# vlongle/pixie

Hardware: AMD Instinct MI355X
Metric: voxels/s (128^3 U-Net fwd) + MPM particle-steps/s (higher is better)
Workload: dtype f32 (operands split fp16 hi+lo, 3 f16 MFMAs/product, fp32 accumulate); 1 GPU; 128^3x64 feature grid -> SegmentationUNet+RegressionUNet forward (+argmax/one-hot combine), 1 scene per GPU per step; grid=128, feature_channels=64, parallelism=scene-parallel x1, executor=c+hip_graph

## Files before the change

### include/pixie_hip.h

```cpp
#ifndef PIXIE_HIP_H
#define PIXIE_HIP_H

#include <stdint.h>

#ifdef __cplusplus
extern "C" {
#endif

const char* pixie_last_error(void);
const char* pixie_build_arch(void);

typedef struct pixie_mpm pixie_mpm;

int pixie_mpm_create(pixie_mpm** out, int n_particles, int n_grid, double grid_lim);
int pixie_mpm_destroy(pixie_mpm* h);
int pixie_mpm_regrid(pixie_mpm* h, int n_grid, double grid_lim, void* stream);

int pixie_mpm_set_field(pixie_mpm* h, const char* name, const void* d_src, int64_t count, void* stream);
int pixie_mpm_get_field(pixie_mpm* h, const char* name, void* d_dst, int64_t count, void* stream);
int pixie_mpm_fill_field(pixie_mpm* h, const char* name, double value, void* stream);

int pixie_mpm_set_scalar(pixie_mpm* h, const char* key, double value);
int pixie_mpm_get_scalar(pixie_mpm* h, const char* key, double* value);

// ... 72 lines not shown
    int32_t in_d, in_h, in_w;
    int32_t upsample;
    int32_t stride;
    int32_t ksize;
    const float* d_pro_a; const float* d_pro_b;
    const float* d_gamma; const float* d_beta;
    int32_t act;
    const float* d_w; const float* d_bias;
    int32_t c_out;
    const float* d_residual;
    float* d_out;
    const void* d_w16;
    const uint32_t* d_in_amax0; const uint32_t* d_in_amax1;
    float in_bound;
    float* d_out_stats;
    uint32_t* d_out_amax;
    void* d_workspace;
    int32_t out_d, out_h, out_w;
    const float* d_skip_in0; int32_t skip_c0;
    const float* d_skip_in1; int32_t skip_c1;
    const void* d_skip_w16; const float* d_skip_bias;
    const uint32_t* d_skip_amax0; const uint32_t* d_skip_amax1;
    int32_t w16_subpixel;
} pixie_conv_desc;

int pixie_conv_cout_padded(int c_out);
int pixie_conv_pack_weights(const float* d_w_oidhw, float* d_w_packed, int c_out, int c_in, int ksize, void* stream);
int64_t pixie_conv_packed16_bytes(int c_out, int c_in, int ksize);
int pixie_conv_pack_weights_f16x2(const float* d_w_oidhw, void* d_packed, int c_out, int c_in, int ksize, void* stream);
int64_t pixie_conv_subpixel_bytes(int c_out, int c_in);
int pixie_conv_pack_weights_subpixel(const float* d_w_oidhw, void* d_packed, int c_out, int c_in, void* stream);
int pixie_conv3d_forward(const pixie_conv_desc* desc, void* stream);
int64_t pixie_conv_stats_floats(const pixie_conv_desc* desc);
int64_t pixie_conv_workspace_bytes(const pixie_conv_desc* desc);
int pixie_stats_finalize(const float* d_stats, const pixie_conv_desc* desc, double* d_sums, void* stream);
int pixie_stats_norm_finalize(const float* d_stats0, const pixie_conv_desc* desc0, double* d_sums0, const float* d_stats1,
                              const pixie_conv_desc* desc1, double* d_sums1, int c1, int64_t spatial, int mode, int groups,
                              double eps, const float* d_weight, const float* d_bias, float* d_a, float* d_b, void* stream);
int pixie_conv_skip_foldable(const pixie_conv_desc* desc);

int pixie_channel_sums(const float* d_x, int channels, int64_t spatial, double* d_sums, void* stream);
int pixie_channel_stats(const float* d_x, int channels, int64_t spatial, double* d_sums, uint32_t* d_amax, void* stream);
int pixie_tensor_amax(const float* d_x, int64_t count, uint32_t* d_slot, void* stream);
int pixie_norm_finalize(const double* d_sums, int channels, int64_t spatial, int mode, int groups, double eps,
                        const float* d_weight, const float* d_bias, float* d_a, float* d_b, void* stream);

int pixie_attention_forward(const float* d_qkv, float* d_out, int channels, int tokens, void* stream);

int pixie_channel_affine(const float* d_x, const float* d_a, const float* d_b, float* d_y, int channels,
                         int64_t spatial, void* stream);

int pixie_voxel_grid_to_ncdhw(const void* d_feat_dhwc_f16, int d, int h, int w, int channels, float* d_out_cdhw, void* stream);

int pixie_projector_conv0(const void* d_feat_dhwc_f16, int64_t voxels, int channels, int n_networks, const void* const* d_w16,
                          const float* const* d_bias, float* const* d_out, int c_out, void* stream);

int pixie_pack_fields(const float* d_cont, const int32_t* d_seg_pred, int64_t n_scenes, int64_t spatial, void* d_wire, int64_t wire_bytes,
                      void* stream);

int pixie_combine_predictions(const float* d_logits, int num_classes, const float* d_cont, int64_t spatial,
                              float* d_combined, int32_t* d_argmax , void* stream);

int pixie_combine_class_ids(const int32_t* d_seg_pred, int num_classes, const float* d_cont, int64_t spatial, float* d_combined,
                            void* stream);

typedef struct pixie_unet pixie_unet;
typedef struct pixie_unet_config {
    int32_t feature_channels, cond_dim, model_channels, num_res_blocks;
    int32_t n_channel_mult; int32_t channel_mult[8];
    int32_t n_attention_resolutions; int32_t attention_resolutions[8];
    int32_t grid_size;
    int32_t out_channels;
    int32_t precision;
} pixie_unet_config;

int pixie_unet_create(pixie_unet** out, const pixie_unet_config* cfg);
int pixie_unet_destroy(pixie_unet* h);
int pixie_unet_param_count(const pixie_unet* h);
int pixie_unet_param_info(const pixie_unet* h, int index, const char** key, int64_t* numel, int32_t* ndim, int64_t shape[5]);
int pixie_unet_set_param(pixie_unet* h, const char* key, const float* d_values, int64_t numel);
int64_t pixie_unet_workspace_bytes(pixie_unet* h, int d, int hh, int w);
int pixie_unet_forward(pixie_unet* h, const float* d_feat, const float* d_proj0, int d, int hh, int w, float* d_out,
                       void* d_workspace, int64_t workspace_bytes, void* stream);
int pixie_unet_set_option(pixie_unet* h, const char* key, int value);

typedef struct pixie_field_desc {
    const float* d_pred;
    const uint8_t* d_mask;
    const float* d_axis_x; const float* d_axis_y; const float* d_axis_z;
    int32_t n_classes, d, h, w;
    double min_spacing;
    double density_min, density_max, E_min, E_max, nu_min, nu_max;
} pixie_field_desc;
int pixie_field_to_particles(const pixie_field_desc* field, const float* d_pos, int n, int k, double nn_distance_threshold,
                             int weighted, int default_material, int default_part_label, float* d_density, float* d_E,
                             float* d_nu, int32_t* d_material, int32_t* d_part_label, float* d_conf, float* d_nearest,
                             void* d_scratch, void* stream);

int pixie_unscale_prediction(const float* d_pred, int channels, int64_t spatial, double density_min, double density_max,
                             double E_min, double E_max, double nu_min, double nu_max, float* d_out, void* stream);
int64_t pixie_field_points_scratch_bytes(const pixie_field_desc* field);
int pixie_field_points(const pixie_field_desc* field, int64_t capacity, float* d_xyz , float* d_density, float* d_E,
                       float* d_nu, int32_t* d_material, float* d_conf, int64_t* d_count, void* d_scratch, void* stream);

int pixie_dbscan_roots(const float* d_pos_sorted, const int32_t* d_orig_index, const int32_t* d_cell_start, int n, int nx, int ny, int nz,
                       const double lo[3], double cell_size, double eps, int min_samples, int32_t* d_core_scratch,
                       int32_t* d_parent_scratch, int32_t* d_root, void* stream);

int pixie_fill_densify(const float* d_pos, const float* d_opacity, const float* d_cov6, int n, int grid_n, double grid_dx,
                       int32_t* d_grid_count, float* d_grid_density, void* stream);
int pixie_fill_dense_cells(int32_t* d_grid_count, const float* d_grid_density, int grid_n, double grid_dx, double density_thres,
                           int max_particles_per_cell, float* d_new_particles , int64_t max_samples,
                           uint64_t* d_counter, uint32_t seed, void* stream);
int pixie_fill_internal_cells(int32_t* d_grid_count, const float* d_grid_density, int grid_n, double grid_dx, int max_particles_per_cell,
                              int exclude_dir, int ray_cast_dir, double threshold, float* d_new_particles, int64_t max_samples,
                              uint64_t* d_counter, uint32_t seed, void* stream);
int pixie_particle_volume(const float* d_pos, int n, int grid_n, double grid_dx, int32_t* d_grid_count_scratch, float* d_vol, void* stream);
int pixie_nearest_particle(const float* d_pos, int n, const float* d_new_pos, int n_new, int32_t* d_nearest, void* stream);

typedef struct pixie_raster_desc {
    int32_t n, width, height;
    float tanfovx, tanfovy, scale_modifier;
    float viewmatrix[16], projmatrix[16], bg[3];
    int32_t pad_;
    const float* d_means;
    const float* d_cov3d;
    const float* d_scales;
    const float* d_rotations;
    const float* d_colors;
    const float* d_opacity;
    float* d_out_color;
    int32_t* d_radii;
    float* d_final_T;
    int32_t* d_n_contrib;
    void* d_workspace;
    int64_t workspace_bytes;
} pixie_raster_desc;
int64_t pixie_raster_workspace_bytes(int n, int width, int height, int64_t max_instances);
int pixie_raster_forward(const pixie_raster_desc* desc, int64_t* instances_out, void* stream);
int pixie_sh_to_rgb(const float* d_shs, int64_t n, int k_coeffs, int degree, const float* d_pos , const float campos[3],
                    const float* d_rot , int64_t n_rot, float* d_out , void* stream);

typedef struct pixie_raster_view {
    float viewmatrix[16], projmatrix[16], campos[3];
    float tanfovx, tanfovy;
} pixie_raster_view;
typedef struct pixie_raster_batch_desc {
    int32_t views, n_dyn, n_static, width, height;
    int32_t sh_degree, k_coeffs;
    float scale_modifier;
    float bg[3];
    int32_t pad_;
    const pixie_raster_view* view;
    const float* d_means;
    const float* d_cov3d;
    int64_t means_view_stride, cov3d_view_stride;
    const float* d_static_means;
    const float* d_static_cov3d;
    const float* d_opacity;
    const float* d_colors;
    int64_t colors_view_stride;
    const float* d_shs;
    float* d_out_color;
    uint8_t* d_out_rgb8;
    int32_t* d_radii;
    float* d_final_T;
// ... 273 lines not shown
```

### pixie_amd/_lib.py

```python
from __future__ import annotations

import ctypes as C
import os

_HERE = os.path.dirname(os.path.abspath(__file__))
LIB_PATH = os.path.join(_HERE, "libpixie_hip.so")
DIAG_LIB_PATH = os.path.join(_HERE, "libpixie_hip_diag.so")


class PixieHipError(RuntimeError):
    pass


class BCDesc(C.Structure):
    _fields_ = [("type", C.c_int32), ("surface_type", C.c_int32), ("reset", C.c_int32), ("pad_", C.c_int32),
                ("point", C.c_double * 3), ("size", C.c_double * 3), ("velocity", C.c_double * 3),
                ("normal", C.c_double * 3), ("start_time", C.c_double), ("end_time", C.c_double),
                ("friction", C.c_double)]


class PModDesc(C.Structure):
    _fields_ = [("type", C.c_int32), ("pad_", C.c_int32),
                ("point", C.c_double * 3), ("size", C.c_double * 3), ("force", C.c_double * 3),
                ("velocity", C.c_double * 3), ("normal", C.c_double * 3), ("h1", C.c_double * 3),
# ... 179 lines not shown
                ("group", GsAdamGroup * 8)]


class GsDensifyDesc(C.Structure):
    _fields_ = [("n", C.c_int64), ("n_rest", C.c_int32), ("has_max_screen_size", C.c_int32),
                ("max_grad", C.c_double), ("min_opacity", C.c_double), ("extent", C.c_double), ("percent_dense", C.c_double),
                ("d_xyz_gradient_accum", C.c_void_p), ("d_denom", C.c_void_p),
                ("d_param", C.c_void_p * 6), ("d_exp_avg", C.c_void_p * 6), ("d_exp_avg_sq", C.c_void_p * 6),
                ("d_workspace", C.c_void_p), ("workspace_bytes", C.c_int64)]


class GsDensifyOuts(C.Structure):
    _fields_ = [("n_out", C.c_int64), ("n_split", C.c_int64), ("d_noise", C.c_void_p),
                ("d_param", C.c_void_p * 6), ("d_exp_avg", C.c_void_p * 6), ("d_exp_avg_sq", C.c_void_p * 6),
                ("d_source_index", C.c_void_p), ("d_xyz_gradient_accum", C.c_void_p), ("d_denom", C.c_void_p),
                ("d_max_radii2D", C.c_void_p)]


GS_DENSIFY_BAD_MAX_GRAD, GS_DENSIFY_TOO_MANY_ROWS, GS_DENSIFY_EMPTY = 2, 3, 4


INGEST_NO_SELECTION, INGEST_ZERO_EXTENT, INGEST_TOO_MANY_ROTATIONS, INGEST_TOO_MANY_ROWS = 2, 3, 4, 5


_VP, _I, _I64, _D, _S = C.c_void_p, C.c_int, C.c_int64, C.c_double, C.c_char_p
_D3 = C.POINTER(C.c_double)
SIGNATURES = {
    "pixie_last_error": (C.c_char_p, []),
    "pixie_build_arch": (C.c_char_p, []),
    "pixie_mpm_create": (_I, [C.POINTER(_VP), _I, _I, _D]),
    "pixie_mpm_destroy": (_I, [_VP]),
    "pixie_mpm_regrid": (_I, [_VP, _I, _D, _VP]),
    "pixie_mpm_set_field": (_I, [_VP, _S, _VP, _I64, _VP]),
    "pixie_mpm_get_field": (_I, [_VP, _S, _VP, _I64, _VP]),
    "pixie_mpm_fill_field": (_I, [_VP, _S, _D, _VP]),
    "pixie_mpm_set_scalar": (_I, [_VP, _S, _D]),
    "pixie_mpm_get_scalar": (_I, [_VP, _S, C.POINTER(_D)]),
    "pixie_mpm_update_mass": (_I, [_VP, _VP]),
    "pixie_mpm_finalize_mu_lam": (_I, [_VP, _I, _VP]),
    "pixie_mpm_apply_additional_params": (_I, [_VP, _D3, _D3, _D, _D, _D, _I, _VP]),
    "pixie_mpm_apply_additional_params_batch": (_I, [_VP, _I64, _VP, _VP, _VP, _VP]),
    "pixie_mpm_add_bc": (_I, [_VP, C.POINTER(BCDesc)]),
    "pixie_mpm_add_particle_modifier": (_I, [_VP, C.POINTER(PModDesc), _VP]),
    "pixie_mpm_step": (_I, [_VP, _D, _I, _VP]),
    "pixie_mpm_export_cov": (_I, [_VP, _VP, _VP]),
    "pixie_mpm_export_R": (_I, [_VP, _VP, _VP]),
    "pixie_mpm_export_frame": (_I, [_VP, _I, _D3, _D, _D3, C.POINTER(C.c_double), _VP, _VP, _VP]),
    "pixie_mpm_out_of_bounds": (_I, [_VP, C.POINTER(_I64), _VP]),
    "pixie_mpm_batch_create": (_I, [C.POINTER(_VP), C.POINTER(_VP), _I]),
    "pixie_mpm_batch_step": (_I, [_VP, _D, _I, _VP]),
    "pixie_mpm_batch_run": (_I, [_VP, C.POINTER(BatchSched), _I, _VP]),
    "pixie_mpm_batch_run_splats": (_I, [_VP, C.POINTER(BatchSched), C.POINTER(BatchSplatOut), _I, _VP]),
    "pixie_splat_from_cov": (_I, [_VP, _I64, _VP, _VP, _VP]),
    "pixie_mpm_export_frame_splats": (_I, [_VP, _I, _D3, _D, _D3, C.POINTER(C.c_double), _VP, _VP, _VP, _VP, _VP]),
    "pixie_mpm_batch_destroy": (_I, [_VP]),
    "pixie_pack_fields": (_I, [_VP, _VP, _I64, _I64, _VP, _I64, _VP]),
    "pixie_conv_cout_padded": (_I, [_I]),
    "pixie_conv_pack_weights": (_I, [_VP, _VP, _I, _I, _I, _VP]),
    "pixie_conv_packed16_bytes": (_I64, [_I, _I, _I]),
    "pixie_conv_pack_weights_f16x2": (_I, [_VP, _VP, _I, _I, _I, _VP]),
    "pixie_conv_subpixel_bytes": (_I64, [_I, _I]),
    "pixie_conv_pack_weights_subpixel": (_I, [_VP, _VP, _I, _I, _VP]),
    "pixie_conv3d_forward": (_I, [C.POINTER(ConvDesc), _VP]),
    "pixie_conv_stats_floats": (_I64, [C.POINTER(ConvDesc)]),
    "pixie_conv_workspace_bytes": (_I64, [C.POINTER(ConvDesc)]),
    "pixie_stats_finalize": (_I, [_VP, C.POINTER(ConvDesc), _VP, _VP]),
    "pixie_stats_norm_finalize": (_I, [_VP, C.POINTER(ConvDesc), _VP, _VP, C.POINTER(ConvDesc), _VP, _I, _I64, _I, _I, _D, _VP, _VP, _VP, _VP, _VP]),
    "pixie_channel_stats": (_I, [_VP, _I, _I64, _VP, _VP, _VP]),
    "pixie_tensor_amax": (_I, [_VP, _I64, _VP, _VP]),
    "pixie_channel_sums": (_I, [_VP, _I, _I64, _VP, _VP]),
    "pixie_norm_finalize": (_I, [_VP, _I, _I64, _I, _I, _D, _VP, _VP, _VP, _VP, _VP]),
    "pixie_attention_forward": (_I, [_VP, _VP, _I, _I, _VP]),
    "pixie_channel_affine": (_I, [_VP, _VP, _VP, _VP, _I, _I64, _VP]),
    "pixie_projector_conv0": (_I, [_VP, _I64, _I, _I, C.POINTER(_VP), C.POINTER(_VP), C.POINTER(_VP), _I, _VP]),
    "pixie_conv_skip_foldable": (_I, [C.POINTER(ConvDesc)]),
    "pixie_unet_create": (_I, [C.POINTER(_VP), C.POINTER(UNetConfigC)]),
    "pixie_unet_destroy": (_I, [_VP]),
    "pixie_unet_param_count": (_I, [_VP]),
    "pixie_unet_param_info": (_I, [_VP, _I, C.POINTER(_S), C.POINTER(_I64), C.POINTER(C.c_int32), C.POINTER(_I64)]),
    "pixie_unet_set_param": (_I, [_VP, _S, _VP, _I64]),
    "pixie_unet_workspace_bytes": (_I64, [_VP, _I, _I, _I]),
    "pixie_unet_set_option": (_I, [_VP, _S, _I]),
    "pixie_unet_forward": (_I, [_VP, _VP, _VP, _I, _I, _I, _VP, _VP, _I64, _VP]),
    "pixie_combine_class_ids": (_I, [_VP, _I, _VP, _I64, _VP, _VP]),
    "pixie_combine_predictions": (_I, [_VP, _I, _VP, _I64, _VP, _VP, _VP]),
    "pixie_voxel_grid_to_ncdhw": (_I, [_VP, _I, _I, _I, _I, _VP, _VP]),
    "pixie_unscale_prediction": (_I, [_VP, _I, _I64, _D, _D, _D, _D, _D, _D, _VP, _VP]),
    "pixie_field_points_scratch_bytes": (_I64, [C.POINTER(FieldDesc)]),
    "pixie_field_points": (_I, [C.POINTER(FieldDesc), _I64, _VP, _VP, _VP, _VP, _VP, _VP, _VP, _VP, _VP]),
    "pixie_fill_densify": (_I, [_VP, _VP, _VP, _I, _I, _D, _VP, _VP, _VP]),
    "pixie_fill_dense_cells": (_I, [_VP, _VP, _I, _D, _D, _I, _VP, _I64, _VP, C.c_uint32, _VP]),
    "pixie_fill_internal_cells": (_I, [_VP, _VP, _I, _D, _I, _I, _I, _D, _VP, _I64, _VP, C.c_uint32, _VP]),
    "pixie_particle_volume": (_I, [_VP, _I, _I, _D, _VP, _VP, _VP]),
    "pixie_nearest_particle": (_I, [_VP, _I, _VP, _I, _VP, _VP]),
    "pixie_dbscan_roots": (_I, [_VP, _VP, _VP, _I, _I, _I, _I, C.POINTER(_D), _D, _D, _I, _VP, _VP, _VP, _VP]),
    "pixie_raster_workspace_bytes": (_I64, [_I, _I, _I, _I64]),
    "pixie_raster_forward": (_I, [C.POINTER(RasterDesc), C.POINTER(_I64), _VP]),
    "pixie_raster_backward_workspace_bytes": (_I64, [_I, _I, _I, _I64]),
    "pixie_raster_backward": (_I, [C.POINTER(RasterBackwardDesc), _VP]),
    "pixie_sh_to_rgb": (_I, [_VP, _I64, _I, _I, _VP, C.POINTER(C.c_float), _VP, _I64, _VP, _VP]),
    "pixie_raster_batch_workspace_bytes": (_I64, [_I, _I, _I, _I, _I64]),
    "pixie_raster_forward_batch": (_I, [C.POINTER(RasterBatchDesc), C.POINTER(_I64), C.POINTER(C.c_int32), _VP]),
    "pixie_scene_ingest_workspace_bytes": (_I64, [_I64]),
    "pixie_scene_ingest": (_I, [C.POINTER(IngestDesc), C.POINTER(_I64), C.POINTER(C.c_float), C.POINTER(C.c_float), _VP]),
    "pixie_field_to_particles": (_I, [C.POINTER(FieldDesc), _VP, _I, _I, _D, _I, _I, _I, _VP, _VP, _VP, _VP, _VP, _VP, _VP, _VP, _VP]),
    "pixie_knn_mean_dist2_scratch_bytes": (_I64, [_I64]),
    "pixie_knn_mean_dist2": (_I, [_VP, _I64, _VP, _I64, _VP, _VP]),
    "pixie_photometric_workspace_bytes": (_I64, [_I, _I, _I, _I, _I]),
    "pixie_photometric_forward": (_I, [_VP, _VP, _I, _I, _I, _I, _VP, _I64, _I, _VP, _VP, _VP]),
    "pixie_photometric_backward": (_I, [_VP, _VP, _I, _I, _I, _I, _VP, _VP, _VP, _VP, _VP]),
    "pixie_gs_adam_step": (_I, [C.POINTER(GsAdamDesc), _VP]),
    "pixie_gs_densify_stats": (_I, [_VP, _VP, _I64, _VP, _VP, _VP, _VP]),
    "pixie_gs_densify_workspace_bytes": (_I64, [_I64]),
    "pixie_gs_densify_plan": (_I, [C.POINTER(GsDensifyDesc), C.POINTER(_I64), C.POINTER(_I64), _VP]),
    "pixie_gs_densify_emit": (_I, [C.POINTER(GsDensifyDesc), C.POINTER(GsDensifyOuts), _VP]),
    "pixie_occupancy_scratch_bytes": (_I64, [C.POINTER(OccupancyDesc), _I]),
    "pixie_occupancy_mask": (_I, [C.POINTER(OccupancyDesc), _VP, _VP, _VP, _VP, _VP]),
    "pixie_part_seg_scratch_bytes": (_I64, [C.POINTER(PartSegDesc)]),
    "pixie_part_segmentation": (_I, [C.POINTER(PartSegDesc), _VP, _VP, _VP, _VP, _VP, _VP, _VP]),
    "pixie_part_material_grid": (_I, [_VP, _VP, _I, _I64, C.c_float, _VP, _VP]),
    "pixie_hashmlp_forward": (_I, [C.POINTER(HashMlpDesc), _VP, _VP, _I64, _VP, _VP]),
    "pixie_hashmlp_train_bytes": (_I, [C.POINTER(HashMlpDesc), _I64, C.POINTER(_I64), C.POINTER(_I64)]),
    "pixie_hashmlp_forward_saved": (_I, [C.POINTER(HashMlpDesc), _VP, _VP, _I64, _VP, _VP, _VP]),
    "pixie_hashmlp_backward": (_I, [C.POINTER(HashMlpDesc), _VP, _VP, _I64, _VP, _VP, _VP, C.POINTER(HashMlpGrads), _VP, _VP]),
    "pixie_ray_composite_bytes": (_I, [C.POINTER(RayDesc), C.POINTER(_I64)]),
    "pixie_ray_composite_forward": (_I, [C.POINTER(RayDesc), C.POINTER(RayInputs), C.POINTER(RayOutputs), _VP]),
    "pixie_ray_composite_backward": (_I, [C.POINTER(RayDesc), C.POINTER(RayInputs), C.POINTER(RayUpstream), C.POINTER(RayGrads), _VP, _VP]),
    "pixie_field_voxelize": (_I, [C.POINTER(FieldVoxelizeDesc), _VP, _VP, _VP, _VP, _VP, _VP]),
    "pixie_field_query_points": (_I, [C.POINTER(FieldVoxelizeDesc), _VP, _I64, _D, _VP, _VP, _VP, _VP, _VP]),
}

DIAG_SIGNATURES = {
    "pixie_mpm_phase": (_I, [_VP, _I, _D, _VP]),
    "pixie_mpm_kernel_times": (_I, [_VP, C.POINTER(_D), C.POINTER(_D), C.POINTER(_I64)]),
    "pixie_conv_kernel_variant": (C.c_int, [C.POINTER(ConvDesc), C.POINTER(C.c_int)]),
    "pixie_conv_tile_geometry": (C.c_int, [C.POINTER(ConvDesc), C.POINTER(C.c_int32)]),
    "pixie_conv_stats_layout": (C.c_int, [C.POINTER(ConvDesc), C.POINTER(C.c_int64)]),
}

_libs = {}


def load(diag: bool = False):
    if diag in _libs:
        return _libs[diag]
    path = DIAG_LIB_PATH if diag else LIB_PATH
    if not os.path.exists(path):
        raise PixieHipError(
            f"{path} not found: build it with `python -m pixie_amd.build` (hipcc, gfx950). "
            "pixie_amd has no CPU fallback.")
    import torch
    lib = C.CDLL(path)
    for name, (res, args) in list(SIGNATURES.items()) + (list(DIAG_SIGNATURES.items()) if diag else []):
        fn = getattr(lib, name)
        fn.restype = res
        fn.argtypes = args
    _libs[diag] = lib
    return lib


def check(rc: int, what: str = "", lib=None):
    if rc != 0:
        msg = (lib or load()).pixie_last_error()
        raise PixieHipError(f"{what}: {msg.decode() if msg else 'unknown error'}")


# ... 11 lines not shown
```

### pixie_amd/csrc/common.hip

```cpp
#include "common.h"

#include <mutex>
#include <set>
#include <utility>

#include "../../include/pixie_hip.h"

namespace pixie {
hipError_t allow_max_dynamic_lds(const void* kern) {
    static std::mutex mu;
    static std::set<std::pair<const void*, int>> done;
    int dev = 0;
    hipError_t e = hipGetDevice(&dev);
    if (e != hipSuccess) return e;
    std::lock_guard<std::mutex> lock(mu);
    if (done.count({kern, dev})) return hipSuccess;
    e = hipFuncSetAttribute(kern, hipFuncAttributeMaxDynamicSharedMemorySize, 160 * 1024);
    if (e == hipSuccess) done.insert({kern, dev});
    return e;
}

std::string& last_error_ref() {
    static thread_local std::string msg;
    return msg;
}
int set_error(const char* fmt, ...) {
    char buf[1024];
    va_list ap;
    va_start(ap, fmt);
    vsnprintf(buf, sizeof buf, fmt, ap);
    va_end(ap);
    last_error_ref() = buf;
    return 1;
}
}

extern "C" const char* pixie_last_error(void) { return pixie::last_error_ref().c_str(); }
extern "C" const char* pixie_build_arch(void) { return "gfx950"; }
```

### pixie_amd/csrc/conv16_body.h

```cpp
#pragma once
#include <type_traits>

#include "conv16_device.h"

namespace pixie {

template <int KS, int MB, int NB, bool EX = false, bool SP = false, int SK = 0, bool PAIR = false>
__device__ __forceinline__ void conv3d_f16x3_body(const Conv16Args& A) {
    static_assert(!PAIR || (MB == 2 && !EX && !SP && SK == 0), "pair form: the plain f16x3 body with 64 c_out per quartet");
    static_assert(!SP || (KS == 3 && NB == 4 && !EX), "sub-pixel path: 3^3, two x parities x two voxel blocks per wave");
    static_assert(SK == 0 || (!EX && !SP), "folded skip (SK: 1 register-fed, 2 staged through LDS): f16x3, no sub-pixel form");
    extern __shared__ uint4 smem16[];
    constexpr int PAD = (KS == 3) ? 1 : 0;
    constexpr int NW = 4, NT = 64 * NW;
    const int bufsz = 4 * A.CS;

    const int tid = threadIdx.x;
    const int lane = tid & 63;
    const int quartet = PAIR ? __builtin_amdgcn_readfirstlane(tid >> 8) : 0;
    const int wave = PAIR ? (tid >> 6) & 3 : tid >> 6;
    const int qtid = PAIR ? tid & 255 : tid;
    const int kh = lane >> 5;
    const int l31 = lane & 31;

    int t = blockIdx.x;
    {
        const int per = (A.n_tiles + 7) >> 3;
        const int cand = (t & 7) * per + (t >> 3);
        if ((A.n_tiles & 7) == 0) t = cand;
    }
    int par = 0;
    if constexpr (SP) { par = t & 3; t >>= 2; }
    const int py = par & 1, pz = par >> 1;
    const int tx = t % A.tiles_x; t /= A.tiles_x;
    const int ty = t % A.tiles_y;
    const int tz = t / A.tiles_y;
    const int ox0 = tx * A.TX, oy0 = ty * A.TY, oz0 = tz * A.TZ;
    const int cout0 = (PAIR ? 2 * (int)blockIdx.y + quartet : (int)blockIdx.y) * (MB * 32);
    const int lx0 = SP ? ox0 - 1 : ox0 * A.stride - PAD;
    const int ly0 = SP ? oy0 - 1 + py : oy0 * A.stride - PAD;
    const int lz0 = SP ? oz0 - 1 + pz : oz0 * A.stride - PAD;
    const size_t ISP = (size_t)A.ID * A.IH * A.IW;
    const size_t OSP = (size_t)A.OD * A.OH * A.OW;

    int voff[NB];
    int ovox[NB];
    bool valid[NB];
#pragma unroll
    for (int nb = 0; nb < NB; ++nb) {
        if constexpr (SP) {
            const int px = nb >> 1;
            const int j = (wave * 2 + (nb & 1)) * 32 + l31;
            int x = j & (A.TX - 1);
            int y = (j >> A.lTX) & (A.TY - 1);
            int z = j >> (A.lTX + A.lTY);
            const int gx = 2 * (ox0 + x) + px, gy = 2 * (oy0 + y) + py, gz = 2 * (oz0 + z) + pz;
            const bool v = (z < A.TZ) && (gx < A.OW) && (gy < A.OH) && (gz < A.OD);
            if (!v) { x = 0; y = 0; z = 0; }
            voff[nb] = (z * A.HY + y) * A.HX + x + px + kh * A.CS;
            ovox[nb] = v ? (gz * A.OH + gy) * A.OW + gx : 0;
            valid[nb] = v;
            continue;
        }
        const int j = (wave * NB + nb) * 32 + l31;
        int x = j & (A.TX - 1);
        int y = (j >> A.lTX) & (A.TY - 1);
        int z = j >> (A.lTX + A.lTY);
        const bool v = (z < A.TZ) && (ox0 + x < A.OW) && (oy0 + y < A.OH) && (oz0 + z < A.OD);
        if (!v) { x = 0; y = 0; z = 0; }
        voff[nb] = ((z * A.HY + y) * A.HX + x) * A.stride + kh * A.CS;
        ovox[nb] = ((oz0 + z) * A.OH + (oy0 + y)) * A.OW + ox0 + x;
        valid[nb] = v;
    }

    float bound = A.in_bound;
    if (A.amax0) {
        bound = __uint_as_float(*A.amax0);
        if (A.amax1) bound = fmaxf(bound, __uint_as_float(*A.amax1));
    }
    const int ex = EX ? 0 : scale_exponent(bound);
    const float sx = pow2i(ex);

    f32x16 acc[MB][NB];
#pragma unroll
    for (int mb = 0; mb < MB; ++mb)
#pragma unroll
        for (int nb = 0; nb < NB; ++nb)
#pragma unroll
            for (int r = 0; r < 16; ++r) acc[mb][nb][r] = 0.0f;

    const int KG = A.cin >> 3;
    const size_t tap_stride = (size_t)KG * A.coutp;
    const size_t plane = (size_t)(SP ? 64 : KS * KS * KS) * tap_stride;
    const uint4* wHi = A.w16 + kW16HeaderU4 + (size_t)kh * A.coutp + cout0 + l31 + (size_t)(par * 16) * tap_stride;
    const uint4* wLo = wHi + plane;
    const float* wF = A.wf + (size_t)kh * A.coutp + cout0 + l31;

    constexpr int TAPS = KS * KS * KS;
#include "conv16_stage.h"
#include "conv16_taps.h"

    float inv2 = 0.0f;
    {
        const int c_begin = A.partial ? (int)blockIdx.z * A.chunks_per_slice * 16 : 0;
        const int c_end = A.partial ? min(A.cin, c_begin + A.chunks_per_slice * 16) : A.cin;
        if constexpr (PAIR) {
            const int n_chunks = (c_end - c_begin) >> 4;
            const int half = (A.CS + 1) >> 1;
            const int s0 = quartet ? half : 0, s1 = quartet ? A.CS : half;
#pragma unroll 1
            for (int h = -1; h < 2 * n_chunks; ++h) {
                const int k = h >> 1;
                const bool stage = (h < 0 || ((h + quartet) & 1) == 0) && k + 1 < n_chunks;
                const bool multiply = h >= 0 && ((h + quartet) & 1) != 0;
                if (stage) stage_chunk(c_begin + 16 * (k + 1), smem16 + ((k + 1) & 1) * bufsz, qtid, NT, s0, s1);
                if (multiply) mfma_chunk(c_begin + 16 * k, smem16 + (k & 1) * bufsz);
                if (h & 1) __syncthreads();
            }
        } else {
            for (int c_base = c_begin; c_base < c_end; c_base += 16) {
                __syncthreads();
                stage_chunk(c_base, smem16, tid, NT, 0, A.CS);
                __syncthreads();
                mfma_chunk(c_base, smem16);
            }
        }
#include "conv16_skip.h"
    }

#include "conv16_epilogue.h"
}

template <int KS, int MB, int NB>
__global__ __launch_bounds__(256, 2) void conv3d_f16x3_kernel(Conv16Args A) {
    conv3d_f16x3_body<KS, MB, NB>(A);
}
template <int KS, int NB>
__global__ __launch_bounds__(512, 1) void conv3d_f16x3_pair_kernel(Conv16Args A) {
    conv3d_f16x3_body<KS, 2, NB, false, false, 0, true>(A);
}
template <int KS, int MB, int NB, bool STAGED>
__global__ __launch_bounds__(256, 2) void conv3d_f16x3_skip_kernel(Conv16Args A) {
    conv3d_f16x3_body<KS, MB, NB, false, false, STAGED ? 2 : 1>(A);
}
template <int KS, int MB, int NB>
__global__ __launch_bounds__(256, 2) void conv3d_exact_kernel(Conv16Args A) {
    conv3d_f16x3_body<KS, MB, NB, true>(A);
}
template <int MB>
__global__ __launch_bounds__(256, 2) void conv3d_f16x3_subpixel_kernel(Conv16Args A) {
    conv3d_f16x3_body<3, MB, 4, false, true>(A);
}
__global__ __launch_bounds__(256, 2) void conv3d_f16x3_c64_fullres_kernel(Conv16Args A) {
    conv3d_f16x3_body<3, 2, 4>(A);
}

}
```

### pixie_amd/csrc/conv16_epilogue.h

```cpp
    const float inv = EX ? 1.0f : (SK != 0 ? inv2 : __uint_as_float(A.w16[0].x) * pow2i(-ex));
    if (A.partial) {
        float* dst = A.partial + (size_t)blockIdx.z * A.cout * OSP;
#pragma unroll
        for (int mb = 0; mb < MB; ++mb)
#pragma unroll
            for (int r = 0; r < 16; ++r) {
                const int co = cout0 + mb * 32 + (r & 3) + 8 * (r >> 2) + 4 * kh;
                if (co < A.cout) {
#pragma unroll
                    for (int nb = 0; nb < NB; ++nb)
                        if (valid[nb]) dst[(size_t)co * OSP + ovox[nb]] = acc[mb][nb][r] * inv;
                }
            }
        return;
    }
    constexpr int LDO_ = NB * 32 + 4;
    float* red = reinterpret_cast<float*>(smem16) + (PAIR ? (A.epi_lds ? 2 * NW * 32 * LDO_ : 0) + quartet * (NW * MB * 64) : 0);
    float wmax = 0.0f;
    const bool full = SP ? (A.epi_lds && cout0 + MB * 32 <= A.cout && (A.TX & 1) == 0 && (A.OW & 3) == 0 && NW * 64 <= A.TX * A.TY * A.TZ &&
                            2 * (ox0 + A.TX) <= A.OW && 2 * (oy0 + A.TY) <= A.OH && 2 * (oz0 + A.TZ) <= A.OD)
                         : (A.epi_lds && cout0 + MB * 32 <= A.cout && (A.TX & 3) == 0 && (A.OW & 3) == 0 && NW * NB * 32 <= A.TX * A.TY * A.TZ &&
                            ox0 + A.TX <= A.OW && oy0 + A.TY <= A.OH && oz0 + A.TZ <= A.OD);
    if (full) {
        constexpr int LDO = NB * 32 + 4;
        float* ldsO = reinterpret_cast<float*>(smem16) + (quartet * NW + wave) * (32 * LDO);
        if constexpr (!PAIR) red = reinterpret_cast<float*>(smem16) + NW * 32 * LDO;
        constexpr int LPR = NB * 8;
        constexpr int RPI = 32 / LPR;
        constexpr int NIT = 16 / RPI;
        constexpr int G = 4;
        constexpr int GPB = NIT / G;
        constexpr int NGRP = MB * GPB;
        const int rsub = l31 / LPR, colq = 4 * (l31 % LPR), nbq = colq >> 5;
        const float* nobias = EX ? A.wf : reinterpret_cast<const float*>(A.w16);
        const bool hb0 = A.bias != nullptr, hb1 = A.sk_bias != nullptr;
        float braw[MB][2];
#pragma unroll
        for (int mb = 0; mb < MB; ++mb) {
            braw[mb][0] = (hb0 ? A.bias : nobias)[cout0 + mb * 32 + l31];
            braw[mb][1] = (hb1 ? A.sk_bias : nobias)[cout0 + mb * 32 + l31];
        }
        __syncthreads();
        const int jq = SP ? wave * 64 + (colq >> 1) : (wave * NB + nbq) * 32 + (colq & 31);
        const int xq = jq & (A.TX - 1), yq = (jq >> A.lTX) & (A.TY - 1), zq = jq >> (A.lTX + A.lTY);
        const size_t ovq = SP ? ((size_t)(2 * (oz0 + zq) + pz) * A.OH + (2 * (oy0 + yq) + py)) * A.OW + 2 * (ox0 + xq)
                              : ((size_t)(oz0 + zq) * A.OH + (oy0 + yq)) * A.OW + ox0 + xq;
        const size_t orow0 = (size_t)(cout0 + kh * RPI + rsub) * OSP + ovq;
        auto rows = [&](auto res_c, auto stats_c) {
            constexpr bool RES = decltype(res_c)::value, STATS = decltype(stats_c)::value;
            size_t step = (size_t)(2 * RPI) * OSP;
            asm volatile("" : "+s"(step));
            const float* pr = A.residual + orow0;
            float* po = A.out + orow0;
            float4 r4[2][G];
            auto fetch = [&](int q) {
#pragma unroll
                for (int g = 0; g < G; ++g) { r4[q & 1][g] = *reinterpret_cast<const float4*>(pr); pr += step; }
            };
#pragma unroll
            for (int q = 0; q < NGRP; ++q) {
                const int mb = q / GPB, it0 = (q % GPB) * G;
                asm volatile("" ::: "memory");
                if (q % GPB == 0) {
                    const int brow = __float_as_int((hb0 ? braw[mb][0] : 0.0f) + (hb1 ? braw[mb][1] : 0.0f));
#pragma unroll
                    for (int r = 0; r < 16; ++r) {
                        const int row = (r & 3) + 8 * (r >> 2);
                        const int blo = __builtin_amdgcn_readlane(brow, row), bhi = __builtin_amdgcn_readlane(brow, row + 4);
                        const float bv = __int_as_float(kh ? bhi : blo);
#pragma unroll
                        for (int nb = 0; nb < NB; ++nb)
                            ldsO[((r & 3) + 8 * (r >> 2) + 4 * kh) * LDO + (SP ? 2 * ((nb & 1) * 32 + l31) + (nb >> 1) : nb * 32 + l31)] =
                                __builtin_fmaf(acc[mb][nb][r], inv, bv);
                    }
                }
                if constexpr (RES) {
                    if (q == 0) fetch(0);
                    if (q + 1 < NGRP) fetch(q + 1);
                }
                float4 v4[G];
#pragma unroll
                for (int g = 0; g < G; ++g) {
                    const int rowl = (2 * (it0 + g) + kh) * RPI + rsub;
                    v4[g] = *reinterpret_cast<const float4*>(ldsO + rowl * LDO + colq);
                    if constexpr (RES) { v4[g].x += r4[q & 1][g].x; v4[g].y += r4[q & 1][g].y; v4[g].z += r4[q & 1][g].z; v4[g].w += r4[q & 1][g].w; }
// ... 78 lines not shown
```

### pixie_amd/csrc/conv3d_f16x3.hip

```cpp
#include <hip/hip_runtime.h>

#include <cstdlib>

#include "../../include/pixie_hip.h"
#include "common.h"
#include "conv_plan.h"
#include "conv_launch.h"
#include "conv16_device.h"
#include "conv16_body.h"
#include "conv_stat_kernels.h"
#include "conv_pack_kernels.h"

namespace pixie {

bool conv_exact_v1() { return getenv("PIXIE_CONV_EXACT_V1") != nullptr; }

ConvShape conv_shape_of(const pixie_conv_desc* d) {
    ConvShape s;
    s.c0 = d->c0; s.c1 = d->c1; s.c_out = d->c_out;
    s.in_d = d->in_d; s.in_h = d->in_h; s.in_w = d->in_w;
    s.ksize = d->ksize; s.stride = d->stride; s.upsample = d->upsample;
    s.out_d = d->out_d; s.out_h = d->out_h; s.out_w = d->out_w;
    s.skip_c0 = d->skip_c0; s.skip_c1 = d->skip_c1;
    s.w16 = d->d_w16 != nullptr; s.subpixel = d->w16_subpixel != 0; s.workspace = d->d_workspace != nullptr; s.skip = d->d_skip_w16 != nullptr;
    s.exact_v1 = conv_exact_v1();
    return s;
}

using ConvKernel = void (*)(Conv16Args);
static ConvKernel conv16_kernel(const ConvPlan& p, bool skip = false, int skip_c0 = 0) {
    if (p.path == CONV_F16X3_SUBPIXEL) return p.MB == 2 ? conv3d_f16x3_subpixel_kernel<2> : conv3d_f16x3_subpixel_kernel<1>;
    if (p.fullres) return conv3d_f16x3_c64_fullres_kernel;
#define PX_CONV16_PICK(KS_, MB_, NB_)                                                                \
    if (p.KS == KS_ && p.MB == MB_ && p.NB == NB_)                                                   \
        return p.path == CONV_EXACT_TILED ? conv3d_exact_kernel<KS_, MB_, NB_>                       \
                                          : (!skip ? conv3d_f16x3_kernel<KS_, MB_, NB_>                                \
                                                   : ((skip_c0 & 8) ? conv3d_f16x3_skip_kernel<KS_, MB_, NB_, true> : conv3d_f16x3_skip_kernel<KS_, MB_, NB_, false>));
    PX_CONV_VARIANTS(PX_CONV16_PICK)
#undef PX_CONV16_PICK
    return nullptr;
}

#ifdef PIXIE_DIAG
static int g_conv_keep_four_wave = 0;
#endif
static size_t conv_pair_lds(const ConvPlan& p, bool skip) {
#ifdef PIXIE_DIAG
    if (g_conv_keep_four_wave) return 0;
#endif
    return conv_pair_lds_bytes(p, skip);
}
static ConvKernel conv16_pair_kernel(const ConvPlan& p) {
#define PX_CONV16_PAIR(KS_, NB_) \
    if (p.KS == KS_ && p.NB == NB_) return conv3d_f16x3_pair_kernel<KS_, NB_>;
    PX_CONV16_PAIR(3, 4) PX_CONV16_PAIR(1, 4)
#undef PX_CONV16_PAIR
    return nullptr;
}

static int launch(ConvKernel kern, const ConvPlan& p, const Conv16Args& a, hipStream_t st, size_t pair_lds = 0) {
    PX_REQUIRE(kern != nullptr, "conv: no kernel variant for ksize=%d MB=%d NB=%d", p.KS, p.MB, p.NB);
    PX_CHECK_HIP(allow_max_dynamic_lds(reinterpret_cast<const void*>(kern)));
    if (pair_lds) hipLaunchKernelGGL(kern, dim3(p.grid_x, p.grid_y / 2, 1), dim3(512), pair_lds, st, a);
    else hipLaunchKernelGGL(kern, dim3(p.grid_x, p.grid_y, p.grid_z), dim3(256), p.lds_bytes, st, a);
    PX_CHECK_HIP(hipGetLastError());
    return 0;
}

static Conv16Args conv16_args(const pixie_conv_desc* d, const ConvPlan& p) {
    Conv16Args a{};
    a.in0 = d->d_in0; a.in1 = d->d_in1; a.c0 = d->c0; a.cin = d->c0 + d->c1;
    a.ID = d->in_d; a.IH = d->in_h; a.IW = d->in_w;
    a.LD = p.LD; a.LH = p.LH; a.LW = p.LW; a.ups = p.ups; a.stride = d->stride;
    a.OD = p.OD; a.OH = p.OH; a.OW = p.OW;
    a.pro_a = d->d_pro_a; a.pro_b = d->d_pro_b; a.gamma = d->d_gamma; a.beta = d->d_beta; a.act = d->act;
    a.bias = d->d_bias; a.cout = d->c_out; a.coutp = p.coutp;
    a.residual = d->d_residual; a.out = d->d_out;
    a.TX = p.TX; a.TY = p.TY; a.TZ = p.TZ; a.lTX = p.lTX; a.lTY = p.lTY;
    a.tiles_x = p.tiles_x; a.tiles_y = p.tiles_y; a.tiles_z = p.tiles_z; a.n_tiles = p.n_tiles;
    a.HX = p.HX; a.HY = p.HY; a.HZ = p.HZ; a.HYX = p.HYX; a.CS = p.CS; a.mHX = p.mHX; a.mHYX = p.mHYX;
    a.chunks_per_slice = p.chunks_per_slice; a.epi_lds = p.epi_lds;
    return a;
}

int conv3d_f16x3_forward(const pixie_conv_desc* d, const ConvPlan& p, hipStream_t st) {
    PX_REQUIRE(p.refusal != CONV_BAD_STRIDE, "f16x3 conv: stride must be 1, or 2 for a 3^3 kernel");
    PX_REQUIRE(p.refusal != CONV_BAD_CHANNELS, "f16x3 conv: c_in must be a multiple of 16 (got %d+%d)", d->c0, d->c1);
    PX_REQUIRE(d->d_in_amax0 != nullptr || d->in_bound > 0.0f, "f16x3 conv: needs d_in_amax0 or a positive in_bound");
    PX_REQUIRE(d->c1 == 0 || d->d_in_amax0 == nullptr || d->d_in_amax1 != nullptr, "f16x3 conv: second input needs its own amax slot");
    PX_REQUIRE(p.refusal != CONV_BAD_SUBPIXEL, "f16x3 conv: sub-pixel weights need upsample = 1, ksize = 3, stride = 1 and no folded skip");
    PX_REQUIRE((int64_t)d->in_d * d->in_h * d->in_w * 16 * (int64_t)sizeof(float) < (int64_t)1 << 32, "f16x3 conv: 16 channels of the input must span less than 4 GiB");
    Conv16Args a = conv16_args(d, p);
    a.w16 = reinterpret_cast<const uint4*>(d->d_w16);
    a.amax0 = d->d_in_amax0; a.amax1 = (d->c1 > 0) ? d->d_in_amax1 : nullptr; a.in_bound = d->in_bound;
    a.stats = d->d_out_stats; a.out_amax = d->d_out_amax;
    if (d->d_skip_w16) {
        PX_REQUIRE(p.skip_foldable, "f16x3 conv: this launch cannot fold a skip convolution (pixie_conv_skip_foldable)");
        PX_REQUIRE(d->d_skip_in0 && d->d_skip_amax0 && (d->skip_c1 == 0 || (d->d_skip_in1 && d->d_skip_amax1)), "f16x3 conv: folded skip needs its inputs and their amax slots");
        PX_REQUIRE((int64_t)d->in_d * d->in_h * d->in_w * 16 * (int64_t)sizeof(float) < (int64_t)1 << 32, "f16x3 conv: folded skip: 16 channels of the skip input must span less than 4 GiB");
        a.sk_in0 = d->d_skip_in0; a.sk_in1 = d->d_skip_in1; a.sk_c0 = d->skip_c0; a.sk_cin = d->skip_c0 + d->skip_c1;
        a.sk_w16 = reinterpret_cast<const uint4*>(d->d_skip_w16); a.sk_bias = d->d_skip_bias;
        a.sk_amax0 = d->d_skip_amax0; a.sk_amax1 = d->skip_c1 > 0 ? d->d_skip_amax1 : nullptr;
    }
    if (p.slices > 1) {
        a.partial = static_cast<float*>(d->d_workspace);
        a.stats = nullptr; a.out_amax = nullptr;
    }
    PX_REQUIRE(p.refusal != CONV_BAD_LDS, "f16x3 conv: tile needs %zu B of LDS", p.lds_bytes);
    PX_REQUIRE(p.f16x3(), "f16x3 conv: bad sizes");
    const size_t pair_lds = conv_pair_lds(p, a.sk_w16 != nullptr);
    if (int rc = launch(pair_lds ? conv16_pair_kernel(p) : conv16_kernel(p, a.sk_w16 != nullptr, a.sk_c0), p, a, st, pair_lds)) return rc;
    if (p.slices == 1) return 0;
    const long osp = (long)a.OD * a.OH * a.OW, n_elems = (long)a.cout * osp;
    if (d->d_out_stats) {
        const dim3 rgrid((unsigned)reduce_segments(osp), (unsigned)a.cout);
        double* rstats = reinterpret_cast<double*>(d->d_out_stats);
        PX_REQUIRE((reinterpret_cast<size_t>(rstats) & 7) == 0, "f16x3 conv: d_out_stats of a split-K launch must be 8-byte aligned");
        const bool vec = osp % 4 == 0 && ((reinterpret_cast<size_t>(a.partial) | reinterpret_cast<size_t>(a.residual) | reinterpret_cast<size_t>(a.out)) & 15) == 0;
        if (vec) hipLaunchKernelGGL(splitk_reduce_stats_kernel<true>, rgrid, dim3(256), 0, st, a.partial, p.slices, n_elems, osp, a.bias, a.residual,
                                    a.out, rstats, d->d_out_amax);
        else hipLaunchKernelGGL(splitk_reduce_stats_kernel<false>, rgrid, dim3(256), 0, st, a.partial, p.slices, n_elems, osp, a.bias, a.residual,
                                a.out, rstats, d->d_out_amax);
    } else {
        hipLaunchKernelGGL(splitk_reduce_kernel, dim3((unsigned)((n_elems + 255) / 256)), dim3(256), 0, st, a.partial, p.slices, n_elems, osp,
                           a.bias, a.residual, a.out);
    }
    PX_CHECK_HIP(hipGetLastError());
    return 0;
}

int conv3d_exact_forward(const pixie_conv_desc* d, const ConvPlan& p, hipStream_t st) {
    PX_REQUIRE(p.refusal != CONV_BAD_LDS, "exact conv: tile needs %zu B of LDS", p.lds_bytes);
    PX_REQUIRE(p.path == CONV_EXACT_TILED, "exact conv: bad sizes");
    Conv16Args a = conv16_args(d, p);
    a.wf = d->d_w;
    a.in_bound = 1.0f;
    return launch(conv16_kernel(p), p, a, st);
}

}

using namespace pixie;

static ConvPlan plan_of(const pixie_conv_desc* d) { return d ? conv_plan(conv_shape_of(d)) : ConvPlan{}; }
static StatParts stat_parts(const ConvPlan& p, const void* stats) { return StatParts{stats, p.stats.n, p.stats.cstride, p.stats.tstride, p.stats.f64}; }

extern "C" int64_t pixie_conv_stats_floats(const pixie_conv_desc* d) { return plan_of(d).stats_floats; }

extern "C" int64_t pixie_conv_workspace_bytes(const pixie_conv_desc* d) {
    if (!d) return 0;
    ConvShape s = conv_shape_of(d);
    s.workspace = true;
    return conv_plan(s).workspace_bytes;
}

#ifdef PIXIE_DIAG
extern "C" int pixie_conv_kernel_variant(const pixie_conv_desc* d, int* slices_out) {
    if (!d) {
        const int before = g_conv_keep_four_wave;
        if (slices_out && (*slices_out == 0 || *slices_out == 1)) g_conv_keep_four_wave = *slices_out;
        return before;
    }
    const ConvPlan p = plan_of(d);
    if (slices_out) *slices_out = p.f16x3() ? p.slices : 1;
    return conv_variant_number(p);
}

extern "C" int pixie_conv_tile_geometry(const pixie_conv_desc* d, int32_t out[10]) {
    const ConvPlan p = plan_of(d);
    if (!out && d) return (int)conv_pair_lds(p, d->d_skip_w16 != nullptr);
    return out && conv_tile_geometry(p, out) ? 0 : 1;
}

extern "C" int pixie_conv_stats_layout(const pixie_conv_desc* d, int64_t out[6]) {
    const ConvPlan p = plan_of(d);
    return out && conv_stats_layout(p, out) ? 0 : 1;
}
#endif

extern "C" int pixie_conv_skip_foldable(const pixie_conv_desc* d) { return plan_of(d).skip_foldable ? 1 : 0; }

extern "C" int pixie_stats_finalize(const float* d_stats, const pixie_conv_desc* d, double* d_sums, void* stream) {
    PX_REQUIRE(d_stats && d && d_sums, "pixie_stats_finalize: null argument");
    hipLaunchKernelGGL(stats_finalize_kernel, dim3((unsigned)d->c_out), dim3(256), 0, as_stream(stream), stat_parts(plan_of(d), d_stats), d_sums);
    PX_CHECK_HIP(hipGetLastError());
    return 0;
}

extern "C" int pixie_stats_norm_finalize(const float* d_stats0, const pixie_conv_desc* desc0, double* d_sums0, const float* d_stats1,
                                         const pixie_conv_desc* desc1, double* d_sums1, int c1, int64_t spatial, int mode, int groups,
                                         double eps, const float* d_weight, const float* d_bias, float* d_a, float* d_b, void* stream) {
    PX_REQUIRE(desc0 && d_sums0 && d_a && d_b && spatial > 0 && c1 >= 0, "pixie_stats_norm_finalize: bad arguments");
    PX_REQUIRE(c1 == 0 || d_sums1, "pixie_stats_norm_finalize: a second part needs d_sums1");
    PX_REQUIRE(!d_stats1 || desc1, "pixie_stats_norm_finalize: d_stats1 needs its descriptor");
    const int c0 = desc0->c_out, channels = c0 + c1;
    PX_REQUIRE(!d_stats1 || desc1->c_out == c1, "pixie_stats_norm_finalize: desc1 has %d output channels, c1 is %d", desc1 ? desc1->c_out : 0, c1);
    PX_REQUIRE(mode == 0 || (mode == 1 && groups > 0 && channels % groups == 0), "pixie_stats_norm_finalize: bad mode/groups");
    const StatParts none{nullptr, 0, 0, 0, 0};
    const StatParts p0 = d_stats0 ? stat_parts(plan_of(desc0), d_stats0) : none;
    const StatParts p1 = d_stats1 ? stat_parts(plan_of(desc1), d_stats1) : none;
    hipLaunchKernelGGL(stats_norm_finalize_kernel, dim3((unsigned)(mode == 0 ? channels : groups)), dim3(256), 0, as_stream(stream), p0, d_sums0, c0,
                       p1, d_sums1, channels, (double)spatial, mode, groups, eps, d_weight, d_bias, d_a, d_b);
    PX_CHECK_HIP(hipGetLastError());
    return 0;
}

extern "C" int64_t pixie_conv_packed16_bytes(int c_out, int c_in, int ksize) {
    if (c_out <= 0 || c_in <= 0 || c_in % 8 != 0 || (ksize != 1 && ksize != 3)) return 0;
    const int64_t taps = (int64_t)ksize * ksize * ksize;
    return ((int64_t)kW16HeaderU4 + 2 * taps * (c_in / 8) * pixie_conv_cout_padded(c_out)) * (int64_t)sizeof(uint4);
}

extern "C" int pixie_tensor_amax(const float* d_x, int64_t count, uint32_t* d_slot, void* stream) {
    PX_REQUIRE(d_x && d_slot && count > 0, "pixie_tensor_amax: bad arguments");
    const int blocks = (int)std::min<int64_t>(2048, (count + 1023) / 1024);
    hipLaunchKernelGGL(amax_kernel, dim3(blocks), dim3(256), 0, as_stream(stream), d_x, (long)count, d_slot);
    PX_CHECK_HIP(hipGetLastError());
    return 0;
}

extern "C" int pixie_conv_pack_weights_f16x2(const float* d_w, void* d_packed, int c_out, int c_in, int ksize, void* stream) {
    PX_REQUIRE(d_w && d_packed && c_out > 0 && c_in > 0 && c_in % 8 == 0 && (ksize == 1 || ksize == 3),
               "pixie_conv_pack_weights_f16x2: bad arguments (c_in must be a multiple of 8)");
    hipStream_t st = as_stream(stream);
    const int taps = ksize * ksize * ksize;
    const int coutp = pixie_conv_cout_padded(c_out);
    unsigned* slot = reinterpret_cast<unsigned*>(d_packed) + 15;
    PX_CHECK_HIP(hipMemsetAsync(d_packed, 0, kW16HeaderU4 * sizeof(uint4), st));
    if (pixie_tensor_amax(d_w, (int64_t)c_out * c_in * taps, slot, stream)) return 1;
    const long total = (long)taps * (c_in / 8) * coutp;
    hipLaunchKernelGGL(pack_weights_f16x2_kernel, dim3(cdiv(total, 256)), dim3(256), 0, st, d_w, reinterpret_cast<uint4*>(d_packed), c_out,
                       c_in, taps, coutp, slot);
    PX_CHECK_HIP(hipGetLastError());
    return 0;
}

extern "C" int64_t pixie_conv_subpixel_bytes(int c_out, int c_in) {
    if (c_out <= 0 || c_in <= 0 || c_in % 16 != 0) return 0;
    return ((int64_t)kW16HeaderU4 + 2 * 64 * (int64_t)(c_in / 8) * pixie_conv_cout_padded(c_out)) * (int64_t)sizeof(uint4);
}

extern "C" int pixie_conv_pack_weights_subpixel(const float* d_w, void* d_packed, int c_out, int c_in, void* stream) {
    PX_REQUIRE(d_w && d_packed && c_out > 0 && c_in > 0 && c_in % 16 == 0,
               "pixie_conv_pack_weights_subpixel: bad arguments (c_in must be a multiple of 16)");
    hipStream_t st = as_stream(stream);
    const int coutp = pixie_conv_cout_padded(c_out);
    unsigned* slot = reinterpret_cast<unsigned*>(d_packed) + 15;
    PX_CHECK_HIP(hipMemsetAsync(d_packed, 0, kW16HeaderU4 * sizeof(uint4), st));
    const long pairs = (long)c_out * c_in;
    hipLaunchKernelGGL(subpixel_amax_kernel, dim3(cdiv(pairs, 256)), dim3(256), 0, st, d_w, pairs, slot);
    PX_CHECK_HIP(hipGetLastError());
    const long total = 64L * (c_in / 8) * coutp;
    hipLaunchKernelGGL(pack_weights_subpixel_kernel, dim3(cdiv(total, 256)), dim3(256), 0, st, d_w, reinterpret_cast<uint4*>(d_packed), c_out,
                       c_in, coutp, slot);
    PX_CHECK_HIP(hipGetLastError());
    return 0;
}
```

### pixie_amd/csrc/conv3d_mfma.hip

```cpp
#include <hip/hip_runtime.h>

#include "../../include/pixie_hip.h"
#include "common.h"
#include "conv_launch.h"
#include "conv_plan.h"

namespace pixie {

typedef float f32x16 __attribute__((ext_vector_type(16)));

struct ConvArgs {
    const float* in0; const float* in1;
    int c0, cin;
    int ID, IH, IW;
    int LD, LH, LW;
    int ups;
    int stride;
    int OD, OH, OW;
    const float* pro_a; const float* pro_b; const float* gamma; const float* beta;
    int act;
    const float* w; const float* bias;
    int cout, coutp;
    const float* residual; float* out;
    int TX, TY, TZ, lTX, lTY;
    int tiles_x, tiles_y, tiles_z;
    int HX, HY, HZ, HYX, CS;
    unsigned mHX, mHYX, mCS;
};

__device__ __forceinline__ int fast_div(int n, int d, unsigned magic) {
    return (d == 1) ? n : (int)__umulhi((unsigned)n, magic);
}

__device__ __forceinline__ float apply_act(float t, int act) {
    if (act == 1) return t > 0.0f ? t : 0.02f * t;
    if (act == 2) return t / (1.0f + __expf(-t));
    return t;
}

template <int KS, int MB, int NB, int CK>
__global__ __launch_bounds__(256, 2) void conv3d_mfma_kernel(ConvArgs A) {
    extern __shared__ __attribute__((aligned(16))) float smem[];
    constexpr int MBW = MB * 32;
    constexpr int TAPS = KS * KS * KS;
    constexpr int PAD = (KS == 3) ? 1 : 0;
    float* ldsX = smem;
    float* ldsW = smem + ((CK * A.CS + 3) & ~3);

    const int tid = threadIdx.x;
    const int lane = tid & 63;
    const int wave = tid >> 6;
    const int half = lane >> 5;
    const int l31 = lane & 31;

    int t = blockIdx.x;
    const int tx = t % A.tiles_x; t /= A.tiles_x;
    const int ty = t % A.tiles_y;
    const int tz = t / A.tiles_y;
    const int ox0 = tx * A.TX, oy0 = ty * A.TY, oz0 = tz * A.TZ;
    const int cout0 = blockIdx.y * MBW;
    const int lx0 = ox0 * A.stride - PAD, ly0 = oy0 * A.stride - PAD, lz0 = oz0 * A.stride - PAD;
    const size_t ISP = (size_t)A.ID * A.IH * A.IW;
    const size_t OSP = (size_t)A.OD * A.OH * A.OW;

    int voff[NB];
    int ovox[NB];
    bool valid[NB];
#pragma unroll
    for (int nb = 0; nb < NB; ++nb) {
        const int j = (wave * NB + nb) * 32 + l31;
        int x = j & (A.TX - 1);
        int y = (j >> A.lTX) & (A.TY - 1);
        int z = j >> (A.lTX + A.lTY);
        const bool v = (z < A.TZ) && (ox0 + x < A.OW) && (oy0 + y < A.OH) && (oz0 + z < A.OD);
        if (!v) { x = 0; y = 0; z = 0; }
        voff[nb] = ((z * A.stride) * A.HY + y * A.stride) * A.HX + x * A.stride + half * A.CS;
        ovox[nb] = ((oz0 + z) * A.OH + (oy0 + y)) * A.OW + ox0 + x;
        valid[nb] = v;
    }
    const int laneA = half * MBW + l31;

    f32x16 acc[MB][NB];
#pragma unroll
    for (int mb = 0; mb < MB; ++mb)
#pragma unroll
        for (int nb = 0; nb < NB; ++nb)
#pragma unroll
            for (int r = 0; r < 16; ++r) acc[mb][nb][r] = 0.0f;
// ... 18 lines not shown
                if (A.pro_a) val = val * A.pro_a[cg] + A.pro_b[cg];
                if (A.gamma) val = val * A.gamma[sidx] + A.beta[sidx];
                val = apply_act(val, A.act);
            }
            ldsX[idx] = val;
        }
        constexpr int WE4 = TAPS * CK * MBW / 4;
        for (int i4 = tid; i4 < WE4; i4 += 256) {
            const int idx = i4 * 4;
            const int m = idx & (MBW - 1);
            const int row = idx / MBW;
            const int c = row % CK;
            const int tap = row / CK;
            const int cg = c_base + c;
            const int co = cout0 + m;
            float4 wv = make_float4(0.f, 0.f, 0.f, 0.f);
            if (cg < A.cin && co < A.coutp)
                wv = *reinterpret_cast<const float4*>(A.w + ((size_t)tap * A.cin + cg) * A.coutp + co);
            *reinterpret_cast<float4*>(ldsW + idx) = wv;
        }
        __syncthreads();
#pragma unroll 1
        for (int dz = 0; dz < KS; ++dz) {
#pragma unroll 1
            for (int dy = 0; dy < KS; ++dy) {
#pragma unroll
                for (int dx = 0; dx < KS; ++dx) {
                    const int tap = (dz * KS + dy) * KS + dx;
                    const int tapoff = (dz * A.HY + dy) * A.HX + dx;
#pragma unroll
                    for (int kp = 0; kp < CK / 2; ++kp) {
                        float a[MB], b[NB];
#pragma unroll
                        for (int mb = 0; mb < MB; ++mb) a[mb] = ldsW[(tap * CK + 2 * kp) * MBW + mb * 32 + laneA];
#pragma unroll
                        for (int nb = 0; nb < NB; ++nb) b[nb] = ldsX[voff[nb] + 2 * kp * A.CS + tapoff];
#pragma unroll
                        for (int mb = 0; mb < MB; ++mb)
#pragma unroll
                            for (int nb = 0; nb < NB; ++nb)
                                acc[mb][nb] = __builtin_amdgcn_mfma_f32_32x32x2f32(a[mb], b[nb], acc[mb][nb], 0, 0, 0);
                    }
                }
            }
        }
    }

#pragma unroll
    for (int mb = 0; mb < MB; ++mb) {
#pragma unroll
        for (int r = 0; r < 16; ++r) {
            const int co = cout0 + mb * 32 + (r & 3) + 8 * (r >> 2) + 4 * half;
            if (co < A.cout) {
                const float bv = A.bias ? A.bias[co] : 0.0f;
#pragma unroll
                for (int nb = 0; nb < NB; ++nb) {
                    if (valid[nb]) {
                        const size_t o = (size_t)co * OSP + ovox[nb];
                        float val = acc[mb][nb][r] + bv;
                        if (A.residual) val += A.residual[o];
                        A.out[o] = val;
                    }
                }
            }
        }
    }
}

__global__ void pack_weights_kernel(const float* __restrict__ src, float* __restrict__ dst, int cout, int cin, int taps, int coutp) {
    const long total = (long)taps * cin * coutp;
    const long i = (long)blockIdx.x * blockDim.x + threadIdx.x;
    if (i >= total) return;
    const int co = (int)(i % coutp);
    const long row = i / coutp;
    const int ci = (int)(row % cin);
    const int tap = (int)(row / cin);
    dst[i] = (co < cout) ? src[((long)co * cin + ci) * taps + tap] : 0.0f;
}

template <int KS, int MB, int NB, int CK>
static int launch_variant(const ConvArgs& a, size_t lds_bytes, dim3 grid, hipStream_t st) {
    auto kern = conv3d_mfma_kernel<KS, MB, NB, CK>;
    PX_CHECK_HIP(allow_max_dynamic_lds(reinterpret_cast<const void*>(kern)));
    hipLaunchKernelGGL(kern, grid, dim3(256), lds_bytes, st, a);
    PX_CHECK_HIP(hipGetLastError());
    return 0;
}

}

using namespace pixie;

extern "C" int pixie_conv_cout_padded(int c_out) { return conv_cout_padded(c_out); }

extern "C" int pixie_conv_pack_weights(const float* d_w, float* d_packed, int c_out, int c_in, int ksize, void* stream) {
    PX_REQUIRE(d_w && d_packed && c_out > 0 && c_in > 0 && (ksize == 1 || ksize == 3), "pixie_conv_pack_weights: bad arguments");
    const int taps = ksize * ksize * ksize;
    const int coutp = pixie_conv_cout_padded(c_out);
    const long total = (long)taps * c_in * coutp;
    hipLaunchKernelGGL(pack_weights_kernel, dim3(cdiv(total, 256)), dim3(256), 0, as_stream(stream), d_w, d_packed, c_out, c_in, taps, coutp);
    PX_CHECK_HIP(hipGetLastError());
    return 0;
}

extern "C" int pixie_conv3d_forward(const pixie_conv_desc* d, void* stream) {
    PX_REQUIRE(d && d->d_in0 && (d->d_w || d->d_w16) && d->d_out, "pixie_conv3d_forward: null pointer in descriptor");
    PX_REQUIRE(d->ksize == 1 || d->ksize == 3, "pixie_conv3d_forward: ksize must be 1 or 3 (got %d)", d->ksize);
    PX_REQUIRE(d->stride == 1 || d->stride == 2, "pixie_conv3d_forward: stride must be 1 or 2 (got %d)", d->stride);
    PX_REQUIRE(d->upsample == 0 || d->upsample == 1, "pixie_conv3d_forward: upsample must be 0 or 1");
    PX_REQUIRE(d->c0 > 0 && d->c1 >= 0 && (d->c1 == 0 || d->d_in1), "pixie_conv3d_forward: bad channel split");
    PX_REQUIRE(d->c_out > 0 && d->in_d > 0 && d->in_h > 0 && d->in_w > 0, "pixie_conv3d_forward: bad sizes");
    PX_REQUIRE((d->d_pro_a == nullptr) == (d->d_pro_b == nullptr), "pixie_conv3d_forward: pro_a/pro_b must come together");
    PX_REQUIRE((d->d_gamma == nullptr) == (d->d_beta == nullptr), "pixie_conv3d_forward: gamma/beta must come together");
    PX_REQUIRE(!(d->d_gamma && d->upsample) || (d->d_w16 && d->w16_subpixel),
               "pixie_conv3d_forward: spatial affine with upsample needs the sub-pixel path (w16_subpixel), with gamma/beta of the stored grid");

    const ConvPlan p = conv_plan(conv_shape_of(d));
    if (d->d_w16) return conv3d_f16x3_forward(d, p, as_stream(stream));
    PX_REQUIRE(!d->d_skip_w16, "pixie_conv3d_forward: a folded skip convolution needs the f16x3 path (d_w16)");
    if (p.path != CONV_FIRST_GEN) return conv3d_exact_forward(d, p, as_stream(stream));

    ConvArgs a{};
    a.in0 = d->d_in0; a.in1 = d->d_in1; a.c0 = d->c0; a.cin = d->c0 + d->c1;
    a.ID = d->in_d; a.IH = d->in_h; a.IW = d->in_w;
    a.ups = p.ups; a.LD = p.LD; a.LH = p.LH; a.LW = p.LW;
    a.stride = d->stride;
    a.OD = p.OD; a.OH = p.OH; a.OW = p.OW;
    a.pro_a = d->d_pro_a; a.pro_b = d->d_pro_b; a.gamma = d->d_gamma; a.beta = d->d_beta; a.act = d->act;
    a.w = d->d_w; a.bias = d->d_bias; a.cout = d->c_out; a.coutp = pixie_conv_cout_padded(d->c_out);
    a.residual = d->d_residual; a.out = d->d_out;

    const long ovol = (long)a.OD * a.OH * a.OW;
    int MB = (a.coutp >= 64) ? 2 : 1;
    int NB = 4;
    auto n_wg = [&](int mb, int nb) {
        const long tiles = (ovol + 128L * nb - 1) / (128L * nb);
        return tiles * ((a.coutp + mb * 32 - 1) / (mb * 32));
    };
    while (n_wg(MB, NB) < 512 && NB > 1) NB /= 2;
    if (n_wg(MB, NB) < 512 && MB > 1) MB = 1;
    if (a.stride == 2 && NB > 2) NB = 2;

    const int tile_vox = 128 * NB;
    a.TX = pow2_le(a.OW, 32);
    a.TY = pow2_le(a.OH, std::max(1, tile_vox / a.TX));
    a.TZ = std::max(1, std::min(a.OD, tile_vox / (a.TX * a.TY)));
    a.lTX = ilog2(a.TX); a.lTY = ilog2(a.TY);
    a.tiles_x = (a.OW + a.TX - 1) / a.TX; a.tiles_y = (a.OH + a.TY - 1) / a.TY; a.tiles_z = (a.OD + a.TZ - 1) / a.TZ;
    a.HX = (a.TX - 1) * a.stride + d->ksize; a.HY = (a.TY - 1) * a.stride + d->ksize; a.HZ = (a.TZ - 1) * a.stride + d->ksize;
    a.HYX = a.HY * a.HX; a.CS = a.HZ * a.HYX;
    a.mHX = magic_of(a.HX); a.mHYX = magic_of(a.HYX); a.mCS = magic_of(a.CS);

    const int CK = d->ksize == 3 ? 4 : 16;
    const int taps = d->ksize * d->ksize * d->ksize;
    const size_t lds = ((size_t)((CK * a.CS + 3) & ~3) + (size_t)taps * CK * MB * 32) * sizeof(float);
    PX_REQUIRE(lds <= 160 * 1024, "pixie_conv3d_forward: tile needs %zu B of LDS", lds);
    const dim3 grid((unsigned)(a.tiles_x * a.tiles_y * a.tiles_z), (unsigned)((a.coutp + MB * 32 - 1) / (MB * 32)));
    hipStream_t st = as_stream(stream);

#define PX_CONV_CASE(KS_, MB_, NB_) \
    if (d->ksize == KS_ && MB == MB_ && NB == NB_) return launch_variant<KS_, MB_, NB_, (KS_ == 3 ? 4 : 16)>(a, lds, grid, st);
    PX_CONV_VARIANTS(PX_CONV_CASE)
#undef PX_CONV_CASE
    return set_error("pixie_conv3d_forward: no kernel variant for ksize=%d MB=%d NB=%d", d->ksize, MB, NB);
}
```

### pixie_amd/csrc/conv_stat_kernels.h

```cpp
#pragma once
#include <hip/hip_runtime.h>

#include "conv_plan.h"

namespace pixie {

struct StatParts { const void* p; int n; long cstride, tstride; int f64; };

__device__ inline void block_channel_sums(const StatParts& P, int c, double* r, double& o1, double& o2) {
    double s1 = 0.0, s2 = 0.0;
    for (int t = threadIdx.x; t < P.n; t += 256) {
        const size_t k = ((size_t)c * P.cstride + (size_t)t * P.tstride) * 2;
        if (P.f64) { const double2 v = *reinterpret_cast<const double2*>(static_cast<const double*>(P.p) + k); s1 += v.x; s2 += v.y; }
        else { const float2 v = *reinterpret_cast<const float2*>(static_cast<const float*>(P.p) + k); s1 += v.x; s2 += v.y; }
    }
    for (int off = 32; off > 0; off >>= 1) { s1 += __shfl_down(s1, off, 64); s2 += __shfl_down(s2, off, 64); }
    if ((threadIdx.x & 63) == 0) { r[2 * (threadIdx.x >> 6)] = s1; r[2 * (threadIdx.x >> 6) + 1] = s2; }
    __syncthreads();
    o1 = r[0] + r[2] + r[4] + r[6]; o2 = r[1] + r[3] + r[5] + r[7];
    __syncthreads();
}

__global__ __launch_bounds__(256) void stats_finalize_kernel(StatParts P, double* __restrict__ sums) {
    const int c = blockIdx.x;
    __shared__ double r[8];
    double s1, s2;
    block_channel_sums(P, c, r, s1, s2);
    if (threadIdx.x == 0) { sums[2 * c] = s1; sums[2 * c + 1] = s2; }
}

__global__ __launch_bounds__(256) void stats_norm_finalize_kernel(StatParts P0, double* sums0, int c0, StatParts P1, double* sums1, int channels,
                                                                  double spatial, int mode, int groups, double eps,
                                                                  const float* __restrict__ weight, const float* __restrict__ bias,
                                                                  float* __restrict__ a, float* __restrict__ b) {
    __shared__ double r[8];
    const int cpg = mode == 0 ? 1 : channels / groups;
    const int first = blockIdx.x * cpg;
    double s1 = 0.0, s2 = 0.0;
    for (int k = first; k < first + cpg; ++k) {
        const bool in0 = k < c0;
        const StatParts& P = in0 ? P0 : P1;
        double* sums = in0 ? sums0 : sums1;
        const int kc = in0 ? k : k - c0;
        double t1, t2;
        if (P.n > 0) {
            block_channel_sums(P, kc, r, t1, t2);
            if (threadIdx.x == 0) { sums[2 * kc] = t1; sums[2 * kc + 1] = t2; }
        } else {
            t1 = sums[2 * kc]; t2 = sums[2 * kc + 1];
        }
        s1 += t1; s2 += t2;
    }
    const double cnt = mode == 0 ? spatial : spatial * cpg;
    const double mean = s1 / cnt;
    double var = s2 / cnt - mean * mean;
    if (var < 0.0) var = 0.0;
    const double rstd = 1.0 / sqrt(var + eps);
    for (int k = first + threadIdx.x; k < first + cpg; k += 256) {
        if (mode == 0) {
            a[k] = (float)rstd;
            b[k] = (float)(-mean * rstd);
        } else {
            const double w = weight ? (double)weight[k] : 1.0;
            const double bb = bias ? (double)bias[k] : 0.0;
            a[k] = (float)(rstd * w);
            b[k] = (float)(bb - mean * rstd * w);
        }
    }
}

__global__ __launch_bounds__(256) void splitk_reduce_kernel(const float* __restrict__ partial, int slices, long n_elems, long osp,
                                                            const float* __restrict__ bias, const float* residual, float* out) {
    const long i = (long)blockIdx.x * 256 + threadIdx.x;
    if (i >= n_elems) return;
    float v = partial[i];
    for (int s = 1; s < slices; ++s) v += partial[(size_t)s * n_elems + i];
    if (bias) v += bias[i / osp];
    if (residual) v += residual[i];
    out[i] = v;
}

template <bool VEC>
__global__ __launch_bounds__(256) void splitk_reduce_stats_kernel(const float* __restrict__ partial, int slices, long n_elems, long osp,
                                                                  const float* __restrict__ bias, const float* residual, float* out,
                                                                  double* __restrict__ stats, unsigned* out_amax) {
    const int c = blockIdx.y;
    const long seg0 = (long)blockIdx.x * kReduceSeg;
    const size_t base = (size_t)c * osp;
    const float bv = bias ? bias[c] : 0.0f;
    double s1 = 0.0, s2 = 0.0;
    float mx = 0.0f;
    if (VEC) {
#pragma unroll
        for (int k = 0; k < kReduceSeg / 1024; ++k) {
            const long j = seg0 + k * 1024 + (long)threadIdx.x * 4;
            if (j < osp) {
                const size_t i = base + j;
                float4 v = *reinterpret_cast<const float4*>(partial + i);
                for (int s = 1; s < slices; ++s) {
                    const float4 q = *reinterpret_cast<const float4*>(partial + (size_t)s * n_elems + i);
                    v.x += q.x; v.y += q.y; v.z += q.z; v.w += q.w;
                }
                if (bias) { v.x += bv; v.y += bv; v.z += bv; v.w += bv; }
                if (residual) {
                    const float4 q = *reinterpret_cast<const float4*>(residual + i);
                    v.x += q.x; v.y += q.y; v.z += q.z; v.w += q.w;
                }
                *reinterpret_cast<float4*>(out + i) = v;
                const double x = v.x, y = v.y, z = v.z, w = v.w;
                s1 += (x + y) + (z + w);
                s2 += (x * x + y * y) + (z * z + w * w);
                mx = fmaxf(fmaxf(mx, fmaxf(fabsf(v.x), fabsf(v.y))), fmaxf(fabsf(v.z), fabsf(v.w)));
            }
        }
    } else {
#pragma unroll 4
        for (int k = 0; k < kReduceSeg / 256; ++k) {
            const long j = seg0 + k * 256 + threadIdx.x;
            if (j < osp) {
                const size_t i = base + j;
                float v = partial[i];
                for (int s = 1; s < slices; ++s) v += partial[(size_t)s * n_elems + i];
                if (bias) v += bv;
                if (residual) v += residual[i];
                out[i] = v;
                const double x = v;
                s1 += x; s2 += x * x; mx = fmaxf(mx, fabsf(v));
            }
        }
    }
    for (int off = 32; off > 0; off >>= 1) {
        s1 += __shfl_down(s1, off, 64);
        s2 += __shfl_down(s2, off, 64);
        mx = fmaxf(mx, __shfl_down(mx, off, 64));
    }
    __shared__ double r[8];
    __shared__ float rmx[4];
    const int lane = threadIdx.x & 63, wave = threadIdx.x >> 6;
    if (lane == 0) { r[2 * wave] = s1; r[2 * wave + 1] = s2; rmx[wave] = mx; }
    __syncthreads();
    if (threadIdx.x == 0) {
        double* dst = stats + ((size_t)c * gridDim.x + blockIdx.x) * 2;
        dst[0] = r[0] + r[2] + r[4] + r[6];
        dst[1] = r[1] + r[3] + r[5] + r[7];
        const unsigned m = __float_as_uint(fmaxf(fmaxf(rmx[0], rmx[1]), fmaxf(rmx[2], rmx[3])));
        if (out_amax && m > __hip_atomic_load(out_amax, __ATOMIC_RELAXED, __HIP_MEMORY_SCOPE_AGENT)) atomicMax(out_amax, m);
    }
}

__global__ __launch_bounds__(256) void amax_kernel(const float* __restrict__ x, long n, unsigned* __restrict__ slot) {
    float m = 0.0f;
    const long stride = (long)gridDim.x * 256 * 4;
    long i = ((long)blockIdx.x * 256 + threadIdx.x) * 4;
    if ((reinterpret_cast<size_t>(x) & 15) == 0) {
        for (; i + 3 < n; i += stride) {
            const float4 v = *reinterpret_cast<const float4*>(x + i);
            m = fmaxf(fmaxf(m, fabsf(v.x)), fmaxf(fabsf(v.y), fmaxf(fabsf(v.z), fabsf(v.w))));
        }
        for (long k = i; k < n && k < i + 4; ++k) m = fmaxf(m, fabsf(x[k]));
    } else {
        for (long k = (long)blockIdx.x * 256 + threadIdx.x; k < n; k += (long)gridDim.x * 256) m = fmaxf(m, fabsf(x[k]));
    }
    for (int off = 32; off > 0; off >>= 1) m = fmaxf(m, __shfl_down(m, off, 64));
    if ((threadIdx.x & 63) == 0 && m > 0.0f) atomicMax(slot, __float_as_uint(m));
}

}
```

### pixie_amd/csrc/unet_exec.hip

```cpp
#include <hip/hip_runtime.h>

#include <algorithm>
#include <cmath>
#include <cstdlib>
#include <cstring>
#include <map>
#include <memory>
#include <stdexcept>
#include <string>
#include <tuple>
#include <unordered_map>
#include <vector>

#include "../../include/pixie_hip.h"
#include "common.h"
#include "conv_launch.h"
#include "conv_plan.h"

namespace pixie {
int channel_stats_prezeroed(const float* d_x, int channels, int64_t spatial, double* d_sums, uint32_t* d_amax, hipStream_t st);
int norm_finalize_cat(const double* d_sums0, int c0, const double* d_sums1, int c1, int64_t spatial, int mode, int groups, double eps,
                      const float* d_weight, const float* d_bias, float* d_a, float* d_b, hipStream_t st);
namespace {

enum { ACT_NONE = 0, ACT_LEAKY = 1, ACT_SILU = 2 };
enum Kind { CONV_IN, RES, DOWN, ATTN, UP };

struct Blk { Kind kind; std::string prefix; int cin, cout, sp; };
struct Plan {
    std::vector<std::vector<Blk>> in_blocks, out_blocks;
    std::vector<Blk> middle;
    int out_sp = 0;
};

struct Err : std::runtime_error { using std::runtime_error::runtime_error; };
[[noreturn]] void fail(const char* fmt, ...) {
    char buf[512];
    va_list ap; va_start(ap, fmt); vsnprintf(buf, sizeof buf, fmt, ap); va_end(ap);
    throw Err(buf);
}
void ok(int rc, const char* what) { if (rc != 0) fail("%s: %s", what, pixie_last_error()); }

bool has(const std::vector<int>& v, int x) { for (int e : v) if (e == x) return true; return false; }

struct Cfg {
    int feature_channels, cond_dim, model_channels, num_res_blocks;
    std::vector<int> mult, attn;
    int grid_size, out_channels, precision;
    bool has_projector() const { return feature_channels != cond_dim; }
    int projector_hidden() const { return feature_channels > cond_dim ? 128 : 0; }
};

Plan build_plan(const Cfg& c) {
    Plan p;
    const int mc = c.model_channels, nrb = c.num_res_blocks;
    auto name = [](const char* part, int idx, int sub) { return std::string("unet.") + part + "." + std::to_string(idx) + "." + std::to_string(sub); };
    p.in_blocks.push_back({Blk{CONV_IN, "unet.input_blocks.0.0", c.cond_dim, mc, c.grid_size}});
    std::vector<int> chans{mc}, sizes{c.grid_size};
    int ch = mc, ds = 1, sp = c.grid_size;
    for (size_t level = 0; level < c.mult.size(); ++level) {
        const int m = c.mult[level];
        for (int r = 0; r < nrb; ++r) {
            const int idx = (int)p.in_blocks.size();
            std::vector<Blk> seq{Blk{RES, name("input_blocks", idx, 0), ch, m * mc, sp}};
            ch = m * mc;
            if (has(c.attn, ds)) seq.push_back(Blk{ATTN, name("input_blocks", idx, 1), ch, ch, sp});
            p.in_blocks.push_back(seq);
            chans.push_back(ch);
        }
        if (level + 1 != c.mult.size()) {
            const int idx = (int)p.in_blocks.size();
            p.in_blocks.push_back({Blk{DOWN, name("input_blocks", idx, 0), ch, ch, sp}});
            chans.push_back(ch);
            sizes.push_back(sp);
            ds *= 2;
            sp = (sp + 1) / 2;
        }
    }
    p.middle = {Blk{RES, "unet.middle_block.0", ch, ch, sp}, Blk{ATTN, "unet.middle_block.1", ch, ch, sp}, Blk{RES, "unet.middle_block.2", ch, ch, sp}};
    for (int level = (int)c.mult.size() - 1; level >= 0; --level) {
        const int m = c.mult[level];
        for (int i = 0; i <= nrb; ++i) {
            const int idx = (int)p.out_blocks.size();
            const int ich = chans.back(); chans.pop_back();
            std::vector<Blk> seq{Blk{RES, name("output_blocks", idx, 0), ch + ich, mc * m, sp}};
            ch = mc * m;
            if (has(c.attn, ds)) seq.push_back(Blk{ATTN, name("output_blocks", idx, (int)seq.size()), ch, ch, sp});
            if (level && i == nrb) {
                seq.push_back(Blk{UP, name("output_blocks", idx, (int)seq.size()), ch, ch, sp});
                ds /= 2;
                sp = sizes.back(); sizes.pop_back();
            }
            p.out_blocks.push_back(seq);
        }
    }
    p.out_sp = sp;
    return p;
}

struct Param {
// ... 94 lines not shown
        auto u = used_.find(off);
        if (u == used_.end()) return;
        int64_t size = u->second;
        used_.erase(u);
        auto next = free_.lower_bound(off);
        if (next != free_.end() && off + size == next->first) { size += next->second; next = free_.erase(next); }
        if (next != free_.begin()) {
            auto prev = std::prev(next);
            if (prev->first + prev->second == off) { prev->second += size; return; }
        }
        free_[off] = size;
    }
    template <class T> T* ptr(int64_t off) const { return reinterpret_cast<T*>(base + off); }
};

struct Exec;
struct Tens {
    Exec* ex = nullptr;
    float* p = nullptr;
    int64_t off = -1;
    int c = 0, d = 0, h = 0, w = 0;
    int64_t sums_off = -1;
    bool has_sums = false;
    double* sums = nullptr;
    int64_t partials_off = -1;
    pixie_conv_desc pdesc;
    uint32_t* slot = nullptr;
    int64_t spatial() const { return (int64_t)d * h * w; }
    ~Tens();
};
using TP = std::shared_ptr<Tens>;

struct Packed { void* d = nullptr; uint64_t version = ~0ull; };
struct Sized { int64_t bytes; int slots; int64_t zsum_doubles; };
struct Bound { float wmax = 0, bmax = 0; uint64_t wver = ~0ull, bver = ~0ull; };

}
}

using namespace pixie;

struct pixie_unet {
    Cfg cfg;
    Plan plan;
    std::vector<Param> params;
    std::unordered_map<std::string, int> index;
    std::unordered_map<std::string, Packed> packed32, packed16;
    std::unordered_map<std::string, Bound> bounds;
    uint32_t* d_bound_slots = nullptr;
    std::vector<uint32_t> h_bound_slots;
    std::map<std::tuple<int, int, int, bool>, Sized> sized;
    bool fuse_stats = true, split_k = true, fold_skip = true, subpixel = true;
    bool split_stats = true;
    struct Replay { const float* feat; const float* proj0; float* out; void* ws; int d; uint64_t epoch; hipGraph_t graph; hipGraphExec_t exec; };
    bool use_graph = false;
    uint64_t epoch = 0;
    std::vector<Replay> replays;
    static constexpr size_t kMaxReplays = 4;
    void drop_replay(size_t i) {
        (void)hipGraphExecDestroy(replays[i].exec);
        (void)hipGraphDestroy(replays[i].graph);
        replays.erase(replays.begin() + (long)i);
    }

    const Param& param(const std::string& key) const {
        auto it = index.find(key);
        if (it == index.end()) fail("pixie_unet: no parameter named '%s'", key.c_str());
        return params[it->second];
    }
};

namespace pixie {
namespace {

struct Exec {
    pixie_unet* net = nullptr;
    Arena arena;
    bool dry = false;
    void* stream = nullptr;
    uint32_t* slots = nullptr;
    int slot_next = 0, slot_cap = 0;
    double* zsums = nullptr;
    int64_t zsum_next = 0, zsum_cap = 0;

    TP make(int c, int d, int h, int w) {
        auto t = std::make_shared<Tens>();
        t->ex = this; t->c = c; t->d = d; t->h = h; t->w = w;
        t->off = arena.alloc((int64_t)c * d * h * w * sizeof(float));
        t->p = arena.ptr<float>(t->off);
        return t;
    }
    TP external(const float* p, int c, int d, int h, int w) {
        auto t = std::make_shared<Tens>();
        t->ex = this; t->p = const_cast<float*>(p); t->c = c; t->d = d; t->h = h; t->w = w;
        return t;
    }
    uint32_t* new_slot() {
        if (!dry && slot_next >= slot_cap) fail("pixie_unet_forward: out of |x|max slots (internal sizing error)");
        return dry ? (slot_next++, nullptr) : slots + slot_next++;
    }
    struct Scratch {
        Exec* ex; int64_t off;
        Scratch(Exec* e, int64_t bytes) : ex(e), off(e->arena.alloc(bytes)) {}
        ~Scratch() { ex->arena.release(off); }
        template <class T> T* as() const { return ex->arena.ptr<T>(off); }
    };

    const float* P(const std::string& key) {
        const Param& p = net->param(key);
        if (!dry && !p.d) fail("pixie_unet_forward: parameter '%s' was never set", key.c_str());
        return p.d;
    }
    const void* w16(const std::string& key, bool subpixel = false) {
        const Param& p = net->param(key + ".weight");
        if (dry) return nullptr;
        Packed& e = net->packed16[subpixel ? key + "#subpixel" : key];
        if (e.version != p.version) {
            const int cout = (int)p.shape[0], cin = (int)p.shape[1], k = (int)p.shape[2];
            const int64_t nb = subpixel ? (k == 3 ? pixie_conv_subpixel_bytes(cout, cin) : 0) : pixie_conv_packed16_bytes(cout, cin, k);
            if (nb <= 0) fail("pixie_unet: '%s' cannot take the f16x3 packing (c_in %d)", key.c_str(), cin);
            if (!e.d && hipMalloc(&e.d, (size_t)nb) != hipSuccess) fail("pixie_unet: hipMalloc of %lld bytes failed", (long long)nb);
            if (!p.d) fail("pixie_unet_forward: parameter '%s.weight' was never set", key.c_str());
            if (subpixel) ok(pixie_conv_pack_weights_subpixel(p.d, e.d, cout, cin, stream), "pixie_conv_pack_weights_subpixel");
            else ok(pixie_conv_pack_weights_f16x2(p.d, e.d, cout, cin, k, stream), "pixie_conv_pack_weights_f16x2");
            e.version = p.version;
        }
        return e.d;
    }
    const float* w32(const std::string& key) {
        const Param& p = net->param(key + ".weight");
        if (dry) return nullptr;
        Packed& e = net->packed32[key];
        if (e.version != p.version) {
            const int cout = (int)p.shape[0], cin = (int)p.shape[1], k = (int)p.shape[2];
            int64_t taps = 1;
            for (size_t i = 2; i < p.shape.size(); ++i) taps *= p.shape[i];
            const int64_t nb = taps * cin * pixie_conv_cout_padded(cout) * (int64_t)sizeof(float);
            if (!e.d && hipMalloc(&e.d, (size_t)nb) != hipSuccess) fail("pixie_unet: hipMalloc of %lld bytes failed", (long long)nb);
            if (!p.d) fail("pixie_unet_forward: parameter '%s.weight' was never set", key.c_str());
            ok(pixie_conv_pack_weights(p.d, static_cast<float*>(e.d), cout, cin, k, stream), "pixie_conv_pack_weights");
            e.version = p.version;
        }
        return static_cast<const float*>(e.d);
    }
    float norm_bound(const std::string& key, int64_t count) {
        if (dry) return 1.0f;
        const Bound& b = net->bounds[key];
        return (float)(std::sqrt((double)count) * (double)b.wmax + (double)b.bmax + 1e-30);
    }

    void stats(const TP& t) {
        if (t->has_sums || t->partials_off >= 0) return;
        t->has_sums = true;
        if (!dry && zsum_next + 2 * t->c > zsum_cap) fail("pixie_unet_forward: out of statistics space (internal sizing error)");
        t->sums = dry ? nullptr : zsums + zsum_next;
        zsum_next += 2 * t->c;
        t->slot = new_slot();
        if (!dry) ok(channel_stats_prezeroed(t->p, t->c, t->spatial(), t->sums, t->slot, as_stream(stream)), "pixie_channel_stats");
    }
    struct AB { std::shared_ptr<Scratch> mem; float* a; float* b; };
    AB norm_finalize(const std::vector<TP>& parts, int64_t spatial, int mode, int groups, const float* w, const float* b) {
        for (auto& t : parts) stats(t);
        const Tens* t0 = parts[0].get();
        const Tens* t1 = parts.size() > 1 ? parts[1].get() : nullptr;
        const int c0 = t0->c, c1 = t1 ? t1->c : 0, c = c0 + c1;
        AB r;
        const int cpad = (c + 63) / 64 * 64;
        r.mem = std::make_shared<Scratch>(this, (int64_t)(cpad + c) * sizeof(float));
        r.a = r.mem->as<float>();
        r.b = r.a + cpad;
        const bool p0 = t0->partials_off >= 0, p1 = t1 && t1->partials_off >= 0;
        if (p0 || p1) {
            pixie_conv_desc d0 = t0->pdesc;
            if (!p0) { std::memset(&d0, 0, sizeof d0); d0.c_out = c0; }
            if (!dry) ok(pixie_stats_norm_finalize(p0 ? arena.ptr<float>(t0->partials_off) : nullptr, &d0, t0->sums,
                                                   p1 ? arena.ptr<float>(t1->partials_off) : nullptr, p1 ? &t1->pdesc : nullptr, t1 ? t1->sums : nullptr,
                                                   c1, spatial, mode, groups, 1e-5, w, b, r.a, r.b, stream), "pixie_stats_norm_finalize");
            for (auto& t : parts)
                if (t->partials_off >= 0) { arena.release(t->partials_off); t->partials_off = -1; t->has_sums = true; }
        } else if (!t1) {
            if (!dry) ok(pixie_norm_finalize(t0->sums, c, spatial, mode, groups, 1e-5, w, b, r.a, r.b, stream), "pixie_norm_finalize");
        } else {
            if (!dry) ok(norm_finalize_cat(t0->sums, c0, t1->sums, c1, spatial, mode, groups, 1e-5, w, b, r.a, r.b, as_stream(stream)), "pixie_norm_finalize");
        }
        return r;
    }

    ConvPlan plan_conv(ConvShape& s, const std::vector<TP>& parts, int cout, int ksize, int stride, bool upsample) const {
        s.c0 = parts[0]->c; s.c1 = parts.size() > 1 ? parts[1]->c : 0; s.c_out = cout;
        s.in_d = parts[0]->d; s.in_h = parts[0]->h; s.in_w = parts[0]->w;
        s.ksize = ksize; s.stride = stride; s.upsample = upsample ? 1 : 0;
        s.w16 = net->cfg.precision == 0; s.workspace = net->split_k; s.exact_v1 = conv_exact_v1();
        ConvPlan p = conv_plan(s);
        if (p.refusal == CONV_BAD_CHANNELS) { s.w16 = s.subpixel = s.skip = false; p = conv_plan(s); }
        return p;
    }
    bool skip_foldable(const TP& x, int cout, int ksize, const std::vector<TP>& sp) const {
        ConvShape s;
        s.skip_c0 = sp[0]->c; s.skip_c1 = sp.size() > 1 ? sp[1]->c : 0;
        return plan_conv(s, {x}, cout, ksize, 1, false).skip_foldable;
    }

    struct ConvOpt {
        int stride = 1; bool upsample = false;
        const AB* pro = nullptr; std::string affine_store;
        int act = ACT_NONE; TP residual; float bound = 0.0f;
        int out_d = 0, out_h = 0, out_w = 0;
        float* out_ptr = nullptr;
        const std::vector<TP>* skip_parts = nullptr; std::string skip_key;
    };
    TP conv(const std::vector<TP>& parts, const std::string& wkey, int cout, int ksize, const ConvOpt& o) {
        const TP& x0 = parts[0];
        const Tens* x1 = parts.size() > 1 ? parts[1].get() : nullptr;
        ConvShape s;
        s.out_d = o.out_d; s.out_h = o.out_h; s.out_w = o.out_w;
        s.subpixel = net->subpixel && o.upsample && ksize == 3 && o.stride == 1;
        if (o.skip_parts) { s.skip = true; s.skip_c0 = (*o.skip_parts)[0]->c; s.skip_c1 = o.skip_parts->size() > 1 ? (*o.skip_parts)[1]->c : 0; }
        const ConvPlan plan = plan_conv(s, parts, cout, ksize, o.stride, o.upsample);
        const int od = plan.OD, oh = plan.OH, ow = plan.OW;
        pixie_conv_desc desc;
        std::memset(&desc, 0, sizeof desc);
        if (o.out_d) { desc.out_d = od; desc.out_h = oh; desc.out_w = ow; }
        const bool f16 = s.w16;
        const bool raw = !o.pro && o.affine_store.empty();
        if (f16 && raw) for (auto& t : parts) stats(t);

        TP out = o.out_ptr ? external(o.out_ptr, cout, od, oh, ow) : make(cout, od, oh, ow);
        desc.d_in0 = x0->p; desc.c0 = x0->c;
        desc.d_in1 = x1 ? x1->p : nullptr; desc.c1 = x1 ? x1->c : 0;
        desc.in_d = x0->d; desc.in_h = x0->h; desc.in_w = x0->w;
        desc.upsample = o.upsample ? 1 : 0;
        desc.stride = o.stride;
        desc.ksize = ksize;
        if (o.pro) { desc.d_pro_a = o.pro->a; desc.d_pro_b = o.pro->b; }
        if (!o.affine_store.empty()) { desc.d_gamma = P(o.affine_store + ".weight"); desc.d_beta = P(o.affine_store + ".bias"); }
        desc.act = o.act;
        desc.d_bias = P(wkey + ".bias");
        desc.c_out = cout;
        desc.d_residual = o.residual ? o.residual->p : nullptr;
        desc.d_out = out->p;
        if (!f16) {
            desc.d_w = w32(wkey);
            if (!dry) ok(pixie_conv3d_forward(&desc, stream), "pixie_conv3d_forward");
            return out;
        }
        desc.d_w16 = w16(wkey, s.subpixel);
        desc.w16_subpixel = s.subpixel ? 1 : 0;
        if (o.skip_parts) {
            const std::vector<TP>& sp = *o.skip_parts;
            desc.d_skip_in0 = sp[0]->p; desc.skip_c0 = sp[0]->c;
            desc.d_skip_in1 = sp.size() > 1 ? sp[1]->p : nullptr; desc.skip_c1 = sp.size() > 1 ? sp[1]->c : 0;
            desc.d_skip_w16 = w16(o.skip_key);
            desc.d_skip_bias = P(o.skip_key + ".bias");
            desc.d_skip_amax0 = sp[0]->slot; desc.d_skip_amax1 = sp.size() > 1 ? sp[1]->slot : nullptr;
        }
        if (raw) {
            desc.d_in_amax0 = parts[0]->slot;
            desc.d_in_amax1 = x1 ? parts[1]->slot : nullptr;
        } else {
            desc.in_bound = o.bound;
        }
        std::unique_ptr<Scratch> workspace;
        if (plan.workspace_bytes > 0) { workspace.reset(new Scratch(this, plan.workspace_bytes)); desc.d_workspace = workspace->as<void>(); }
        bool have_stats = false;
        if (net->fuse_stats) {
            uint32_t* slot = new_slot();
            const int64_t nfl = plan.stats_floats;
            if (nfl > 0 && (!workspace || net->split_stats)) {
                out->partials_off = arena.alloc(nfl * (int64_t)sizeof(float));
                desc.d_out_stats = arena.ptr<float>(out->partials_off);
                desc.d_out_amax = slot;
                have_stats = true;
                out->slot = slot;
            }
        }
        if (!dry) ok(pixie_conv3d_forward(&desc, stream), "pixie_conv3d_forward");
        if (have_stats) {
            out->sums_off = arena.alloc((int64_t)cout * 2 * sizeof(double));
            out->sums = arena.ptr<double>(out->sums_off);
            out->pdesc = desc;
        }
        return out;
    }

    TP res(const Blk& b, const std::vector<TP>& parts) {
        const std::string& p = b.prefix;
        const int64_t spatial = parts[0]->spatial();
        AB pro = norm_finalize(parts, spatial, 0, 1, nullptr, nullptr);
        ConvOpt o1; o1.pro = &pro; o1.affine_store = p + ".in_layers.0"; o1.act = ACT_LEAKY; o1.bound = norm_bound(p + ".in_layers.0", spatial);
        TP h = conv(parts, p + ".in_layers.2", b.cout, 3, o1);
        AB pro2 = norm_finalize({h}, spatial, 0, 1, nullptr, nullptr);
        TP skip = parts[0];
        ConvOpt o2; o2.pro = &pro2; o2.affine_store = p + ".out_layers.0"; o2.act = ACT_LEAKY; o2.bound = norm_bound(p + ".out_layers.0", spatial);
        if (b.cin != b.cout) {
            if (net->fold_skip && skip_foldable(h, b.cout, 3, parts)) {
                skip.reset();
                for (auto& t : parts) stats(t);
                o2.skip_parts = &parts; o2.skip_key = p + ".skip_connection";
            } else {
                skip = conv(parts, p + ".skip_connection", b.cout, 1, ConvOpt{});
            }
        }
        o2.residual = skip;
        return conv({h}, p + ".out_layers.3", b.cout, 3, o2);
    }
    TP attn(const Blk& b, const TP& x) {
        const std::string& p = b.prefix;
        const int c = x->c;
        const int64_t spatial = x->spatial();
        AB pro = norm_finalize({x}, spatial, 1, 32, P(p + ".norm.weight"), P(p + ".norm.bias"));
        ConvOpt o; o.pro = &pro; o.bound = norm_bound(p + ".norm", spatial * (c / 32));
        TP qkv = conv({x}, p + ".qkv", 3 * c, 1, o);
        TP att = make(c, x->d, x->h, x->w);
        if (!dry) ok(pixie_attention_forward(qkv->p, att->p, c, (int)spatial, stream), "pixie_attention_forward");
        qkv.reset();
        ConvOpt o2; o2.residual = x;
        return conv({att}, p + ".proj_out", c, 1, o2);
    }
    TP block(const Blk& b, const std::vector<TP>& parts, const Tens* up_to) {
        if (b.kind == RES) return res(b, parts);
        const TP& x = parts[0];
        if (b.kind == ATTN) return attn(b, x);
        if (b.kind == DOWN) { ConvOpt o; o.stride = 2; return conv({x}, b.prefix + ".op", b.cout, 3, o); }
        if (b.kind == UP) {
            ConvOpt o; o.upsample = true;
            if (up_to) { o.out_d = up_to->d; o.out_h = up_to->h; o.out_w = up_to->w; }
            return conv({x}, b.prefix + ".conv", b.cout, 3, o);
        }
        fail("pixie_unet: unexpected block kind");
    }

    TP forward(const float* d_feat, const float* d_proj0, int D, int H, int W, float* d_out) {
        const Cfg& c = net->cfg;
        const int64_t spatial = (int64_t)D * H * W;
        TP x;
        AB pro_in; const AB* pro_in_p = nullptr;
        int act_in = ACT_NONE; float bound_in = 0.0f;
        if (c.has_projector()) {
            const std::string q = "projector.net.";
            const int hid = c.projector_hidden();
            if (!hid) {
                const int g = std::max(c.cond_dim / 2, 1);
                x = conv({external(d_feat, c.feature_channels, D, H, W)}, q + "0", c.cond_dim, 1, ConvOpt{});
                pro_in = norm_finalize({x}, spatial, 1, g, P(q + "1.weight"), P(q + "1.bias"));
                act_in = ACT_SILU;
                bound_in = norm_bound(q + "1", spatial * (c.cond_dim / g));
            } else {
                if (d_proj0) x = external(d_proj0, hid, D, H, W);
                else x = conv({external(d_feat, c.feature_channels, D, H, W)}, q + "0", hid, 1, ConvOpt{});
                AB pro = norm_finalize({x}, spatial, 1, 32, P(q + "1.weight"), P(q + "1.bias"));
                ConvOpt o; o.pro = &pro; o.act = ACT_SILU; o.bound = norm_bound(q + "1", spatial * (hid / 32));
                x = conv({x}, q + "3", hid, 3, o);
                AB pro2 = norm_finalize({x}, spatial, 1, 32, P(q + "4.weight"), P(q + "4.bias"));
                ConvOpt o2; o2.pro = &pro2; o2.act = ACT_SILU; o2.bound = norm_bound(q + "4", spatial * (hid / 32));
                x = conv({x}, q + "6", c.cond_dim, 1, o2);
                pro_in = norm_finalize({x}, spatial, 1, 32, P(q + "7.weight"), P(q + "7.bias"));
                bound_in = norm_bound(q + "7", spatial * std::max(c.cond_dim / 32, 1));
            }
            pro_in_p = &pro_in;
        } else {
            x = external(d_feat, c.feature_channels, D, H, W);
        }
        const Plan& plan = net->plan;
        std::vector<TP> hs;
        const Blk& first = plan.in_blocks[0][0];
        ConvOpt of; of.pro = pro_in_p; of.act = act_in; of.bound = bound_in;
        TP h = conv({x}, first.prefix, first.cout, 3, of);
        x.reset();
        pro_in = AB{};
        hs.push_back(h);
        for (size_t i = 1; i < plan.in_blocks.size(); ++i) {
            for (const Blk& b : plan.in_blocks[i]) h = block(b, {h}, nullptr);
            hs.push_back(h);
        }
        for (const Blk& b : plan.middle) h = block(b, {h}, nullptr);
        for (auto& seq : plan.out_blocks) {
            TP skip = hs.back(); hs.pop_back();
            if (skip->d != h->d || skip->h != h->h || skip->w != h->w) fail("pixie_unet_forward: skip tensor and decoder tensor differ in size");
            std::vector<TP> parts{h, skip};
            h.reset(); skip.reset();
            for (const Blk& b : seq) {
                TP nh = block(b, parts, (b.kind == UP && !hs.empty()) ? hs.back().get() : nullptr);
                parts.clear();
                parts.push_back(nh);
            }
            h = parts[0];
        }
        AB pro = norm_finalize({h}, h->spatial(), 0, 1, nullptr, nullptr);
        ConvOpt oo; oo.pro = &pro; oo.affine_store = "unet.out.0"; oo.act = ACT_LEAKY; oo.bound = norm_bound("unet.out.0", h->spatial());
        oo.out_ptr = d_out;
        return conv({h}, "unet.out.2", c.out_channels, 3, oo);
    }
};

Tens::~Tens() {
    if (!ex) return;
    if (off >= 0) ex->arena.release(off);
    if (sums_off >= 0) ex->arena.release(sums_off);
    if (partials_off >= 0) ex->arena.release(partials_off);
}

void refresh_bounds(pixie_unet* net, void* stream) {
    std::vector<std::pair<std::string, int>> todo;
    int n_norm = 0;
    for (const Param& p : net->params) {
        if (!p.norm || p.key.size() < 7 || p.key.compare(p.key.size() - 7, 7, ".weight") != 0) continue;
        const std::string key = p.key.substr(0, p.key.size() - 7);
        const Param& pb = net->param(key + ".bias");
        Bound& b = net->bounds[key];
        if (b.wver != p.version || b.bver != pb.version) todo.push_back({key, 2 * n_norm});
        ++n_norm;
    }
    if (todo.empty()) return;
    const size_t bytes = (size_t)2 * n_norm * sizeof(uint32_t);
    if (!net->d_bound_slots && hipMalloc(&net->d_bound_slots, bytes) != hipSuccess) fail("pixie_unet: hipMalloc failed");
    net->h_bound_slots.assign((size_t)2 * n_norm, 0u);
    hipStream_t s = as_stream(stream);
    if (hipMemsetAsync(net->d_bound_slots, 0, bytes, s) != hipSuccess) fail("pixie_unet: hipMemsetAsync failed");
    for (auto& t : todo) {
        const Param& pw = net->param(t.first + ".weight");
        const Param& pb = net->param(t.first + ".bias");
        if (!pw.d || !pb.d) fail("pixie_unet_forward: parameter '%s' was never set", t.first.c_str());
        ok(pixie_tensor_amax(pw.d, pw.numel, net->d_bound_slots + t.second, stream), "pixie_tensor_amax");
        ok(pixie_tensor_amax(pb.d, pb.numel, net->d_bound_slots + t.second + 1, stream), "pixie_tensor_amax");
    }
    if (hipMemcpyAsync(net->h_bound_slots.data(), net->d_bound_slots, bytes, hipMemcpyDeviceToHost, s) != hipSuccess ||
        hipStreamSynchronize(s) != hipSuccess)
        fail("pixie_unet: reading the normalisation bounds back failed: %s", hipGetErrorString(hipGetLastError()));
    for (auto& t : todo) {
        Bound& b = net->bounds[t.first];
        std::memcpy(&b.wmax, &net->h_bound_slots[t.second], 4);
        std::memcpy(&b.bmax, &net->h_bound_slots[t.second + 1], 4);
        b.wver = net->param(t.first + ".weight").version;
        b.bver = net->param(t.first + ".bias").version;
    }
}

__global__ void zero_head_kernel(uint4* p, int64_t n16) {
    const int64_t i = (int64_t)blockIdx.x * 256 + threadIdx.x;
    if (i < n16) p[i] = make_uint4(0u, 0u, 0u, 0u);
}

constexpr int64_t kSlotAlign = 256;
int64_t slot_region_bytes(int n_slots) { return ((int64_t)n_slots * 4 + kSlotAlign - 1) / kSlotAlign * kSlotAlign; }
int64_t zsum_region_bytes(int64_t n_doubles) { return (n_doubles * 8 + kSlotAlign - 1) / kSlotAlign * kSlotAlign; }

Sized size_pass(pixie_unet* net, int D, int H, int W, bool from_proj0) {
    auto key = std::make_tuple(D, H, W, from_proj0);
    auto it = net->sized.find(key);
    if (it != net->sized.end()) return it->second;
    Exec ex;
    ex.net = net; ex.dry = true; ex.stream = nullptr;
    ex.arena.reset(reinterpret_cast<char*>(0x10000000), (int64_t)1 << 50);
    {
        const float* fake = reinterpret_cast<const float*>(0x100);
        TP out = ex.forward(from_proj0 ? nullptr : fake, from_proj0 ? fake : nullptr, D, H, W, reinterpret_cast<float*>(0x100));
    }
    Sized r{ex.arena.peak + slot_region_bytes(ex.slot_next) + zsum_region_bytes(ex.zsum_next), ex.slot_next, ex.zsum_next};
    net->sized[key] = r;
    return r;
}

template <class F> int guarded(F f) {
    try { return f(); }
    catch (const std::exception& e) { return set_error("%s", e.what()); }
}

}
}

extern "C" int pixie_unet_create(pixie_unet** out, const pixie_unet_config* c) {
    PX_REQUIRE(out && c, "pixie_unet_create: null argument");
    PX_REQUIRE(c->n_channel_mult >= 1 && c->n_channel_mult <= 8 && c->n_attention_resolutions >= 0 && c->n_attention_resolutions <= 8,
               "pixie_unet_create: channel_mult needs 1..8 entries, attention_resolutions 0..8");
    PX_REQUIRE(c->feature_channels > 0 && c->cond_dim > 0 && c->model_channels > 0 && c->num_res_blocks > 0 && c->grid_size > 0 && c->out_channels > 0,
               "pixie_unet_create: non-positive size");
    PX_REQUIRE(c->precision == 0 || c->precision == 1, "pixie_unet_create: precision is 0 (f16x3) or 1 (exact fp32)");
    return guarded([&] {
        std::unique_ptr<pixie_unet> n(new pixie_unet);
        n->cfg.feature_channels = c->feature_channels; n->cfg.cond_dim = c->cond_dim; n->cfg.model_channels = c->model_channels;
        n->cfg.num_res_blocks = c->num_res_blocks; n->cfg.grid_size = c->grid_size; n->cfg.out_channels = c->out_channels;
        n->cfg.precision = c->precision;
        n->cfg.mult.assign(c->channel_mult, c->channel_mult + c->n_channel_mult);
        n->cfg.attn.assign(c->attention_resolutions, c->attention_resolutions + c->n_attention_resolutions);
        n->plan = build_plan(n->cfg);
        n->params = param_table(n->cfg, n->plan);
        for (size_t i = 0; i < n->params.size(); ++i) n->index[n->params[i].key] = (int)i;
        const char* fs = getenv("PIXIE_FUSE_STATS"); n->fuse_stats = !(fs && fs[0] == '0');
        const char* sk = getenv("PIXIE_CONV_SPLIT_K"); n->split_k = !(sk && sk[0] == '0');
        const char* fk = getenv("PIXIE_FOLD_SKIP"); n->fold_skip = !(fk && fk[0] == '0');
        const char* ss = getenv("PIXIE_SPLIT_STATS"); n->split_stats = !(ss && ss[0] == '0');
        const char* sx = getenv("PIXIE_CONV_SUBPIXEL"); n->subpixel = !(sx && sx[0] == '0');
        *out = n.release();
        return 0;
    });
}

extern "C" int pixie_unet_destroy(pixie_unet* h) {
    if (!h) return 0;
    for (auto& kv : h->packed16) if (kv.second.d) (void)hipFree(kv.second.d);
    for (auto& kv : h->packed32) if (kv.second.d) (void)hipFree(kv.second.d);
    if (h->d_bound_slots) (void)hipFree(h->d_bound_slots);
    while (!h->replays.empty()) h->drop_replay(0);
    delete h;
    return 0;
}

extern "C" int pixie_unet_param_count(const pixie_unet* h) { return h ? (int)h->params.size() : 0; }

extern "C" int pixie_unet_param_info(const pixie_unet* h, int i, const char** key, int64_t* numel, int32_t* ndim, int64_t shape[5]) {
    PX_REQUIRE(h && i >= 0 && i < (int)h->params.size(), "pixie_unet_param_info: index out of range");
    const Param& p = h->params[i];
    if (key) *key = p.key.c_str();
    if (numel) *numel = p.numel;
    if (ndim) *ndim = (int32_t)p.shape.size();
    if (shape) for (size_t k = 0; k < p.shape.size() && k < 5; ++k) shape[k] = p.shape[k];
    return 0;
}

extern "C" int pixie_unet_set_param(pixie_unet* h, const char* key, const float* d_values, int64_t numel) {
    PX_REQUIRE(h && key && d_values, "pixie_unet_set_param: null argument");
    auto it = h->index.find(key);
    PX_REQUIRE(it != h->index.end(), "pixie_unet_set_param: unexpected key '%s' (the reference's load_state_dict(strict=True) raises here too)", key);
    Param& p = h->params[it->second];
    PX_REQUIRE(numel == p.numel, "pixie_unet_set_param: '%s' has %lld elements, got %lld", key, (long long)p.numel, (long long)numel);
    p.d = d_values;
    ++p.version;
    ++h->epoch;
    return 0;
}

extern "C" int64_t pixie_unet_workspace_bytes(pixie_unet* h, int d, int hh, int w) {
    if (!h || d <= 0 || hh <= 0 || w <= 0) { set_error("pixie_unet_workspace_bytes: bad argument"); return -1; }
    int64_t bytes = -1;
    const int rc = guarded([&] {
        bytes = size_pass(h, d, hh, w, false).bytes;
        if (h->cfg.projector_hidden() > 0) bytes = std::max(bytes, size_pass(h, d, hh, w, true).bytes);
        return 0;
    });
    return rc == 0 ? bytes : -1;
}

extern "C" int pixie_unet_forward(pixie_unet* h, const float* d_feat, const float* d_proj0, int d, int hh, int w, float* d_out,
                                  void* d_workspace, int64_t workspace_bytes, void* stream) {
    PX_REQUIRE(h && d_out && d_workspace && (d_feat || d_proj0), "pixie_unet_forward: null argument");
    PX_REQUIRE(d == h->cfg.grid_size && hh == d && w == d,
               "pixie_unet_forward: the network was built for a %d^3 grid (its LayerNorm parameters have that shape), got %d x %d x %d", h->cfg.grid_size, d, hh, w);
    PX_REQUIRE(!d_proj0 || h->cfg.projector_hidden() > 0, "pixie_unet_forward: d_proj0 needs the hidden-128 projector (feature_channels > cond_dim)");
    PX_REQUIRE(d_feat || (d_proj0 && h->cfg.has_projector()), "pixie_unet_forward: d_feat is null");
    return guarded([&] {
        const auto sized = size_pass(h, d, hh, w, d_proj0 != nullptr);
        if (workspace_bytes < sized.bytes)
            fail("pixie_unet_forward: workspace of %lld bytes, this grid needs %lld (pixie_unet_workspace_bytes)", (long long)workspace_bytes, (long long)sized.bytes);
        auto launch_all = [&] {
            Exec ex;
            ex.net = h; ex.dry = false; ex.stream = stream;
            const int64_t slot_bytes = slot_region_bytes(sized.slots), head_bytes = slot_bytes + zsum_region_bytes(sized.zsum_doubles);
            ex.slots = static_cast<uint32_t*>(d_workspace);
            ex.slot_cap = sized.slots;
            ex.zsums = reinterpret_cast<double*>(static_cast<char*>(d_workspace) + slot_bytes);
            ex.zsum_cap = sized.zsum_doubles;
            hipLaunchKernelGGL(zero_head_kernel, dim3((unsigned)((head_bytes / 16 + 255) / 256)), dim3(256), 0, as_stream(stream),
                               static_cast<uint4*>(d_workspace), head_bytes / 16);
            if (hipGetLastError() != hipSuccess) fail("pixie_unet_forward: clearing the workspace head failed");
            ex.arena.reset(static_cast<char*>(d_workspace) + head_bytes, workspace_bytes - head_bytes);
            TP out = ex.forward(d_feat, d_proj0, d, hh, w, d_out);
        };
        if (h->use_graph) {
            for (size_t i = 0; i < h->replays.size(); ++i) {
                const pixie_unet::Replay& r = h->replays[i];
                if (r.feat != d_feat || r.proj0 != d_proj0 || r.out != d_out || r.ws != d_workspace || r.d != d) continue;
                if (r.epoch != h->epoch) { h->drop_replay(i); break; }
                if (hipGraphLaunch(r.exec, as_stream(stream)) != hipSuccess) fail("pixie_unet_forward: hipGraphLaunch failed: %s", hipGetErrorString(hipGetLastError()));
                if (i + 1 != h->replays.size()) std::rotate(h->replays.begin() + (long)i, h->replays.begin() + (long)i + 1, h->replays.end());
                return 0;
            }
        }
        if (h->use_graph && as_stream(stream) == nullptr)
            fail("pixie_unet_forward: option \"graph\" needs a non-default stream (the legacy stream cannot be captured); pass a created stream or set graph = 0");
        refresh_bounds(h, stream);
        launch_all();
        if (h->use_graph) {
            hipStream_t st = as_stream(stream);
            if (hipStreamBeginCapture(st, hipStreamCaptureModeThreadLocal) != hipSuccess)
                fail("pixie_unet_forward: cannot capture on this stream (graph replay needs a non-default stream): %s", hipGetErrorString(hipGetLastError()));
            hipGraph_t graph = nullptr;
            try { launch_all(); }
            catch (...) { (void)hipStreamEndCapture(st, &graph); if (graph) (void)hipGraphDestroy(graph); throw; }
            if (hipStreamEndCapture(st, &graph) != hipSuccess || !graph) fail("pixie_unet_forward: hipStreamEndCapture failed: %s", hipGetErrorString(hipGetLastError()));
            hipGraphExec_t exec = nullptr;
            if (hipGraphInstantiate(&exec, graph, nullptr, nullptr, 0) != hipSuccess) { (void)hipGraphDestroy(graph); fail("pixie_unet_forward: hipGraphInstantiate failed"); }
            if (h->replays.size() >= pixie_unet::kMaxReplays) h->drop_replay(0);
            h->replays.push_back(pixie_unet::Replay{d_feat, d_proj0, d_out, d_workspace, d, h->epoch, graph, exec});
        }
        return 0;
    });
}

extern "C" int pixie_unet_set_option(pixie_unet* h, const char* key, int value) {
    PX_REQUIRE(h && key, "pixie_unet_set_option: null argument");
    const std::string k(key);
    if (k == "graph") {
        h->use_graph = value != 0;
        if (!h->use_graph) while (!h->replays.empty()) h->drop_replay(0);
        return 0;
    }
    return set_error("pixie_unet_set_option: unknown key '%s' (known: graph)", key);
}
```

### pixie_amd/csrc/unet_ops.hip

```cpp
#include <hip/hip_runtime.h>

#include <algorithm>

#include "../../include/pixie_hip.h"
#include "common.h"

namespace pixie {

__global__ __launch_bounds__(256) void channel_sums_kernel(const float* __restrict__ x, long spatial, long seg, double* __restrict__ sums,
                                                           unsigned* __restrict__ amax) {
    const int c = blockIdx.y;
    const long begin = (long)blockIdx.x * seg;
    const long end = begin + seg < spatial ? begin + seg : spatial;
    const float* p = x + (size_t)c * spatial;
    double s1 = 0.0, s2 = 0.0;
    float mx = 0.0f;
    const bool vec_ok = ((reinterpret_cast<size_t>(p + begin) & 15) == 0);
    long i = begin + (long)threadIdx.x * 4;
    if (vec_ok) {
        float a1 = 0.f, a2 = 0.f;
        int cnt = 0;
        for (; i + 3 < end; i += 256 * 4) {
            const float4 v = *reinterpret_cast<const float4*>(p + i);
            a1 += (v.x + v.y) + (v.z + v.w);
            a2 += (v.x * v.x + v.y * v.y) + (v.z * v.z + v.w * v.w);
            mx = fmaxf(fmaxf(mx, fabsf(v.x)), fmaxf(fabsf(v.y), fmaxf(fabsf(v.z), fabsf(v.w))));
            if (++cnt == 64) { s1 += a1; s2 += a2; a1 = 0.f; a2 = 0.f; cnt = 0; }
        }
        s1 += a1; s2 += a2;
        for (long k = i; k < end && k < i + 4; ++k) { const float v = p[k]; s1 += v; s2 += (double)v * v; mx = fmaxf(mx, fabsf(v)); }
    } else {
        for (long k = begin + threadIdx.x; k < end; k += 256) { const float v = p[k]; s1 += v; s2 += (double)v * v; mx = fmaxf(mx, fabsf(v)); }
    }
    for (int off = 32; off > 0; off >>= 1) {
        s1 += __shfl_down(s1, off, 64);
        s2 += __shfl_down(s2, off, 64);
        mx = fmaxf(mx, __shfl_down(mx, off, 64));
    }
    if (amax && (threadIdx.x & 63) == 0 && mx > 0.0f) atomicMax(amax, __float_as_uint(mx));
    __shared__ double red[8];
    const int lane = threadIdx.x & 63, wave = threadIdx.x >> 6;
    if (lane == 0) { red[2 * wave] = s1; red[2 * wave + 1] = s2; }
    __syncthreads();
    if (threadIdx.x == 0) {
        const double t1 = red[0] + red[2] + red[4] + red[6];
        const double t2 = red[1] + red[3] + red[5] + red[7];
        atomicAdd(&sums[2 * c], t1);
        atomicAdd(&sums[2 * c + 1], t2);
    }
}

__global__ void norm_finalize_kernel(const double* __restrict__ sums, int c0, const double* __restrict__ sums1, int channels, double spatial,
                                     int mode, int groups, double eps, const float* __restrict__ weight, const float* __restrict__ bias,
                                     float* __restrict__ a, float* __restrict__ b) {
    const int c = blockIdx.x * blockDim.x + threadIdx.x;
    if (c >= channels) return;
    auto S = [&](int k, int which) { return k < c0 ? sums[2 * k + which] : sums1[2 * (k - c0) + which]; };
    double mean, var;
    if (mode == 0) {
        mean = S(c, 0) / spatial;
        var = S(c, 1) / spatial - mean * mean;
    } else {
        const int cpg = channels / groups;
        const int g = c / cpg;
        double s1 = 0.0, s2 = 0.0;
        for (int k = g * cpg; k < (g + 1) * cpg; ++k) { s1 += S(k, 0); s2 += S(k, 1); }
        const double cnt = spatial * cpg;
        mean = s1 / cnt;
        var = s2 / cnt - mean * mean;
    }
    if (var < 0.0) var = 0.0;
    const double rstd = 1.0 / sqrt(var + eps);
    if (mode == 0) {
        a[c] = (float)rstd;
        b[c] = (float)(-mean * rstd);
    } else {
        const double w = weight ? (double)weight[c] : 1.0;
        const double bb = bias ? (double)bias[c] : 0.0;
        a[c] = (float)(rstd * w);
        b[c] = (float)(bb - mean * rstd * w);
    }
}

__global__ void channel_affine_kernel(const float* __restrict__ x, const float* __restrict__ a, const float* __restrict__ b,
                                      float* __restrict__ y, long spatial, long total) {
    const long i = (long)blockIdx.x * blockDim.x + threadIdx.x;
    if (i >= total) return;
    const int c = (int)(i / spatial);
// ... 117 lines not shown
        ++it;
        tile = next;
    }

    __syncthreads();
    float* wm = sm;
    float* wl = wm + ATT_WAVES * ATT_BQ;
    float* wo = wl + ATT_WAVES * ATT_BQ;
    if (quad == 0) wm[wave * ATT_BQ + col] = m;
    __syncthreads();
    float M = -3.0e38f;
#pragma unroll
    for (int w = 0; w < ATT_WAVES; ++w) M = fmaxf(M, wm[w * ATT_BQ + col]);
    const float fw = __expf(m - M);
    if (quad == 0) wl[wave * ATT_BQ + col] = l * fw;
#pragma unroll
    for (int mt = 0; mt < MT; ++mt) {
        float* dst = wo + ((size_t)wave * C + 16 * mt + 4 * quad) * ATT_BQ + col;
        dst[0 * ATT_BQ] = O[mt].x * fw;
        dst[1 * ATT_BQ] = O[mt].y * fw;
        dst[2 * ATT_BQ] = O[mt].z * fw;
        dst[3 * ATT_BQ] = O[mt].w * fw;
    }
    __syncthreads();
    for (int i = tid; i < C * ATT_BQ; i += ATT_WAVES * 64) {
        const int c = i >> 4, qi = i & 15;
        float acc = 0.0f, lt = 0.0f;
#pragma unroll
        for (int w = 0; w < ATT_WAVES; ++w) {
            acc += wo[((size_t)w * C + c) * ATT_BQ + qi];
            lt += wl[w * ATT_BQ + qi];
        }
        if (t0 + qi < T) out[(size_t)c * T + t0 + qi] = acc / lt;
    }
}

__global__ void combine_kernel(const float* __restrict__ logits, int ncls, const float* __restrict__ cont, long spatial,
                               float* __restrict__ combined, int* __restrict__ argmax_out) {
    const long i = (long)blockIdx.x * blockDim.x + threadIdx.x;
    if (i >= spatial) return;
    int best = 0;
    float bv = logits[i];
    for (int c = 1; c < ncls; ++c) {
        const float v = logits[(size_t)c * spatial + i];
        if (v > bv) { bv = v; best = c; }
    }
    for (int c = 0; c < 3; ++c) combined[(size_t)c * spatial + i] = cont[(size_t)c * spatial + i];
    for (int c = 0; c < ncls; ++c) combined[(size_t)(3 + c) * spatial + i] = (c == best) ? 1.0f : 0.0f;
    if (argmax_out) argmax_out[i] = best;
}

__global__ void combine_ids_kernel(const int* __restrict__ seg, int ncls, const float* __restrict__ cont, long spatial,
                                   float* __restrict__ combined) {
    const long i = (long)blockIdx.x * blockDim.x + threadIdx.x;
    if (i >= spatial) return;
    const int id = seg[i];
    for (int c = 0; c < 3; ++c) combined[(size_t)c * spatial + i] = cont[(size_t)c * spatial + i];
    for (int c = 0; c < ncls; ++c) combined[(size_t)(3 + c) * spatial + i] = (c == id) ? 1.0f : 0.0f;
}

__global__ __launch_bounds__(256) void pack_fields_kernel(const float* __restrict__ cont, const int* __restrict__ seg, long n_float, long n_vox,
                                                          unsigned char* __restrict__ wire, long wire_bytes) {
    const long t = (long)blockIdx.x * blockDim.x + threadIdx.x;
    float4* wf = reinterpret_cast<float4*>(wire);
    if (4 * t + 3 < n_float) wf[t] = reinterpret_cast<const float4*>(cont)[t];
    else for (long i = 4 * t; i < n_float; ++i) reinterpret_cast<float*>(wire)[i] = cont[i];
    unsigned char* wb = wire + 4 * n_float;
    if (4 * t + 3 < n_vox && (n_vox & 3) == 0) {
        const int4 q = reinterpret_cast<const int4*>(seg)[t];
        reinterpret_cast<unsigned*>(wb)[t] = (unsigned)(q.x & 0xff) | ((unsigned)(q.y & 0xff) << 8) | ((unsigned)(q.z & 0xff) << 16) | ((unsigned)(q.w & 0xff) << 24);
    } else {
        for (long i = 4 * t; i < n_vox && i < 4 * t + 4; ++i) wb[i] = (unsigned char)seg[i];
    }
    if (t == 0) for (long i = 4 * n_float + n_vox; i < wire_bytes; ++i) wire[i] = 0;
}

template <int C>
static int launch_attention(const float* qkv, float* out, int T, hipStream_t st) {
    const size_t merge = ((size_t)ATT_WAVES * C * ATT_BQ + 2 * ATT_WAVES * ATT_BQ) * sizeof(float);
    const size_t qs = (size_t)C * ATT_BQ * sizeof(float);
    const size_t lds = merge > qs ? merge : qs;
    auto kern = attention_kernel<C>;
    PX_CHECK_HIP(allow_max_dynamic_lds(reinterpret_cast<const void*>(kern)));
    hipLaunchKernelGGL(kern, dim3((T + ATT_BQ - 1) / ATT_BQ), dim3(ATT_WAVES * 64), lds, st, qkv, out, T);
    PX_CHECK_HIP(hipGetLastError());
    return 0;
}

__global__ __launch_bounds__(256) void voxel_grid_to_ncdhw_kernel(const _Float16* __restrict__ src, float* __restrict__ dst, long nvox, int C) {
    __shared__ float tile[64][65];
    const long v0 = (long)blockIdx.x * 64;
    const int c0 = blockIdx.y * 64;
    const int tx = threadIdx.x & 63, ty = threadIdx.x >> 6;
    for (int r = ty; r < 64; r += 4) {
        const long v = v0 + r;
        const int c = c0 + tx;
        tile[r][tx] = (v < nvox && c < C) ? (float)src[v * C + c] : 0.0f;
    }
    __syncthreads();
    for (int r = ty; r < 64; r += 4) {
        const long v = v0 + tx;
        const int c = c0 + r;
        if (v < nvox && c < C) dst[(size_t)c * nvox + v] = tile[tx][r];
    }
}

}

using namespace pixie;

extern "C" int pixie_voxel_grid_to_ncdhw(const void* d_feat_dhwc_f16, int d, int h, int w, int channels, float* d_out_cdhw, void* stream) {
    PX_REQUIRE(d_feat_dhwc_f16 && d_out_cdhw && d > 0 && h > 0 && w > 0 && channels > 0, "pixie_voxel_grid_to_ncdhw: bad arguments");
    const long nvox = (long)d * h * w;
    hipLaunchKernelGGL(voxel_grid_to_ncdhw_kernel, dim3((unsigned)((nvox + 63) / 64), (unsigned)((channels + 63) / 64)), dim3(256), 0,
                       as_stream(stream), static_cast<const _Float16*>(d_feat_dhwc_f16), d_out_cdhw, nvox, channels);
    PX_CHECK_HIP(hipGetLastError());
    return 0;
}

namespace pixie {
int channel_stats_prezeroed(const float* d_x, int channels, int64_t spatial, double* d_sums, uint32_t* d_amax, hipStream_t st) {
    long splits = (spatial + 16383) / 16384;
    const long max_splits = std::max(1L, 2048L / channels);
    if (splits > max_splits) splits = max_splits;
    long seg = (spatial + splits - 1) / splits;
    seg = (seg + 3) & ~3L;
    splits = (spatial + seg - 1) / seg;
    hipLaunchKernelGGL(channel_sums_kernel, dim3((unsigned)splits, (unsigned)channels), dim3(256), 0, st, d_x, (long)spatial, seg, d_sums,
                       reinterpret_cast<unsigned*>(d_amax));
    PX_CHECK_HIP(hipGetLastError());
    return 0;
}
}

namespace pixie {
__global__ void zero_doubles_kernel(double* p, int n) {
    const int i = blockIdx.x * 256 + threadIdx.x;
    if (i < n) p[i] = 0.0;
}
}

extern "C" int pixie_channel_stats(const float* d_x, int channels, int64_t spatial, double* d_sums, uint32_t* d_amax, void* stream) {
    PX_REQUIRE(d_x && d_sums && channels > 0 && spatial > 0, "pixie_channel_stats: bad arguments");
    hipStream_t st = as_stream(stream);
    hipLaunchKernelGGL(pixie::zero_doubles_kernel, dim3((unsigned)((2 * channels + 255) / 256)), dim3(256), 0, st, d_sums, 2 * channels);
    PX_CHECK_HIP(hipGetLastError());
    return pixie::channel_stats_prezeroed(d_x, channels, spatial, d_sums, d_amax, st);
}

extern "C" int pixie_channel_sums(const float* d_x, int channels, int64_t spatial, double* d_sums, void* stream) {
    return pixie_channel_stats(d_x, channels, spatial, d_sums, nullptr, stream);
}

extern "C" int pixie_norm_finalize(const double* d_sums, int channels, int64_t spatial, int mode, int groups, double eps,
                                   const float* d_weight, const float* d_bias, float* d_a, float* d_b, void* stream) {
    PX_REQUIRE(d_sums && d_a && d_b && channels > 0 && spatial > 0, "pixie_norm_finalize: bad arguments");
    PX_REQUIRE(mode == 0 || (mode == 1 && groups > 0 && channels % groups == 0), "pixie_norm_finalize: bad mode/groups");
    hipLaunchKernelGGL(norm_finalize_kernel, dim3(cdiv(channels, 64)), dim3(64), 0, as_stream(stream), d_sums, channels,
                       static_cast<const double*>(nullptr), channels, (double)spatial, mode, groups, eps, d_weight, d_bias, d_a, d_b);
    PX_CHECK_HIP(hipGetLastError());
    return 0;
}

namespace pixie {
int norm_finalize_cat(const double* d_sums0, int c0, const double* d_sums1, int c1, int64_t spatial, int mode, int groups, double eps,
                      const float* d_weight, const float* d_bias, float* d_a, float* d_b, hipStream_t st) {
    const int channels = c0 + c1;
    hipLaunchKernelGGL(norm_finalize_kernel, dim3(cdiv(channels, 64)), dim3(64), 0, st, d_sums0, c0, d_sums1, channels, (double)spatial, mode, groups,
                       eps, d_weight, d_bias, d_a, d_b);
    PX_CHECK_HIP(hipGetLastError());
    return 0;
}
}

extern "C" int pixie_channel_affine(const float* d_x, const float* d_a, const float* d_b, float* d_y, int channels, int64_t spatial,
                                    void* stream) {
    PX_REQUIRE(d_x && d_a && d_b && d_y, "pixie_channel_affine: null argument");
    const long total = (long)channels * spatial;
    hipLaunchKernelGGL(channel_affine_kernel, dim3(cdiv(total, 256)), dim3(256), 0, as_stream(stream), d_x, d_a, d_b, d_y, (long)spatial, total);
    PX_CHECK_HIP(hipGetLastError());
    return 0;
}

extern "C" int pixie_attention_forward(const float* d_qkv, float* d_out, int channels, int tokens, void* stream) {
    PX_REQUIRE(d_qkv && d_out && tokens > 0, "pixie_attention_forward: bad arguments");
    hipStream_t st = as_stream(stream);
    switch (channels) {
        case 32: return launch_attention<32>(d_qkv, d_out, tokens, st);
        case 64: return launch_attention<64>(d_qkv, d_out, tokens, st);
        case 128: return launch_attention<128>(d_qkv, d_out, tokens, st);
        case 256: return launch_attention<256>(d_qkv, d_out, tokens, st);
        default: return set_error("pixie_attention_forward: unsupported channel count %d (32/64/128/256)", channels);
    }
}

extern "C" int pixie_combine_class_ids(const int32_t* d_seg_pred, int num_classes, const float* d_cont, int64_t spatial, float* d_combined,
                                       void* stream) {
    PX_REQUIRE(d_seg_pred && d_cont && d_combined && num_classes > 0 && spatial > 0, "pixie_combine_class_ids: bad arguments");
    hipLaunchKernelGGL(combine_ids_kernel, dim3(cdiv(spatial, 256)), dim3(256), 0, as_stream(stream), d_seg_pred, num_classes, d_cont,
                       (long)spatial, d_combined);
    PX_CHECK_HIP(hipGetLastError());
    return 0;
}

extern "C" int pixie_pack_fields(const float* d_cont, const int32_t* d_seg_pred, int64_t n_scenes, int64_t spatial, void* d_wire, int64_t wire_bytes,
                                 void* stream) {
    const int64_t n_float = 3 * n_scenes * spatial, n_vox = n_scenes * spatial;
    PX_REQUIRE(d_cont && d_seg_pred && d_wire && n_scenes > 0 && spatial > 0, "pixie_pack_fields: bad arguments");
    PX_REQUIRE((((uintptr_t)d_cont | (uintptr_t)d_seg_pred | (uintptr_t)d_wire) & 15) == 0, "pixie_pack_fields: pointers must be 16-byte aligned");
    PX_REQUIRE(wire_bytes >= 4 * n_float + n_vox && wire_bytes < 4 * n_float + n_vox + 16, "pixie_pack_fields: wire buffer of %lld bytes for %lld scenes x %lld voxels",
               (long long)wire_bytes, (long long)n_scenes, (long long)spatial);
    const int64_t threads = (std::max(n_float, n_vox) + 3) / 4;
    hipLaunchKernelGGL(pack_fields_kernel, dim3((unsigned)cdiv(threads, 256)), dim3(256), 0, as_stream(stream), d_cont, d_seg_pred, (long)n_float, (long)n_vox,
                       (unsigned char*)d_wire, (long)wire_bytes);
    PX_CHECK_HIP(hipGetLastError());
    return 0;
}

extern "C" int pixie_combine_predictions(const float* d_logits, int num_classes, const float* d_cont, int64_t spatial, float* d_combined,
                                         int32_t* d_argmax, void* stream) {
    PX_REQUIRE(d_logits && d_cont && d_combined && num_classes > 0 && spatial > 0, "pixie_combine_predictions: bad arguments");
    hipLaunchKernelGGL(combine_kernel, dim3(cdiv(spatial, 256)), dim3(256), 0, as_stream(stream), d_logits, num_classes, d_cont, (long)spatial,
                       d_combined, d_argmax);
    PX_CHECK_HIP(hipGetLastError());
    return 0;
}
```

### pixie_amd/unet.py

```python
from __future__ import annotations

import ctypes as C
import math
import os
import warnings
import weakref
from typing import Dict, List, Optional, Sequence, Tuple

import torch
import torch.nn as nn

from . import _lib
from ._lib import ConvDesc, check
from .unet_plan import Block, UNetConfig, UNetPlan, build_plan, param_shapes, is_norm_key

ACT_NONE, ACT_LEAKY, ACT_SILU = 0, 1, 2
DEFAULT_PRECISION = os.environ.get("PIXIE_CONV_PRECISION", "f16x3")
_ZERO_INIT_SUFFIXES = (".out_layers.3.weight", ".out_layers.3.bias", ".proj_out.weight", ".proj_out.bias",
                       "unet.out.2.weight", "unet.out.2.bias")


def _ptr(t: Optional[torch.Tensor]):
    return C.c_void_p(t.data_ptr()) if t is not None else C.c_void_p(0)

# ... 664 lines not shown
                ent = self._graphs[src.data_ptr()] = (graph, None, static_out)
            else:
                ent = self._graphs["copy"] = (graph, static_in, static_out)
        graph, static_in, static_out = ent
        if static_in is not None:
            static_in.copy_(src)
        graph.replay()
        return static_out.clone()


class SegmentationUNet(_PixieUNet):

    def __init__(self, feature_channels: int, cond_dim: int, model_channels: int, num_res_blocks: int,
                 channel_mult: Tuple[int, ...], attention_resolutions: Tuple[int, ...], grid_size: int, num_classes: int):
        super().__init__(UNetConfig(feature_channels, cond_dim, model_channels, num_res_blocks, tuple(channel_mult),
                                    tuple(attention_resolutions), grid_size, num_classes))


class RegressionUNet(_PixieUNet):

    def __init__(self, feature_channels: int, cond_dim: int, model_channels: int, num_res_blocks: int,
                 channel_mult: Tuple[int, ...], attention_resolutions: Tuple[int, ...], grid_size: int, out_channels: int = 3):
        super().__init__(UNetConfig(feature_channels, cond_dim, model_channels, num_res_blocks, tuple(channel_mult),
                                    tuple(attention_resolutions), grid_size, out_channels))


@torch.no_grad()
def predict_material_field_from_voxel_grid(seg_network: "SegmentationUNet", cont_network: "RegressionUNet", grid_dhwc_f16: torch.Tensor,
                                           dual_stream: Optional[bool] = None):
    dev = next(seg_network.parameters()).device
    g = grid_dhwc_f16
    if g.dim() != 4 or g.dtype != torch.float16 or g.device != dev or dev.type != "cuda":
        raise ValueError("expected a (D, H, W, C) float16 tensor on the networks' HIP device")
    nets = (seg_network, cont_network)
    for net in nets:
        if net.cfg.projector_hidden is None or net.cfg.feature_channels != g.shape[3] or net.conv_precision != "f16x3":
            raise ValueError("the fused grid path needs the hidden-128 projector, matching feature_channels and conv_precision 'f16x3'")
        net._prepare(dev)
    ops = seg_network._runner.ops
    q = "projector.net.0"
    packed = [(net._runner._w16(q), net._runner._b(q)) for net in nets]
    x_seg, x_cont = ops.projector_conv0(g, packed, seg_network.cfg.projector_hidden)
    if dual_stream is None:
        dual_stream = _dual_stream_default(seg_network, cont_network, int(g.shape[0]) * int(g.shape[1]) * int(g.shape[2]))

    def fwd(net, p0):
        return net._forward_graphed(None, p0) if net.use_graph else net._forward_one(None, proj0=p0)

    if dual_stream:
        cur = torch.cuda.current_stream()
        s1, s2 = _side_streams(dev)
        s1.wait_stream(cur); s2.wait_stream(cur)
        with torch.cuda.stream(s1):
            seg_logits = fwd(seg_network, x_seg)[None]
        with torch.cuda.stream(s2):
            cont_pred = fwd(cont_network, x_cont)[None]
        x_seg.record_stream(s1); x_cont.record_stream(s2)
        cur.wait_stream(s1); cur.wait_stream(s2)
        seg_logits.record_stream(cur); cont_pred.record_stream(cur)
    else:
        seg_logits = fwd(seg_network, x_seg)[None]
        cont_pred = fwd(cont_network, x_cont)[None]
    combined, seg_pred = ops.combine(seg_logits[0].contiguous(), cont_pred[0].contiguous())
    return combined[None], seg_pred[None], seg_logits, cont_pred


_SIDE_STREAMS: Dict[str, Tuple[torch.cuda.Stream, torch.cuda.Stream]] = {}


def _dual_stream_default(seg_network, cont_network, voxels: int) -> bool:
    env = os.environ.get("PIXIE_DUAL_STREAM")
    if env is not None:
        return env == "1"
    return not (seg_network.use_graph and cont_network.use_graph and voxels >= 128 ** 3)


def _side_streams(device):
    key = str(device)
    if key not in _SIDE_STREAMS:
        _SIDE_STREAMS[key] = (torch.cuda.Stream(device), torch.cuda.Stream(device))
    return _SIDE_STREAMS[key]


@torch.no_grad()
def predict_material_field(seg_network: SegmentationUNet, cont_network: RegressionUNet, feat_grid: torch.Tensor,
                           dual_stream: Optional[bool] = None):
    if feat_grid.is_cuda and feat_grid.device.index != torch.cuda.current_device():
        with torch.cuda.device(feat_grid.device):
            return predict_material_field(seg_network, cont_network, feat_grid, dual_stream)
    if dual_stream is None:
        dual_stream = _dual_stream_default(seg_network, cont_network, int(feat_grid[0, 0].numel()))
    if dual_stream and feat_grid.is_cuda:
        cur = torch.cuda.current_stream()
        s1, s2 = _side_streams(feat_grid.device)
        s1.wait_stream(cur); s2.wait_stream(cur)
        with torch.cuda.stream(s1):
            seg_logits = seg_network(feat_grid)
        with torch.cuda.stream(s2):
            cont_pred = cont_network(feat_grid)
        feat_grid.record_stream(s1); feat_grid.record_stream(s2)
        cur.wait_stream(s1); cur.wait_stream(s2)
        seg_logits.record_stream(cur); cont_pred.record_stream(cur)
    else:
        seg_logits = seg_network(feat_grid)
        cont_pred = cont_network(feat_grid)
    ops = seg_network._runner.ops
    combined, seg_pred = [], []
    for n in range(feat_grid.shape[0]):
        cmb, am = ops.combine(seg_logits[n].contiguous(), cont_pred[n].contiguous())
        combined.append(cmb)
        seg_pred.append(am)
    return torch.stack(combined), torch.stack(seg_pred), seg_logits, cont_pred
```

Before: 27.52 million voxels/s.

## Run seg and regression U-Nets as one paired launch stream with grouped kernels

Adds a paired forward that records the kernel launches of both U-Nets, then merges matching launches into single grouped kernels. Each grouped kernel covers both networks by doubling grid.z and choosing the argument set from blockIdx.z. The pair is captured in one HIP graph and used by default when both nets use graphs at full grid size. The aim is to halve launch count and fill the GPU better on small, low-occupancy layers. In exchange it adds recording machinery, an extra output clone, and more complex capture and fallback logic.

```diff
diff --git a/include/pixie_hip.h b/include/pixie_hip.h
--- a/include/pixie_hip.h
+++ b/include/pixie_hip.h
@@ -178,6 +178,9 @@
 int64_t pixie_unet_workspace_bytes(pixie_unet* h, int d, int hh, int w);
 int pixie_unet_forward(pixie_unet* h, const float* d_feat, const float* d_proj0, int d, int hh, int w, float* d_out,
                        void* d_workspace, int64_t workspace_bytes, void* stream);
+int pixie_unet_forward_pair(pixie_unet* h0, pixie_unet* h1, const float* d_feat, int d, int hh, int w, float* d_out0, float* d_out1,
+                            void* d_workspace0, int64_t workspace0_bytes, void* d_workspace1, int64_t workspace1_bytes, void* stream,
+                            int32_t launch_counts[4]);
 int pixie_unet_set_option(pixie_unet* h, const char* key, int value);
 
 typedef struct pixie_field_desc {
diff --git a/pixie_amd/_lib.py b/pixie_amd/_lib.py
--- a/pixie_amd/_lib.py
+++ b/pixie_amd/_lib.py
@@ -285,6 +285,7 @@
     "pixie_unet_workspace_bytes": (_I64, [_VP, _I, _I, _I]),
     "pixie_unet_set_option": (_I, [_VP, _S, _I]),
     "pixie_unet_forward": (_I, [_VP, _VP, _VP, _I, _I, _I, _VP, _VP, _I64, _VP]),
+    "pixie_unet_forward_pair": (_I, [_VP, _VP, _VP, _I, _I, _I, _VP, _VP, _VP, _I64, _VP, _I64, _VP, _VP]),
     "pixie_combine_class_ids": (_I, [_VP, _I, _VP, _I64, _VP, _VP]),
     "pixie_combine_predictions": (_I, [_VP, _I, _VP, _I64, _VP, _VP, _VP]),
     "pixie_voxel_grid_to_ncdhw": (_I, [_VP, _I, _I, _I, _I, _VP, _VP]),
diff --git a/pixie_amd/csrc/common.hip b/pixie_amd/csrc/common.hip
--- a/pixie_amd/csrc/common.hip
+++ b/pixie_amd/csrc/common.hip
@@ -5,6 +5,7 @@
 #include <utility>
 
 #include "../../include/pixie_hip.h"
+#include "launch_record.h"
 
 namespace pixie {
 hipError_t allow_max_dynamic_lds(const void* kern) {
@@ -18,6 +19,11 @@
     e = hipFuncSetAttribute(kern, hipFuncAttributeMaxDynamicSharedMemorySize, 160 * 1024);
     if (e == hipSuccess) done.insert({kern, dev});
     return e;
+}
+
+LaunchList*& launch_recorder() {
+    static thread_local LaunchList* rec = nullptr;
+    return rec;
 }
 
 std::string& last_error_ref() {
diff --git a/pixie_amd/csrc/conv16_body.h b/pixie_amd/csrc/conv16_body.h
--- a/pixie_amd/csrc/conv16_body.h
+++ b/pixie_amd/csrc/conv16_body.h
@@ -2,10 +2,11 @@
 #include <type_traits>
 
 #include "conv16_device.h"
+#include "launch_record.h"
 
 namespace pixie {
 
-template <int KS, int MB, int NB, bool EX = false, bool SP = false, int SK = 0, bool PAIR = false>
+template <int KS, int MB, int NB, bool EX = false, bool SP = false, int SK = 0, bool PAIR = false, bool GRP = false>
 __device__ __forceinline__ void conv3d_f16x3_body(const Conv16Args& A) {
     static_assert(!PAIR || (MB == 2 && !EX && !SP && SK == 0), "pair form: the plain f16x3 body with 64 c_out per quartet");
     static_assert(!SP || (KS == 3 && NB == 4 && !EX), "sub-pixel path: 3^3, two x parities x two voxel blocks per wave");
@@ -15,6 +16,7 @@
     constexpr int NW = 4, NT = 64 * NW;
     const int bufsz = 4 * A.CS;
 
+    const unsigned zslice = GRP ? blockIdx.z - (blockIdx.z >= (gridDim.z >> 1) ? (gridDim.z >> 1) : 0u) : blockIdx.z;
     const int tid = threadIdx.x;
     const int lane = tid & 63;
     const int quartet = PAIR ? __builtin_amdgcn_readfirstlane(tid >> 8) : 0;
@@ -102,7 +104,7 @@
 
     float inv2 = 0.0f;
     {
-        const int c_begin = A.partial ? (int)blockIdx.z * A.chunks_per_slice * 16 : 0;
+        const int c_begin = A.partial ? (int)zslice * A.chunks_per_slice * 16 : 0;
         const int c_end = A.partial ? min(A.cin, c_begin + A.chunks_per_slice * 16) : A.cin;
         if constexpr (PAIR) {
             const int n_chunks = (c_end - c_begin) >> 4;
@@ -151,6 +153,14 @@
 __global__ __launch_bounds__(256, 2) void conv3d_f16x3_subpixel_kernel(Conv16Args A) {
     conv3d_f16x3_body<3, MB, 4, false, true>(A);
 }
+template <int KS, int MB, int NB>
+__global__ __launch_bounds__(256, 2) void conv3d_f16x3_group_kernel(Group2<Conv16Args> G) {
+    conv3d_f16x3_body<KS, MB, NB, false, false, 0, false, true>(G.a[blockIdx.z >= (gridDim.z >> 1) ? 1 : 0]);
+}
+template <int MB>
+__global__ __launch_bounds__(256, 2) void conv3d_f16x3_subpixel_group_kernel(Group2<Conv16Args> G) {
+    conv3d_f16x3_body<3, MB, 4, false, true, 0, false, true>(G.a[blockIdx.z >= (gridDim.z >> 1) ? 1 : 0]);
+}
 __global__ __launch_bounds__(256, 2) void conv3d_f16x3_c64_fullres_kernel(Conv16Args A) {
     conv3d_f16x3_body<3, 2, 4>(A);
 }
diff --git a/pixie_amd/csrc/conv16_epilogue.h b/pixie_amd/csrc/conv16_epilogue.h
--- a/pixie_amd/csrc/conv16_epilogue.h
+++ b/pixie_amd/csrc/conv16_epilogue.h
@@ -1,6 +1,6 @@
     const float inv = EX ? 1.0f : (SK != 0 ? inv2 : __uint_as_float(A.w16[0].x) * pow2i(-ex));
     if (A.partial) {
-        float* dst = A.partial + (size_t)blockIdx.z * A.cout * OSP;
+        float* dst = A.partial + (size_t)zslice * A.cout * OSP;
 #pragma unroll
         for (int mb = 0; mb < MB; ++mb)
 #pragma unroll
diff --git a/pixie_amd/csrc/conv3d_f16x3.hip b/pixie_amd/csrc/conv3d_f16x3.hip
--- a/pixie_amd/csrc/conv3d_f16x3.hip
+++ b/pixie_amd/csrc/conv3d_f16x3.hip
@@ -6,6 +6,7 @@
 #include "common.h"
 #include "conv_plan.h"
 #include "conv_launch.h"
+#include "launch_record.h"
 #include "conv16_device.h"
 #include "conv16_body.h"
 #include "conv_stat_kernels.h"
@@ -41,6 +42,21 @@
     return nullptr;
 }
 
+using ConvGroupKernel = void (*)(Group2<Conv16Args>);
+template <int KS, int MB, int NB> static ConvGroupKernel conv16_group_pick() {
+    if constexpr ((KS == 3 && MB == 2 && NB == 4) || (KS == 1 && MB == 2 && (NB == 2 || NB == 1))) return conv3d_f16x3_group_kernel<KS, MB, NB>;
+    else return nullptr;
+}
+static ConvGroupKernel conv16_group_kernel(const ConvPlan& p, bool skip = false) {
+    if (p.path == CONV_F16X3_SUBPIXEL) return p.MB == 2 ? conv3d_f16x3_subpixel_group_kernel<2> : nullptr;
+    if (p.fullres || p.path == CONV_EXACT_TILED || skip) return nullptr;
+#define PX_CONV16_PICK(KS_, MB_, NB_)                \
+    if (p.KS == KS_ && p.MB == MB_ && p.NB == NB_) return conv16_group_pick<KS_, MB_, NB_>();
+    PX_CONV_VARIANTS(PX_CONV16_PICK)
+#undef PX_CONV16_PICK
+    return nullptr;
+}
+
 #ifdef PIXIE_DIAG
 static int g_conv_keep_four_wave = 0;
 #endif
@@ -58,11 +74,13 @@
     return nullptr;
 }
 
-static int launch(ConvKernel kern, const ConvPlan& p, const Conv16Args& a, hipStream_t st, size_t pair_lds = 0) {
+static int launch(ConvKernel kern, const ConvPlan& p, const Conv16Args& a, hipStream_t st, size_t pair_lds = 0, ConvGroupKernel twin = nullptr) {
     PX_REQUIRE(kern != nullptr, "conv: no kernel variant for ksize=%d MB=%d NB=%d", p.KS, p.MB, p.NB);
     PX_CHECK_HIP(allow_max_dynamic_lds(reinterpret_cast<const void*>(kern)));
-    if (pair_lds) hipLaunchKernelGGL(kern, dim3(p.grid_x, p.grid_y / 2, 1), dim3(512), pair_lds, st, a);
-    else hipLaunchKernelGGL(kern, dim3(p.grid_x, p.grid_y, p.grid_z), dim3(256), p.lds_bytes, st, a);
+    if (twin && launch_recorder()) PX_CHECK_HIP(allow_max_dynamic_lds(reinterpret_cast<const void*>(twin)));
+    if (pair_lds) px_launch(kern, dim3(p.grid_x, p.grid_y / 2, 1), dim3(512), pair_lds, st, a);
+    else if (twin) px_launch_grouped(kern, twin, dim3(p.grid_x, p.grid_y, p.grid_z), dim3(256), p.lds_bytes, st, a);
+    else px_launch(kern, dim3(p.grid_x, p.grid_y, p.grid_z), dim3(256), p.lds_bytes, st, a);
     PX_CHECK_HIP(hipGetLastError());
     return 0;
 }
@@ -109,7 +127,9 @@
     PX_REQUIRE(p.refusal != CONV_BAD_LDS, "f16x3 conv: tile needs %zu B of LDS", p.lds_bytes);
     PX_REQUIRE(p.f16x3(), "f16x3 conv: bad sizes");
     const size_t pair_lds = conv_pair_lds(p, a.sk_w16 != nullptr);
-    if (int rc = launch(pair_lds ? conv16_pair_kernel(p) : conv16_kernel(p, a.sk_w16 != nullptr, a.sk_c0), p, a, st, pair_lds)) return rc;
+    if (int rc = launch(pair_lds ? conv16_pair_kernel(p) : conv16_kernel(p, a.sk_w16 != nullptr, a.sk_c0), p, a, st, pair_lds,
+                        pair_lds ? nullptr : conv16_group_kernel(p, a.sk_w16 != nullptr)))
+        return rc;
     if (p.slices == 1) return 0;
     const long osp = (long)a.OD * a.OH * a.OW, n_elems = (long)a.cout * osp;
     if (d->d_out_stats) {
@@ -117,13 +137,13 @@
         double* rstats = reinterpret_cast<double*>(d->d_out_stats);
         PX_REQUIRE((reinterpret_cast<size_t>(rstats) & 7) == 0, "f16x3 conv: d_out_stats of a split-K launch must be 8-byte aligned");
         const bool vec = osp % 4 == 0 && ((reinterpret_cast<size_t>(a.partial) | reinterpret_cast<size_t>(a.residual) | reinterpret_cast<size_t>(a.out)) & 15) == 0;
-        if (vec) hipLaunchKernelGGL(splitk_reduce_stats_kernel<true>, rgrid, dim3(256), 0, st, a.partial, p.slices, n_elems, osp, a.bias, a.residual,
-                                    a.out, rstats, d->d_out_amax);
-        else hipLaunchKernelGGL(splitk_reduce_stats_kernel<false>, rgrid, dim3(256), 0, st, a.partial, p.slices, n_elems, osp, a.bias, a.residual,
-                                a.out, rstats, d->d_out_amax);
+        if (vec) px_launch_grouped(splitk_reduce_stats_kernel<true>, splitk_reduce_stats_group_kernel<true>, rgrid, dim3(256), 0, st, a.partial, p.slices,
+                                   n_elems, osp, a.bias, a.residual, a.out, rstats, d->d_out_amax);
+        else px_launch_grouped(splitk_reduce_stats_kernel<false>, splitk_reduce_stats_group_kernel<false>, rgrid, dim3(256), 0, st, a.partial, p.slices,
+                               n_elems, osp, a.bias, a.residual, a.out, rstats, d->d_out_amax);
     } else {
-        hipLaunchKernelGGL(splitk_reduce_kernel, dim3((unsigned)((n_elems + 255) / 256)), dim3(256), 0, st, a.partial, p.slices, n_elems, osp,
-                           a.bias, a.residual, a.out);
+        px_launch(splitk_reduce_kernel, dim3((unsigned)((n_elems + 255) / 256)), dim3(256), 0, st, a.partial, p.slices, n_elems, osp,
+                  a.bias, a.residual, a.out);
     }
     PX_CHECK_HIP(hipGetLastError());
     return 0;
@@ -182,7 +202,7 @@
 
 extern "C" int pixie_stats_finalize(const float* d_stats, const pixie_conv_desc* d, double* d_sums, void* stream) {
     PX_REQUIRE(d_stats && d && d_sums, "pixie_stats_finalize: null argument");
-    hipLaunchKernelGGL(stats_finalize_kernel, dim3((unsigned)d->c_out), dim3(256), 0, as_stream(stream), stat_parts(plan_of(d), d_stats), d_sums);
+    px_launch(stats_finalize_kernel, dim3((unsigned)d->c_out), dim3(256), 0, as_stream(stream), stat_parts(plan_of(d), d_stats), d_sums);
     PX_CHECK_HIP(hipGetLastError());
     return 0;
 }
@@ -199,8 +219,8 @@
     const StatParts none{nullptr, 0, 0, 0, 0};
     const StatParts p0 = d_stats0 ? stat_parts(plan_of(desc0), d_stats0) : none;
     const StatParts p1 = d_stats1 ? stat_parts(plan_of(desc1), d_stats1) : none;
-    hipLaunchKernelGGL(stats_norm_finalize_kernel, dim3((unsigned)(mode == 0 ? channels : groups)), dim3(256), 0, as_stream(stream), p0, d_sums0, c0,
-                       p1, d_sums1, channels, (double)spatial, mode, groups, eps, d_weight, d_bias, d_a, d_b);
+    px_launch_grouped(stats_norm_finalize_kernel, stats_norm_finalize_group_kernel, dim3((unsigned)(mode == 0 ? channels : groups)), dim3(256), 0,
+                      as_stream(stream), p0, d_sums0, c0, p1, d_sums1, channels, (double)spatial, mode, groups, eps, d_weight, d_bias, d_a, d_b);
     PX_CHECK_HIP(hipGetLastError());
     return 0;
 }
diff --git a/pixie_amd/csrc/conv3d_mfma.hip b/pixie_amd/csrc/conv3d_mfma.hip
--- a/pixie_amd/csrc/conv3d_mfma.hip
+++ b/pixie_amd/csrc/conv3d_mfma.hip
@@ -4,6 +4,7 @@
 #include "common.h"
 #include "conv_launch.h"
 #include "conv_plan.h"
+#include "launch_record.h"
 
 namespace pixie {
 
@@ -188,7 +189,7 @@
 static int launch_variant(const ConvArgs& a, size_t lds_bytes, dim3 grid, hipStream_t st) {
     auto kern = conv3d_mfma_kernel<KS, MB, NB, CK>;
     PX_CHECK_HIP(allow_max_dynamic_lds(reinterpret_cast<const void*>(kern)));
-    hipLaunchKernelGGL(kern, grid, dim3(256), lds_bytes, st, a);
+    px_launch(kern, grid, dim3(256), lds_bytes, st, a);
     PX_CHECK_HIP(hipGetLastError());
     return 0;
 }
diff --git a/pixie_amd/csrc/conv_stat_kernels.h b/pixie_amd/csrc/conv_stat_kernels.h
--- a/pixie_amd/csrc/conv_stat_kernels.h
+++ b/pixie_amd/csrc/conv_stat_kernels.h
@@ -2,6 +2,7 @@
 #include <hip/hip_runtime.h>
 
 #include "conv_plan.h"
+#include "launch_record.h"
 
 namespace pixie {
 
@@ -33,40 +34,20 @@
                                                                   double spatial, int mode, int groups, double eps,
                                                                   const float* __restrict__ weight, const float* __restrict__ bias,
                                                                   float* __restrict__ a, float* __restrict__ b) {
-    __shared__ double r[8];
-    const int cpg = mode == 0 ? 1 : channels / groups;
-    const int first = blockIdx.x * cpg;
-    double s1 = 0.0, s2 = 0.0;
-    for (int k = first; k < first + cpg; ++k) {
-        const bool in0 = k < c0;
-        const StatParts& P = in0 ? P0 : P1;
-        double* sums = in0 ? sums0 : sums1;
-        const int kc = in0 ? k : k - c0;
-        double t1, t2;
-        if (P.n > 0) {
-            block_channel_sums(P, kc, r, t1, t2);
-            if (threadIdx.x == 0) { sums[2 * kc] = t1; sums[2 * kc + 1] = t2; }
-        } else {
-            t1 = sums[2 * kc]; t2 = sums[2 * kc + 1];
-        }
-        s1 += t1; s2 += t2;
-    }
-    const double cnt = mode == 0 ? spatial : spatial * cpg;
-    const double mean = s1 / cnt;
-    double var = s2 / cnt - mean * mean;
-    if (var < 0.0) var = 0.0;
-    const double rstd = 1.0 / sqrt(var + eps);
-    for (int k = first + threadIdx.x; k < first + cpg; k += 256) {
-        if (mode == 0) {
-            a[k] = (float)rstd;
-            b[k] = (float)(-mean * rstd);
-        } else {
-            const double w = weight ? (double)weight[k] : 1.0;
-            const double bb = bias ? (double)bias[k] : 0.0;
-            a[k] = (float)(rstd * w);
-            b[k] = (float)(bb - mean * rstd * w);
-        }
-    }
+#include "conv_stat_norm_finalize.h"
+}
+struct StatsNormFinalizeArgs {
+    StatParts P0; double* sums0; int c0; StatParts P1; double* sums1; int channels; double spatial; int mode, groups; double eps;
+    const float* weight; const float* bias; float* a; float* b;
+};
+__global__ __launch_bounds__(256) void stats_norm_finalize_group_kernel(Group2<StatsNormFinalizeArgs> G) {
+    const StatsNormFinalizeArgs& A = G.a[blockIdx.z];
+    const StatParts& P0 = A.P0; const StatParts& P1 = A.P1;
+    double* sums0 = A.sums0; double* sums1 = A.sums1;
+    const int c0 = A.c0, channels = A.channels, mode = A.mode, groups = A.groups;
+    const double spatial = A.spatial, eps = A.eps;
+    const float* weight = A.weight; const float* bias = A.bias; float* a = A.a; float* b = A.b;
+#include "conv_stat_norm_finalize.h"
 }
 
 __global__ __launch_bounds__(256) void splitk_reduce_kernel(const float* __restrict__ partial, int slices, long n_elems, long osp,
@@ -84,68 +65,19 @@
 __global__ __launch_bounds__(256) void splitk_reduce_stats_kernel(const float* __restrict__ partial, int slices, long n_elems, long osp,
                                                                   const float* __restrict__ bias, const float* residual, float* out,
                                                                   double* __restrict__ stats, unsigned* out_amax) {
-    const int c = blockIdx.y;
-    const long seg0 = (long)blockIdx.x * kReduceSeg;
-    const size_t base = (size_t)c * osp;
-    const float bv = bias ? bias[c] : 0.0f;
-    double s1 = 0.0, s2 = 0.0;
-    float mx = 0.0f;
-    if (VEC) {
-#pragma unroll
-        for (int k = 0; k < kReduceSeg / 1024; ++k) {
-            const long j = seg0 + k * 1024 + (long)threadIdx.x * 4;
-            if (j < osp) {
-                const size_t i = base + j;
-                float4 v = *reinterpret_cast<const float4*>(partial + i);
-                for (int s = 1; s < slices; ++s) {
-                    const float4 q = *reinterpret_cast<const float4*>(partial + (size_t)s * n_elems + i);
-                    v.x += q.x; v.y += q.y; v.z += q.z; v.w += q.w;
-                }
-                if (bias) { v.x += bv; v.y += bv; v.z += bv; v.w += bv; }
-                if (residual) {
-                    const float4 q = *reinterpret_cast<const float4*>(residual + i);
-                    v.x += q.x; v.y += q.y; v.z += q.z; v.w += q.w;
-                }
-                *reinterpret_cast<float4*>(out + i) = v;
-                const double x = v.x, y = v.y, z = v.z, w = v.w;
-                s1 += (x + y) + (z + w);
-                s2 += (x * x + y * y) + (z * z + w * w);
-                mx = fmaxf(fmaxf(mx, fmaxf(fabsf(v.x), fabsf(v.y))), fmaxf(fabsf(v.z), fabsf(v.w)));
-            }
-        }
-    } else {
-#pragma unroll 4
-        for (int k = 0; k < kReduceSeg / 256; ++k) {
-            const long j = seg0 + k * 256 + threadIdx.x;
-            if (j < osp) {
-                const size_t i = base + j;
-                float v = partial[i];
-                for (int s = 1; s < slices; ++s) v += partial[(size_t)s * n_elems + i];
-                if (bias) v += bv;
-                if (residual) v += residual[i];
-                out[i] = v;
-                const double x = v;
-                s1 += x; s2 += x * x; mx = fmaxf(mx, fabsf(v));
-            }
-        }
-    }
-    for (int off = 32; off > 0; off >>= 1) {
-        s1 += __shfl_down(s1, off, 64);
-        s2 += __shfl_down(s2, off, 64);
-        mx = fmaxf(mx, __shfl_down(mx, off, 64));
-    }
-    __shared__ double r[8];
-    __shared__ float rmx[4];
-    const int lane = threadIdx.x & 63, wave = threadIdx.x >> 6;
-    if (lane == 0) { r[2 * wave] = s1; r[2 * wave + 1] = s2; rmx[wave] = mx; }
-    __syncthreads();
-    if (threadIdx.x == 0) {
-        double* dst = stats + ((size_t)c * gridDim.x + blockIdx.x) * 2;
-        dst[0] = r[0] + r[2] + r[4] + r[6];
-        dst[1] = r[1] + r[3] + r[5] + r[7];
-        const unsigned m = __float_as_uint(fmaxf(fmaxf(rmx[0], rmx[1]), fmaxf(rmx[2], rmx[3])));
-        if (out_amax && m > __hip_atomic_load(out_amax, __ATOMIC_RELAXED, __HIP_MEMORY_SCOPE_AGENT)) atomicMax(out_amax, m);
-    }
+#include "conv_stat_splitk_reduce.h"
+}
+struct SplitkReduceStatsArgs {
+    const float* partial; int slices; long n_elems, osp; const float* bias; const float* residual; float* out; double* stats; unsigned* out_amax;
+};
+template <bool VEC>
+__global__ __launch_bounds__(256) void splitk_reduce_stats_group_kernel(Group2<SplitkReduceStatsArgs> G) {
+    const SplitkReduceStatsArgs& A = G.a[blockIdx.z];
+    const float* partial = A.partial; const float* bias = A.bias; const float* residual = A.residual;
+    const int slices = A.slices;
+    const long n_elems = A.n_elems, osp = A.osp;
+    float* out = A.out; double* stats = A.stats; unsigned* out_amax = A.out_amax;
+#include "conv_stat_splitk_reduce.h"
 }
 
 __global__ __launch_bounds__(256) void amax_kernel(const float* __restrict__ x, long n, unsigned* __restrict__ slot) {
diff --git a/pixie_amd/csrc/conv_stat_norm_finalize.h b/pixie_amd/csrc/conv_stat_norm_finalize.h
--- /dev/null
+++ b/pixie_amd/csrc/conv_stat_norm_finalize.h
@@ -0,0 +1,34 @@
+    __shared__ double r[8];
+    const int cpg = mode == 0 ? 1 : channels / groups;
+    const int first = blockIdx.x * cpg;
+    double s1 = 0.0, s2 = 0.0;
+    for (int k = first; k < first + cpg; ++k) {
+        const bool in0 = k < c0;
+        const StatParts& P = in0 ? P0 : P1;
+        double* sums = in0 ? sums0 : sums1;
+        const int kc = in0 ? k : k - c0;
+        double t1, t2;
+        if (P.n > 0) {
+            block_channel_sums(P, kc, r, t1, t2);
+            if (threadIdx.x == 0) { sums[2 * kc] = t1; sums[2 * kc + 1] = t2; }
+        } else {
+            t1 = sums[2 * kc]; t2 = sums[2 * kc + 1];
+        }
+        s1 += t1; s2 += t2;
+    }
+    const double cnt = mode == 0 ? spatial : spatial * cpg;
+    const double mean = s1 / cnt;
+    double var = s2 / cnt - mean * mean;
+    if (var < 0.0) var = 0.0;
+    const double rstd = 1.0 / sqrt(var + eps);
+    for (int k = first + threadIdx.x; k < first + cpg; k += 256) {
+        if (mode == 0) {
+            a[k] = (float)rstd;
+            b[k] = (float)(-mean * rstd);
+        } else {
+            const double w = weight ? (double)weight[k] : 1.0;
+            const double bb = bias ? (double)bias[k] : 0.0;
+            a[k] = (float)(rstd * w);
+            b[k] = (float)(bb - mean * rstd * w);
+        }
+    }
diff --git a/pixie_amd/csrc/conv_stat_splitk_reduce.h b/pixie_amd/csrc/conv_stat_splitk_reduce.h
--- /dev/null
+++ b/pixie_amd/csrc/conv_stat_splitk_reduce.h
@@ -0,0 +1,62 @@
+    const int c = blockIdx.y;
+    const long seg0 = (long)blockIdx.x * kReduceSeg;
+    const size_t base = (size_t)c * osp;
+    const float bv = bias ? bias[c] : 0.0f;
+    double s1 = 0.0, s2 = 0.0;
+    float mx = 0.0f;
+    if (VEC) {
+#pragma unroll
+        for (int k = 0; k < kReduceSeg / 1024; ++k) {
+            const long j = seg0 + k * 1024 + (long)threadIdx.x * 4;
+            if (j < osp) {
+                const size_t i = base + j;
+                float4 v = *reinterpret_cast<const float4*>(partial + i);
+                for (int s = 1; s < slices; ++s) {
+                    const float4 q = *reinterpret_cast<const float4*>(partial + (size_t)s * n_elems + i);
+                    v.x += q.x; v.y += q.y; v.z += q.z; v.w += q.w;
+                }
+                if (bias) { v.x += bv; v.y += bv; v.z += bv; v.w += bv; }
+                if (residual) {
+                    const float4 q = *reinterpret_cast<const float4*>(residual + i);
+                    v.x += q.x; v.y += q.y; v.z += q.z; v.w += q.w;
+                }
+                *reinterpret_cast<float4*>(out + i) = v;
+                const double x = v.x, y = v.y, z = v.z, w = v.w;
+                s1 += (x + y) + (z + w);
+                s2 += (x * x + y * y) + (z * z + w * w);
+                mx = fmaxf(fmaxf(mx, fmaxf(fabsf(v.x), fabsf(v.y))), fmaxf(fabsf(v.z), fabsf(v.w)));
+            }
+        }
+    } else {
+#pragma unroll 4
+        for (int k = 0; k < kReduceSeg / 256; ++k) {
+            const long j = seg0 + k * 256 + threadIdx.x;
+            if (j < osp) {
+                const size_t i = base + j;
+                float v = partial[i];
+                for (int s = 1; s < slices; ++s) v += partial[(size_t)s * n_elems + i];
+                if (bias) v += bv;
+                if (residual) v += residual[i];
+                out[i] = v;
+                const double x = v;
+                s1 += x; s2 += x * x; mx = fmaxf(mx, fabsf(v));
+            }
+        }
+    }
+    for (int off = 32; off > 0; off >>= 1) {
+        s1 += __shfl_down(s1, off, 64);
+        s2 += __shfl_down(s2, off, 64);
+        mx = fmaxf(mx, __shfl_down(mx, off, 64));
+    }
+    __shared__ double r[8];
+    __shared__ float rmx[4];
+    const int lane = threadIdx.x & 63, wave = threadIdx.x >> 6;
+    if (lane == 0) { r[2 * wave] = s1; r[2 * wave + 1] = s2; rmx[wave] = mx; }
+    __syncthreads();
+    if (threadIdx.x == 0) {
+        double* dst = stats + ((size_t)c * gridDim.x + blockIdx.x) * 2;
+        dst[0] = r[0] + r[2] + r[4] + r[6];
+        dst[1] = r[1] + r[3] + r[5] + r[7];
+        const unsigned m = __float_as_uint(fmaxf(fmaxf(rmx[0], rmx[1]), fmaxf(rmx[2], rmx[3])));
+        if (out_amax && m > __hip_atomic_load(out_amax, __ATOMIC_RELAXED, __HIP_MEMORY_SCOPE_AGENT)) atomicMax(out_amax, m);
+    }
diff --git a/pixie_amd/csrc/launch_list.h b/pixie_amd/csrc/launch_list.h
--- /dev/null
+++ b/pixie_amd/csrc/launch_list.h
@@ -0,0 +1,82 @@
+#pragma once
+#include <cstddef>
+#include <cstdint>
+#include <cstring>
+#include <vector>
+
+namespace pixie {
+
+enum LaunchSection : int { SEC_FULLRES = 0, SEC_INNER = 1 };
+
+struct LaunchRec {
+    const void* kernel = nullptr;
+    const void* twin = nullptr;
+    uint32_t grid[3] = {1, 1, 1}, block[3] = {1, 1, 1};
+    uint32_t lds = 0;
+    int section = SEC_FULLRES;
+    int net = 0;
+    std::vector<unsigned char> args;
+    std::vector<uint32_t> offs;
+    uint32_t arg_stride = 0;
+};
+
+struct LaunchList {
+    std::vector<LaunchRec> recs;
+    int section = SEC_FULLRES;
+};
+
+inline bool launch_groupable(const LaunchRec& a, const LaunchRec& b) {
+    return a.kernel == b.kernel && a.twin != nullptr && a.twin == b.twin && a.lds == b.lds && a.arg_stride == b.arg_stride &&
+           a.args.size() == b.args.size() && std::memcmp(a.grid, b.grid, sizeof a.grid) == 0 && std::memcmp(a.block, b.block, sizeof a.block) == 0;
+}
+
+inline LaunchRec launch_group(const LaunchRec& a, const LaunchRec& b) {
+    LaunchRec g;
+    g.kernel = a.twin;
+    std::memcpy(g.grid, a.grid, sizeof g.grid);
+    std::memcpy(g.block, a.block, sizeof g.block);
+    g.grid[2] *= 2;
+    g.lds = a.lds;
+    g.section = a.section;
+    g.net = -1;
+    g.args.assign((size_t)2 * a.arg_stride, 0);
+    std::memcpy(g.args.data(), a.args.data(), a.args.size());
+    std::memcpy(g.args.data() + a.arg_stride, b.args.data(), b.args.size());
+    g.offs.assign(1, 0u);
+    g.arg_stride = 2 * a.arg_stride;
+    return g;
+}
+
+inline std::vector<LaunchRec> merge_pair(const LaunchList& l0, const LaunchList& l1, int* n_grouped = nullptr, bool group = true) {
+    const LaunchList* ls[2] = {&l0, &l1};
+    size_t lo[2], hi[2];
+    for (int k = 0; k < 2; ++k) {
+        const std::vector<LaunchRec>& r = ls[k]->recs;
+        lo[k] = hi[k] = r.size();
+        for (size_t i = 0; i < r.size(); ++i)
+            if (r[i].section == SEC_INNER) { if (lo[k] == r.size()) lo[k] = i; hi[k] = i + 1; }
+        if (lo[k] == r.size()) lo[k] = hi[k] = r.size();
+    }
+    std::vector<LaunchRec> out;
+    out.reserve(l0.recs.size() + l1.recs.size());
+    auto put = [&](int k, size_t i) { out.push_back(ls[k]->recs[i]); out.back().net = k; };
+    int grouped = 0;
+    for (int k = 0; k < 2; ++k)
+        for (size_t i = 0; i < lo[k]; ++i) put(k, i);
+    const size_t n0 = hi[0] - lo[0], n1 = hi[1] - lo[1];
+    for (size_t i = 0; i < (n0 > n1 ? n0 : n1); ++i) {
+        if (group && i < n0 && i < n1 && launch_groupable(l0.recs[lo[0] + i], l1.recs[lo[1] + i])) {
+            out.push_back(launch_group(l0.recs[lo[0] + i], l1.recs[lo[1] + i]));
+            ++grouped;
+            continue;
+        }
+        if (i < n0) put(0, lo[0] + i);
+        if (i < n1) put(1, lo[1] + i);
+    }
+    for (int k = 0; k < 2; ++k)
+        for (size_t i = hi[k]; i < ls[k]->recs.size(); ++i) put(k, i);
+    if (n_grouped) *n_grouped = grouped;
+    return out;
+}
+
+}
diff --git a/pixie_amd/csrc/launch_record.h b/pixie_amd/csrc/launch_record.h
--- /dev/null
+++ b/pixie_amd/csrc/launch_record.h
@@ -0,0 +1,67 @@
+#pragma once
+#include <hip/hip_runtime.h>
+
+#include <type_traits>
+#include <utility>
+
+#include "launch_list.h"
+
+namespace pixie {
+
+LaunchList*& launch_recorder();
+
+template <class Args> struct Group2 { Args a[2]; };
+
+template <class P> inline void launch_push_arg(LaunchRec& r, const P& v) {
+    static_assert(std::is_trivially_copyable<P>::value, "kernel parameters are plain data");
+    const size_t al = alignof(P);
+    const size_t off = (r.args.size() + al - 1) / al * al;
+    r.args.resize(off + sizeof(P), 0);
+    std::memcpy(r.args.data() + off, &v, sizeof(P));
+    r.offs.push_back((uint32_t)off);
+}
+
+template <class... P> constexpr size_t launch_args_stride() {
+    size_t off = 0, ma = 1;
+    ((off = (off + alignof(P) - 1) / alignof(P) * alignof(P) + sizeof(P), ma = alignof(P) > ma ? alignof(P) : ma), ...);
+    return (off + ma - 1) / ma * ma;
+}
+
+template <class... P, class... A>
+inline void px_launch_impl(void (*kern)(P...), const void* twin, dim3 grid, dim3 block, size_t lds, hipStream_t st, A&&... a) {
+    static_assert(sizeof...(P) == sizeof...(A), "one argument per kernel parameter");
+    LaunchList* rec = launch_recorder();
+    if (!rec) {
+        hipLaunchKernelGGL(kern, grid, block, lds, st, std::forward<A>(a)...);
+        return;
+    }
+    LaunchRec r;
+    r.kernel = reinterpret_cast<const void*>(kern);
+    r.twin = twin;
+    r.grid[0] = grid.x; r.grid[1] = grid.y; r.grid[2] = grid.z;
+    r.block[0] = block.x; r.block[1] = block.y; r.block[2] = block.z;
+    r.lds = (uint32_t)lds;
+    r.section = rec->section;
+    (launch_push_arg<P>(r, static_cast<P>(a)), ...);
+    r.arg_stride = (uint32_t)launch_args_stride<P...>();
+    rec->recs.push_back(std::move(r));
+}
+
+template <class... P, class... A>
+inline void px_launch(void (*kern)(P...), dim3 grid, dim3 block, size_t lds, hipStream_t st, A&&... a) {
+    px_launch_impl(kern, nullptr, grid, block, lds, st, std::forward<A>(a)...);
+}
+template <class Args, class... P, class... A>
+inline void px_launch_grouped(void (*kern)(P...), void (*twin)(Group2<Args>), dim3 grid, dim3 block, size_t lds, hipStream_t st, A&&... a) {
+    static_assert(sizeof(Args) == launch_args_stride<P...>(), "the twin's argument struct does not match the kernel's parameters");
+    px_launch_impl(kern, reinterpret_cast<const void*>(twin), grid, block, lds, st, std::forward<A>(a)...);
+}
+
+inline hipError_t launch_rec(const LaunchRec& r, hipStream_t st) {
+    void* argv[32];
+    if (r.offs.size() > 32) return hipErrorInvalidValue;
+    for (size_t i = 0; i < r.offs.size(); ++i) argv[i] = const_cast<unsigned char*>(r.args.data()) + r.offs[i];
+    return hipLaunchKernel(r.kernel, dim3(r.grid[0], r.grid[1], r.grid[2]), dim3(r.block[0], r.block[1], r.block[2]), argv, r.lds, st);
+}
+
+}
diff --git a/pixie_amd/csrc/unet_exec.hip b/pixie_amd/csrc/unet_exec.hip
--- a/pixie_amd/csrc/unet_exec.hip
+++ b/pixie_amd/csrc/unet_exec.hip
@@ -16,6 +16,7 @@
 #include "common.h"
 #include "conv_launch.h"
 #include "conv_plan.h"
+#include "launch_record.h"
 
 namespace pixie {
 int channel_stats_prezeroed(const float* d_x, int channels, int64_t spatial, double* d_sums, uint32_t* d_amax, hipStream_t st);
@@ -276,6 +277,10 @@
     int slot_next = 0, slot_cap = 0;
     double* zsums = nullptr;
     int64_t zsum_next = 0, zsum_cap = 0;
+    LaunchList* rec = nullptr;
+    const float* in_ptr = nullptr;
+    double* in_sums = nullptr; uint32_t* in_slot = nullptr;
+    double* share_sums = nullptr; uint32_t* share_slot = nullptr;
 
     TP make(int c, int d, int h, int w) {
         auto t = std::make_shared<Tens>();
@@ -346,11 +351,14 @@
     void stats(const TP& t) {
         if (t->has_sums || t->partials_off >= 0) return;
         t->has_sums = true;
+        const bool input = t->off < 0 && in_ptr && t->p == in_ptr;
+        if (input && share_slot) { t->sums = share_sums; t->slot = share_slot; return; }
         if (!dry && zsum_next + 2 * t->c > zsum_cap) fail("pixie_unet_forward: out of statistics space (internal sizing error)");
         t->sums = dry ? nullptr : zsums + zsum_next;
         zsum_next += 2 * t->c;
         t->slot = new_slot();
         if (!dry) ok(channel_stats_prezeroed(t->p, t->c, t->spatial(), t->sums, t->slot, as_stream(stream)), "pixie_channel_stats");
+        if (input) { in_sums = t->sums; in_slot = t->slot; }
     }
     struct AB { std::shared_ptr<Scratch> mem; float* a; float* b; };
     AB norm_finalize(const std::vector<TP>& parts, int64_t spatial, int mode, int groups, const float* w, const float* b) {
@@ -515,10 +523,14 @@
         if (b.kind == RES) return res(b, parts);
         const TP& x = parts[0];
         if (b.kind == ATTN) return attn(b, x);
-        if (b.kind == DOWN) { ConvOpt o; o.stride = 2; return conv({x}, b.prefix + ".op", b.cout, 3, o); }
+        if (b.kind == DOWN) {
+            if (rec && x->d == net->cfg.grid_size) rec->section = SEC_INNER;
+            ConvOpt o; o.stride = 2; return conv({x}, b.prefix + ".op", b.cout, 3, o);
+        }
         if (b.kind == UP) {
             ConvOpt o; o.upsample = true;
             if (up_to) { o.out_d = up_to->d; o.out_h = up_to->h; o.out_w = up_to->w; }
+            if (rec && (up_to ? up_to->d : 2 * x->d) == net->cfg.grid_size) rec->section = SEC_FULLRES;
             return conv({x}, b.prefix + ".conv", b.cout, 3, o);
         }
         fail("pixie_unet: unexpected block kind");
@@ -655,6 +667,31 @@
     return r;
 }
 
+void run_pass(pixie_unet* h, const float* d_feat, const float* d_proj0, int d, int hh, int w, float* d_out, void* d_workspace, int64_t workspace_bytes,
+              const Sized& sized, void* stream, LaunchList* rec = nullptr, Exec* ex_out = nullptr, const Exec* share = nullptr) {
+    Exec local;
+    Exec& ex = ex_out ? *ex_out : local;
+    ex.net = h; ex.dry = false; ex.stream = stream; ex.rec = rec;
+    ex.in_ptr = d_feat;
+    if (share && share->in_ptr == d_feat && share->in_slot) { ex.share_sums = share->in_sums; ex.share_slot = share->in_slot; }
+    const int64_t slot_bytes = slot_region_bytes(sized.slots), head_bytes = slot_bytes + zsum_region_bytes(sized.zsum_doubles);
+    ex.slots = static_cast<uint32_t*>(d_workspace);
+    ex.slot_cap = sized.slots;
+    ex.zsums = reinterpret_cast<double*>(static_cast<char*>(d_workspace) + slot_bytes);
+    ex.zsum_cap = sized.zsum_doubles;
+    struct Recording {
+        LaunchList* before;
+        explicit Recording(LaunchList* r) : before(launch_recorder()) { launch_recorder() = r; }
+        ~Recording() { launch_recorder() = before; }
+    } recording(rec);
+    if (rec) rec->section = SEC_FULLRES;
+    px_launch(zero_head_kernel, dim3((unsigned)((head_bytes / 16 + 255) / 256)), dim3(256), 0, as_stream(stream),
+              static_cast<uint4*>(d_workspace), head_bytes / 16);
+    if (!rec && hipGetLastError() != hipSuccess) fail("pixie_unet_forward: clearing the workspace head failed");
+    ex.arena.reset(static_cast<char*>(d_workspace) + head_bytes, workspace_bytes - head_bytes);
+    TP out = ex.forward(d_feat, d_proj0, d, hh, w, d_out);
+}
+
 template <class F> int guarded(F f) {
     try { return f(); }
     catch (const std::exception& e) { return set_error("%s", e.what()); }
@@ -746,20 +783,7 @@
         const auto sized = size_pass(h, d, hh, w, d_proj0 != nullptr);
         if (workspace_bytes < sized.bytes)
             fail("pixie_unet_forward: workspace of %lld bytes, this grid needs %lld (pixie_unet_workspace_bytes)", (long long)workspace_bytes, (long long)sized.bytes);
-        auto launch_all = [&] {
-            Exec ex;
-            ex.net = h; ex.dry = false; ex.stream = stream;
-            const int64_t slot_bytes = slot_region_bytes(sized.slots), head_bytes = slot_bytes + zsum_region_bytes(sized.zsum_doubles);
-            ex.slots = static_cast<uint32_t*>(d_workspace);
-            ex.slot_cap = sized.slots;
-            ex.zsums = reinterpret_cast<double*>(static_cast<char*>(d_workspace) + slot_bytes);
-            ex.zsum_cap = sized.zsum_doubles;
-            hipLaunchKernelGGL(zero_head_kernel, dim3((unsigned)((head_bytes / 16 + 255) / 256)), dim3(256), 0, as_stream(stream),
-                               static_cast<uint4*>(d_workspace), head_bytes / 16);
-            if (hipGetLastError() != hipSuccess) fail("pixie_unet_forward: clearing the workspace head failed");
-            ex.arena.reset(static_cast<char*>(d_workspace) + head_bytes, workspace_bytes - head_bytes);
-            TP out = ex.forward(d_feat, d_proj0, d, hh, w, d_out);
-        };
+        auto launch_all = [&] { run_pass(h, d_feat, d_proj0, d, hh, w, d_out, d_workspace, workspace_bytes, sized, stream); };
         if (h->use_graph) {
             for (size_t i = 0; i < h->replays.size(); ++i) {
                 const pixie_unet::Replay& r = h->replays[i];
@@ -791,6 +815,44 @@
     });
 }
 
+extern "C" int pixie_unet_forward_pair(pixie_unet* h0, pixie_unet* h1, const float* d_feat, int d, int hh, int w, float* d_out0, float* d_out1,
+                                       void* d_workspace0, int64_t workspace0_bytes, void* d_workspace1, int64_t workspace1_bytes, void* stream,
+                                       int32_t* launch_counts) {
+    PX_REQUIRE(h0 && h1 && h0 != h1 && d_feat && d_out0 && d_out1 && d_workspace0 && d_workspace1, "pixie_unet_forward_pair: null argument, or one handle twice");
+    PX_REQUIRE(d_out0 != d_out1 && d_workspace0 != d_workspace1, "pixie_unet_forward_pair: the two networks need outputs and workspaces of their own");
+    pixie_unet* hs[2] = {h0, h1};
+    for (pixie_unet* h : hs)
+        PX_REQUIRE(d == h->cfg.grid_size && hh == d && w == d,
+                   "pixie_unet_forward_pair: a network was built for a %d^3 grid (its LayerNorm parameters have that shape), got %d x %d x %d", h->cfg.grid_size, d, hh, w);
+    return guarded([&] {
+        float* outs[2] = {d_out0, d_out1};
+        void* wss[2] = {d_workspace0, d_workspace1};
+        const int64_t wsb[2] = {workspace0_bytes, workspace1_bytes};
+        Sized sized[2];
+        for (int k = 0; k < 2; ++k) {
+            sized[k] = size_pass(hs[k], d, hh, w, false);
+            if (wsb[k] < sized[k].bytes)
+                fail("pixie_unet_forward_pair: workspace %d of %lld bytes, this grid needs %lld (pixie_unet_workspace_bytes)", k, (long long)wsb[k], (long long)sized[k].bytes);
+        }
+        for (pixie_unet* h : hs) refresh_bounds(h, stream);
+        LaunchList lists[2];
+        Exec ex[2];
+        for (int k = 0; k < 2; ++k)
+            run_pass(hs[k], d_feat, nullptr, d, hh, w, outs[k], wss[k], wsb[k], sized[k], stream, &lists[k], &ex[k], k ? &ex[0] : nullptr);
+        int grouped = 0;
+        const char* pg = getenv("PIXIE_UNET_PAIR_GROUP");
+        const std::vector<LaunchRec> merged = merge_pair(lists[0], lists[1], &grouped, !(pg && pg[0] == '0'));
+        for (const LaunchRec& r : merged)
+            if (launch_rec(r, as_stream(stream)) != hipSuccess) fail("pixie_unet_forward_pair: a launch failed: %s", hipGetErrorString(hipGetLastError()));
+        if (launch_counts) {
+            launch_counts[0] = (int32_t)(lists[0].recs.size() + lists[1].recs.size()); launch_counts[1] = (int32_t)merged.size(); launch_counts[2] = grouped;
+            launch_counts[3] = 0;
+            for (const LaunchRec& r : merged) launch_counts[3] += r.net < 0 && r.lds > 0;
+        }
+        return 0;
+    });
+}
+
 extern "C" int pixie_unet_set_option(pixie_unet* h, const char* key, int value) {
     PX_REQUIRE(h && key, "pixie_unet_set_option: null argument");
     const std::string k(key);
diff --git a/pixie_amd/csrc/unet_ops.hip b/pixie_amd/csrc/unet_ops.hip
--- a/pixie_amd/csrc/unet_ops.hip
+++ b/pixie_amd/csrc/unet_ops.hip
@@ -4,6 +4,7 @@
 
 #include "../../include/pixie_hip.h"
 #include "common.h"
+#include "launch_record.h"
 
 namespace pixie {
 
@@ -287,7 +288,7 @@
     const size_t lds = merge > qs ? merge : qs;
     auto kern = attention_kernel<C>;
     PX_CHECK_HIP(allow_max_dynamic_lds(reinterpret_cast<const void*>(kern)));
-    hipLaunchKernelGGL(kern, dim3((T + ATT_BQ - 1) / ATT_BQ), dim3(ATT_WAVES * 64), lds, st, qkv, out, T);
+    px_launch(kern, dim3((T + ATT_BQ - 1) / ATT_BQ), dim3(ATT_WAVES * 64), lds, st, qkv, out, T);
     PX_CHECK_HIP(hipGetLastError());
     return 0;
 }
@@ -331,8 +332,8 @@
     long seg = (spatial + splits - 1) / splits;
     seg = (seg + 3) & ~3L;
     splits = (spatial + seg - 1) / seg;
-    hipLaunchKernelGGL(channel_sums_kernel, dim3((unsigned)splits, (unsigned)channels), dim3(256), 0, st, d_x, (long)spatial, seg, d_sums,
-                       reinterpret_cast<unsigned*>(d_amax));
+    px_launch(channel_sums_kernel, dim3((unsigned)splits, (unsigned)channels), dim3(256), 0, st, d_x, (long)spatial, seg, d_sums,
+              reinterpret_cast<unsigned*>(d_amax));
     PX_CHECK_HIP(hipGetLastError());
     return 0;
 }
@@ -361,8 +362,8 @@
                                    const float* d_weight, const float* d_bias, float* d_a, float* d_b, void* stream) {
     PX_REQUIRE(d_sums && d_a && d_b && channels > 0 && spatial > 0, "pixie_norm_finalize: bad arguments");
     PX_REQUIRE(mode == 0 || (mode == 1 && groups > 0 && channels % groups == 0), "pixie_norm_finalize: bad mode/groups");
-    hipLaunchKernelGGL(norm_finalize_kernel, dim3(cdiv(channels, 64)), dim3(64), 0, as_stream(stream), d_sums, channels,
-                       static_cast<const double*>(nullptr), channels, (double)spatial, mode, groups, eps, d_weight, d_bias, d_a, d_b);
+    px_launch(norm_finalize_kernel, dim3(cdiv(channels, 64)), dim3(64), 0, as_stream(stream), d_sums, channels,
+              static_cast<const double*>(nullptr), channels, (double)spatial, mode, groups, eps, d_weight, d_bias, d_a, d_b);
     PX_CHECK_HIP(hipGetLastError());
     return 0;
 }
@@ -371,8 +372,8 @@
 int norm_finalize_cat(const double* d_sums0, int c0, const double* d_sums1, int c1, int64_t spatial, int mode, int groups, double eps,
                       const float* d_weight, const float* d_bias, float* d_a, float* d_b, hipStream_t st) {
     const int channels = c0 + c1;
-    hipLaunchKernelGGL(norm_finalize_kernel, dim3(cdiv(channels, 64)), dim3(64), 0, st, d_sums0, c0, d_sums1, channels, (double)spatial, mode, groups,
-                       eps, d_weight, d_bias, d_a, d_b);
+    px_launch(norm_finalize_kernel, dim3(cdiv(channels, 64)), dim3(64), 0, st, d_sums0, c0, d_sums1, channels, (double)spatial, mode, groups,
+              eps, d_weight, d_bias, d_a, d_b);
     PX_CHECK_HIP(hipGetLastError());
     return 0;
 }
diff --git a/pixie_amd/unet.py b/pixie_amd/unet.py
--- a/pixie_amd/unet.py
+++ b/pixie_amd/unet.py
@@ -770,6 +770,71 @@
     return _SIDE_STREAMS[key]
 
 
+def _pair_call(seg_network, cont_network, x: torch.Tensor, counts=None):
+    hs, hc = seg_network._handle, cont_network._handle
+    d, h, w = (int(v) for v in x.shape[1:])
+    outs = [torch.empty((net.cfg.out_channels, d, h, w), device=x.device, dtype=torch.float32) for net in (seg_network, cont_network)]
+    nbytes = [hs.workspace_bytes(d, h, w), hc.workspace_bytes(d, h, w)]
+    wss = [torch.empty(n, device=x.device, dtype=torch.uint8) for n in nbytes]
+    check(hs.lib.pixie_unet_forward_pair(hs._h, hc._h, _ptr(x), d, h, w, _ptr(outs[0]), _ptr(outs[1]), _ptr(wss[0]), nbytes[0], _ptr(wss[1]), nbytes[1],
+                                         _lib.current_stream_ptr(), counts), "pixie_unet_forward_pair")
+    return outs[0], outs[1]
+
+
+def _forward_pair(seg_network, cont_network, feat_grid: torch.Tensor):
+    if os.environ.get("PIXIE_UNET_PAIR", "1") == "0":
+        return None
+    nets = (seg_network, cont_network)
+    if not (feat_grid.is_cuda and feat_grid.dim() == 5 and feat_grid.shape[0] == 1 and seg_network is not cont_network):
+        return None
+    dev = feat_grid.device
+    for net in nets:
+        if not (net.executor == "c" and net.use_graph and net.cfg.feature_channels == feat_grid.shape[1] and next(net.parameters()).device == dev
+                and tuple(feat_grid.shape[2:]) == (net.cfg.grid_size,) * 3):
+            return None
+    with torch.cuda.device(dev):
+        for net in nets:
+            net._prepare(dev)
+        src = feat_grid.detach().to(torch.float32).contiguous()[0]
+        base = (tuple(src.shape), tuple(src.stride()), src.dtype, dev.index, id(cont_network),
+                tuple((net.conv_precision, tuple((id(p), p.data_ptr(), p._version) for p in net._param_list())) for net in nets))
+        graphs = seg_network.__dict__.setdefault("_pair_graphs", {})
+        if graphs.get("base") != base:
+            graphs.clear()
+            graphs.update({"base": base, "first_ptr": None})
+        if graphs.get("failed"):
+            return None
+        ent = graphs.get(src.data_ptr()) or graphs.get("copy")
+        if ent is None:
+            outs = _pair_call(seg_network, cont_network, src)
+            if graphs["first_ptr"] is None:
+                graphs["first_ptr"] = src.data_ptr()
+                return outs[0][None], outs[1][None]
+            in_place = (graphs["first_ptr"] == src.data_ptr() and "copy" not in graphs and os.environ.get("PIXIE_UNET_GRAPH_INPLACE", "1") == "1")
+            try:
+                static_in = src if in_place else src.clone()
+                side = torch.cuda.Stream(dev)
+                side.wait_stream(torch.cuda.current_stream())
+                with torch.cuda.stream(side):
+                    _pair_call(seg_network, cont_network, static_in)
+                torch.cuda.current_stream().wait_stream(side)
+                graph = torch.cuda.CUDAGraph()
+                with torch.cuda.graph(graph, capture_error_mode="thread_local"):
+                    static_outs = _pair_call(seg_network, cont_network, static_in)
+            except RuntimeError as exc:
+                warnings.warn(f"pixie_amd: HIP-graph capture of the paired U-Net forward failed ({exc}); continuing with one graph per network",
+                              RuntimeWarning)
+                graphs["failed"] = True
+                return outs[0][None], outs[1][None]
+            ent = (graph, None if in_place else static_in, static_outs)
+            graphs[src.data_ptr() if in_place else "copy"] = ent
+        graph, static_in, static_outs = ent
+        if static_in is not None:
+            static_in.copy_(src)
+        graph.replay()
+        return static_outs[0].clone()[None], static_outs[1].clone()[None]
+
+
 @torch.no_grad()
 def predict_material_field(seg_network: SegmentationUNet, cont_network: RegressionUNet, feat_grid: torch.Tensor,
                            dual_stream: Optional[bool] = None):
@@ -790,8 +855,12 @@
         cur.wait_stream(s1); cur.wait_stream(s2)
         seg_logits.record_stream(cur); cont_pred.record_stream(cur)
     else:
-        seg_logits = seg_network(feat_grid)
-        cont_pred = cont_network(feat_grid)
+        pair = _forward_pair(seg_network, cont_network, feat_grid)
+        if pair is not None:
+            seg_logits, cont_pred = pair
+        else:
+            seg_logits = seg_network(feat_grid)
+            cont_pred = cont_network(feat_grid)
     ops = seg_network._runner.ops
     combined, seg_pred = [], []
     for n in range(feat_grid.shape[0]):
```

Result: faster. 27.99 million voxels/s (median of 6 runs) (+1.7%).
